# willake/cpu-ray-tracer

Measured on AMD Instinct MI355X. Metric: Mrays/sec (primary+secondary), 1280x720 64spp path trace — pipelined throughput over 878 consecutive 64-spp windows of one progressive render (single_render = one such render alone), higher is better.
Workload: dtype f32; 1 GPU; bunny_scene.xml FileScene BVH-SAH path tracer, 1280x720, 64 spp/step (passes=1, depthLimit=5); 1 step = 64 frames = the next spp window of a progressive render; the 878 steps are one crt_render job (14 render kernel launch(es), a wavefront per (tile, 128 consecutive frames), + ordered accumulate), one sync at the end; triangles=4968, parallelism=tile-wave x1

## Files before the change

cpu-ray-tracer_amd/csrc/abi.cpp:

```cpp
#include "../../include/crt_abi.h"
#include "device/launch.h"
#include "device/tile_class.h"
#include "host/grid_resolution.h"

#include <cmath>
#include <cstdarg>
#include <cstddef>
#include <cstdio>
#include <cstdlib>
#include <cstring>
#include <deque>
#include <string>
#include <algorithm>
#include <vector>
#include <chrono>

static_assert(sizeof(crt_bvh_node) == 32 && sizeof(crt_tri) == 112 && sizeof(crt_tlas_node) == 32, "reference layouts");
static_assert(sizeof(crt::NodePair) == 64 && sizeof(crt::LeafTri) == 48 && sizeof(crt::ShadeTri) == 64 && sizeof(crt::TlasNode) == 32 &&
              sizeof(crt::Instance) == 128 && sizeof(crt::Material) == 32 && offsetof(crt::Instance, T) == 64, "device layouts");
static_assert(sizeof(crt_counters) == sizeof(crt::Counters), "counter layout");
static_assert(sizeof(crt_kd_node) == 48 && sizeof(crt::KdNode) == sizeof(crt_kd_node) && sizeof(crt::AltTri) == 48, "flat KD node (uploaded as it comes), alternative accelerators' triangle record");
static_assert(offsetof(crt::PrimDev, red) == 536 && sizeof(crt::PrimDev) == 552, "PrimDev: 134 floats, then the two texel pointers");
static_assert(sizeof(crt::BlasAltDesc) == 72, "BLAS descriptor");
static_assert(sizeof(crt_shadow_ray) == 28 && sizeof(crt_ray) == 28 && sizeof(crt_hit) == 28, "query records");
static_assert(sizeof(crt_hit_info) == 48 && offsetof(crt_hit_info, material) == 12 && offsetof(crt_hit_info, N) == 16 && offsetof(crt_hit_info, albedo) == 32 && offsetof(crt_hit_info, v) == 44, "crt_hit_info: three 16-byte pieces");
static_assert(sizeof(crt::Instance) == 128 && offsetof(crt::Instance, triCount) == 112, "Instance record");

namespace {

thread_local std::string g_createError;

bool g_hooks = false;
inline const char* hook(const char* name) { return g_hooks ? getenv(name) : nullptr; }

struct EventPair { hipEvent_t a, b; int mode = -1; bool seen = false; };

}

extern "C" uint32_t crt_debug_query_grid(void)
{
    const char* e = hook("CRT_DEBUG_QUERY_GRID");
    const long k = e ? strtol(e, nullptr, 10) : 0;
    return k > 0 ? (uint32_t)(k > 0x7fffffffL ? 0x7fffffffL : k) : 0u;
}

struct crt_ctx {
    crt_config cfg{};
    std::string err;
    hipStream_t stream = nullptr;
    int tilesX = 0, tilesY = 0;
    uint32_t tileFirst = 0, tileStride = 1, tileCount = 0;
    void* dAccOwned = nullptr; void* dAcc = nullptr;
    std::vector<hipStream_t> streams; uint64_t launchSeq = 0;
    struct Region { size_t off, bytes; hipEvent_t freed; bool held = false; };
    std::deque<Region> inflight;
    char* pool = nullptr; size_t poolBytes = 0, poolHead = 0; bool poolCapped = false;
    hipEvent_t mustWait = nullptr;
    std::vector<hipEvent_t> freeEvents;
    std::vector<hipEvent_t> doneEvents;
    struct Ahead { hipEvent_t end; size_t off; const char* slab; uint64_t epoch; uint32_t sppFirst, nf, passes, used; };
    std::deque<Ahead> ahead;
    uint64_t epoch = 1;
    uint64_t tickEpoch = 0; uint32_t tickNextSpp = 0, tickPasses = 0;
    uint32_t aheadFrames = 0;
    hipStream_t aheadStream = nullptr;
    crt::Scene hScene{};
    crt::Counters* dCounters = nullptr;
    uint32_t* dQueryCursor = nullptr;
    int32_t* dInspectCounts = nullptr; void* dInspectWork = nullptr; size_t inspectCap = 0;
    uint32_t* dPixels = nullptr; float* dTileSums = nullptr;
    unsigned long long* dTileClocks = nullptr;
    std::vector<void*> sceneAllocs;
    float meshLo[3] = {0, 0, 0}, meshHi[3] = {0, 0, 0}; bool orderDirty = true;
    uint32_t* dTileOrder = nullptr;
    uint32_t* hTileOrder[2] = {nullptr, nullptr}; hipEvent_t orderCopied[2] = {nullptr, nullptr}; hipEvent_t orderReady = nullptr; int orderFlip = 0;
    bool classDirty = true;
    uint8_t* dTileClass = nullptr;
    uint8_t* hTileClass[2] = {nullptr, nullptr}; hipEvent_t classCopied[2] = {nullptr, nullptr}; int classFlip = 0;
    bool haveScene = false;
    struct Flat { int32_t kind = 0; uint64_t leafOff = 0, tlasOff = 0, tlasPairOff = 0, instOff = 0, shadeOff = 0; uint32_t tlasNodeCount = 0, maxHeight = 0;
                  uint32_t objects = 0;
                  std::vector<uint64_t> pairBase, triBase; std::vector<uint32_t> nodesUsed, triCount; std::vector<char> geom;
                  std::vector<float> rootBox; } flat;
    char* hStage[2] = {nullptr, nullptr}; size_t stageBytes[2] = {0, 0}; hipEvent_t stageCopied[2] = {nullptr, nullptr}; int stageFlip = 0;
    hipEvent_t sceneReady = nullptr, writeFence = nullptr;
    bool havePrim = false; crt::PrimDev prim{}; uint32_t* dPrimTex = nullptr;
    int renderAccel = 0;
    crt::AltAccelDev alt{}; bool haveKd = false, haveGrid = false; std::vector<void*> altAllocs[2]; crt::AltTri* altTris = nullptr; uint32_t altTriCount = 0;
    crt::TlasAltDev blasAlt[2]{}; bool haveBlas[2] = {false, false}; std::vector<void*> blasAllocs[2];
    bool hasAlt(int kind) const { return (kind == CRT_ACCEL_KDTREE && (haveKd || haveBlas[0])) || (kind == CRT_ACCEL_GRID && (haveGrid || haveBlas[1])); }
    char* dStage = nullptr; size_t stageCap = 0;
    static constexpr int kQuerySlots = 64;
    uint32_t* dQuerySlots = nullptr;
    struct QuerySlot { hipEvent_t done = nullptr; bool pending = false; } qslot[kQuerySlots];
    int qslotNext = 0;
    struct RefitPlan { void* dPlan = nullptr; uint32_t* dLevelOff = nullptr; uint32_t levels = 0, rootCode = 0; bool built = false; };
    std::vector<RefitPlan> refitPlans; std::vector<void*> refitAllocs;
    struct Refit {
        float* dBack = nullptr; float* hBack = nullptr; hipEvent_t done = nullptr;
        void release() { if (done) (void)hipEventDestroy(done); (void)hipFree(dBack); (void)hipHostFree(hBack); *this = Refit{}; }
    } refit;
    float* dRootBox = nullptr;
    struct TlasBuild {
        char* dBuild = nullptr; char* hBack = nullptr; size_t bytes = 0;
        hipEvent_t back = nullptr, done = nullptr, t0 = nullptr, t1 = nullptr; bool timed = false;
        void release() { for (hipEvent_t e : {back, done, t0, t1}) if (e) (void)hipEventDestroy(e); (void)hipFree(dBuild); (void)hipHostFree(hBack); *this = TlasBuild{}; }
    } tlasBuild;
    struct GridBuild {
        crt::GridBuildState* dState = nullptr; crt::GridBuildState* hState = nullptr;
        unsigned long long* dChunks = nullptr; uint32_t* dCursor = nullptr; int32_t* dUnsorted = nullptr; size_t cursorCap = 0, unsortedCap = 0;
        hipEvent_t back = nullptr, done = nullptr, t0 = nullptr, t1 = nullptr; bool built = false, timed = false; uint32_t blocks = 0;
        double waitMs[2] = {0, 0};
        void release() { for (hipEvent_t e : {back, done, t0, t1}) if (e) (void)hipEventDestroy(e); for (void* p : {(void*)dState, (void*)dChunks, (void*)dCursor, (void*)dUnsorted}) (void)hipFree(p); (void)hipHostFree(hState); *this = GridBuild{}; }
    } gridBuild;
    struct Retired { std::vector<void*> ptrs; void* pinned = nullptr; hipEvent_t unread = nullptr; };
    std::deque<Retired> retired; std::vector<hipEvent_t> retiredEvents;
    uint32_t gridRefCount = 0;
    struct BlasGrid { std::vector<crt::BlasAltDesc> desc; std::vector<uint32_t> cells, refs; std::vector<uint8_t> current; bool held = false; } blasGrid;
    hipEvent_t altReady = nullptr;
    static constexpr int kLatStages = 4;
    double tuneMs[kLatStages + 1] = {}; int tuneCount[kLatStages + 1] = {};
    hipEvent_t lastRenderEnd = nullptr;
    int latStage = 0;
    int latBest = 0;
    bool latDone = false;
    bool latConfirming = false; std::vector<int> latQueue;
    bool latWarm = false;
    uint32_t latSlots = 0;
    bool latProbed = false;
    std::vector<uint8_t> latL[kLatStages + 1];
    std::vector<uint32_t> latCost[kLatStages + 1];
    uint32_t* dTileCost = nullptr; uint32_t* hTileCost = nullptr; hipEvent_t costCopied = nullptr; bool costPending = false; int costStage = 0;
    uint32_t* dBlockDesc = nullptr; uint32_t* hBlockDesc = nullptr; uint32_t nBlocks = 0, descCap = 0; hipEvent_t descReady = nullptr;
    uint32_t* dJobCost = nullptr; uint32_t* hJobCost = nullptr; hipEvent_t jobCostCopied = nullptr; bool jobCostPending = false, jobCostValid = false;
    uint32_t recWaves = 0, recResident = 0, recWindows = 0; bool recPool = false;
    double poolWindowTicks = 0;
    std::vector<uint32_t> jobCost;
    std::vector<uint32_t> jobOrder;
    uint32_t* dJobDesc = nullptr; uint32_t* hJobDesc = nullptr; uint32_t jobDescCap = 0, jobBlocks = 0, jobHead = 0; hipEvent_t jobDescReady = nullptr;
    uint32_t planWindows = 0, planFrames = 0; bool planPool = false, planValid = false;
    double jobTrialMs[2] = {0, 0};
    uint32_t jobWaveOff = 0, jobWaveBlocks = 0, jobLongFrames = 0, jobLongWaves = 0, lastLongWaves = 0;
    std::vector<hipEvent_t> splitEvents;
    size_t splitSeq = 0; uint32_t splitLaunches = 0;
    uint64_t poolMinWaves = 65000;
    bool usePool = true;
    uint32_t ldsBytes = 0;
    uint32_t extraLds = 0;
    uint32_t poolLdsLimit = 0;
    std::vector<EventPair> evPool; size_t evUsedRender = 0, evUsedAcc = 0;
    std::deque<EventPair> evRender, evAcc;
    double foldedRenderMs = 0, foldedAccMs = 0; uint32_t foldedLaunches = 0, poolLaunches = 0;

    int fail(int code, const char* fmt, ...)
    {
        char buf[1024];
        va_list ap; va_start(ap, fmt); vsnprintf(buf, sizeof(buf), fmt, ap); va_end(ap);
        err = buf; return code;
    }
    int hip(hipError_t e, const char* what)
    {
        if (e == hipSuccess) return 0;
        return fail(CRT_ERR_DEVICE, "%s: %s", what, hipGetErrorString(e));
    }
    void freeAlt()
    {
        for (auto& v : altAllocs) { for (void* p : v) (void)hipFree(p); v.clear(); }
        if (altTris) (void)hipFree(altTris);
        altTris = nullptr; altTriCount = 0; haveKd = haveGrid = false; alt = crt::AltAccelDev{}; renderAccel = 0;
        for (int k = 0; k < 2; k++) { for (void* p : blasAllocs[k]) (void)hipFree(p); blasAllocs[k].clear(); haveBlas[k] = false; blasAlt[k] = crt::TlasAltDev{}; }
        blasGrid = BlasGrid{}; gridRefCount = 0;
        freeRetired(true);
    }
    void freeRetired(bool all)
    {
        while (!retired.empty()) {
            Retired& r = retired.front();
            if (!all && hipEventQuery(r.unread) != hipSuccess) { (void)hipGetLastError(); break; }
            for (void* p : r.ptrs) (void)hipFree(p);
            if (r.pinned) (void)hipHostFree(r.pinned);
            retiredEvents.push_back(r.unread); retired.pop_front();
        }
    }
    void freeScene()
    {
        for (void* p : sceneAllocs) (void)hipFree(p);
        sceneAllocs.clear(); haveScene = false; dRootBox = nullptr;
        for (void* p : refitAllocs) (void)hipFree(p);
        refitAllocs.clear(); refitPlans.clear();
        if (dPrimTex) { (void)hipFree(dPrimTex); dPrimTex = nullptr; }
        havePrim = false;
        freeAlt();
    }
};

#define HIPCK(ctx, call) do { hipError_t e_ = (call); if (e_ != hipSuccess) return (ctx)->hip(e_, #call); } while (0)

namespace {

template <class T>
int upload(crt_ctx* c, const std::vector<T>& v, const T** out)
{
    *out = nullptr;
    if (v.empty()) return 0;
    void* d = nullptr;
    HIPCK(c, hipMalloc(&d, v.size() * sizeof(T)));
    c->sceneAllocs.push_back(d);
    HIPCK(c, hipMemcpyAsync(d, v.data(), v.size() * sizeof(T), hipMemcpyHostToDevice, c->stream));
    HIPCK(c, hipStreamSynchronize(c->stream));
    *out = reinterpret_cast<const T*>(d);
    return 0;
}

template <class T>
int upload_array(crt_ctx* c, std::vector<void*>& allocs, const void* src, size_t bytes, const T** out)
{
    *out = nullptr; if (!bytes) return 0;
    void* d = nullptr; HIPCK(c, hipMalloc(&d, bytes)); allocs.push_back(d);
    HIPCK(c, hipMemcpy(d, src, bytes, hipMemcpyHostToDevice)); *out = static_cast<const T*>(d); return 0;
}

int bvh_height(crt_ctx* c, const crt_bvh& b, uint32_t* heightOut)
{
    std::vector<std::pair<uint32_t, uint32_t>> st; st.push_back({0u, 0u});
    uint32_t h = 0; size_t visited = 0;
    while (!st.empty()) {
        auto [n, d] = st.back(); st.pop_back();
        if (++visited > (size_t)b.nodesUsed) return c->fail(CRT_ERR_INVALID, "BVH node graph is not a tree");
        const crt_bvh_node& nd = b.nodes[n];
        if (nd.triCount > 0) { if (d > h) h = d; continue; }
        if (nd.leftFirst == 0 || nd.leftFirst + 1 >= b.nodesUsed) return c->fail(CRT_ERR_INVALID, "BVH child index out of range (node %u)", n);
        st.push_back({nd.leftFirst, d + 1}); st.push_back({nd.leftFirst + 1, d + 1});
    }
    *heightOut = h;
    return 0;
}

int wait_queries(crt_ctx* c)
{
    for (auto& q : c->qslot) if (q.pending) { HIPCK(c, hipEventSynchronize(q.done)); q.pending = false; }
    return 0;
}

hipError_t ensure_event(hipEvent_t* e, unsigned flags = hipEventDisableTiming) { return *e ? hipSuccess : hipEventCreateWithFlags(e, flags); }

int drain_all(crt_ctx* c)
{
    for (auto st : c->streams) HIPCK(c, hipStreamSynchronize(st));
    if (c->aheadStream) HIPCK(c, hipStreamSynchronize(c->aheadStream));
    HIPCK(c, hipStreamSynchronize(c->stream));
    return wait_queries(c);
}

}

extern "C" {

int crt_abi_version(void) { return CRT_ABI_VERSION; }

void crt_debug_enable_hooks(int on) { g_hooks = on != 0; }

static void primary_changed(crt_ctx* c) { crt::set_primary(c->hScene); c->classDirty = true; }

int crt_device_count(void)
{
    int n = 0;
    if (hipGetDeviceCount(&n) != hipSuccess) return 0;
    return n;
}

const char* crt_last_error(crt_ctx* ctx) { return ctx ? ctx->err.c_str() : g_createError.c_str(); }

int crt_create(crt_ctx** out, const crt_config* cfg)
{
    if (!out || !cfg) { g_createError = "crt_create: null argument"; return CRT_ERR_INVALID; }
    *out = nullptr;
    setenv("GPU_MAX_HW_QUEUES", "16", 0);
    if (cfg->width < 16 || cfg->height < 16) { g_createError = "crt_create: width and height must be at least one 16x16 tile"; return CRT_ERR_INVALID; }
    int ndev = 0;
    hipError_t e = hipGetDeviceCount(&ndev);
    if (e != hipSuccess || ndev == 0) {
        g_createError = "crt_create: no HIP device visible (this library has no CPU path)";
        return CRT_ERR_NO_DEVICE;
    }
    if (cfg->device < 0 || cfg->device >= ndev) { g_createError = "crt_create: device ordinal out of range"; return CRT_ERR_INVALID; }
    crt_ctx* c = new crt_ctx();
    c->cfg = *cfg;
    if (const char* k = hook("CRT_RENDER_KERNEL")) {
        c->usePool = strcmp(k, "tiles") != 0;
        if (!strcmp(k, "pool_always")) c->poolMinWaves = 0;
    }
    if (c->cfg.depthLimit < 0) c->cfg.depthLimit = 5;
    if (c->cfg.depthLimit > 5) { g_createError = "crt_create: depthLimit > 5 unsupported (throughput stack holds 5 factors; reference default is 5)"; delete c; return CRT_ERR_UNSUPPORTED; }
    if (c->cfg.maxFramesPerLaunch <= 0) c->cfg.maxFramesPerLaunch = c->cfg.collectStats ? 64 : 4096;
    if (c->cfg.maxFramesPerLaunch > 64) c->cfg.maxFramesPerLaunch = c->cfg.maxFramesPerLaunch / 64 * 64;
    if (c->cfg.renderStreams < 0) c->cfg.renderStreams = 0;
    c->tilesX = cfg->width / 16; c->tilesY = cfg->height / 16;
    const int tiles = c->tilesX * c->tilesY;
    int first = cfg->tileFirst, stride = cfg->tileStride <= 0 ? 1 : cfg->tileStride, count = cfg->tileCount;
    if (count < 0) { first = 0; stride = 1; count = tiles; }
    if (first < 0 || (count > 0 && (long long)first + (long long)(count - 1) * stride >= tiles)) {
        g_createError = "crt_create: tile range exceeds the image"; delete c; return CRT_ERR_INVALID;
    }
    c->tileFirst = (uint32_t)first; c->tileStride = (uint32_t)stride; c->tileCount = (uint32_t)count;

    auto bail = [&](hipError_t he, const char* what) {
        g_createError = std::string("crt_create: ") + what + ": " + hipGetErrorString(he);
        crt_destroy(c); return CRT_ERR_DEVICE;
    };
    if ((e = hipSetDevice(cfg->device)) != hipSuccess) return bail(e, "hipSetDevice");
    if ((e = hipStreamCreateWithFlags(&c->stream, hipStreamNonBlocking)) != hipSuccess) return bail(e, "hipStreamCreate");
    const size_t px = (size_t)cfg->width * cfg->height;
    if ((e = hipMalloc(&c->dAccOwned, px * 16)) != hipSuccess) return bail(e, "hipMalloc(accumulator)");
    c->dAcc = c->dAccOwned;
    if ((e = hipMemsetAsync(c->dAcc, 0, px * 16, c->stream)) != hipSuccess) return bail(e, "hipMemset(accumulator)");
    if ((e = hipMalloc((void**)&c->dPixels, px * 4)) != hipSuccess) return bail(e, "hipMalloc(pixels)");
    if ((e = hipMemsetAsync(c->dPixels, 0, px * 4, c->stream)) != hipSuccess) return bail(e, "hipMemset(pixels)");
    if ((e = hipMalloc((void**)&c->dTileSums, (size_t)tiles * 4)) != hipSuccess) return bail(e, "hipMalloc(tileSums)");
    if ((e = hipMemsetAsync(c->dTileSums, 0, (size_t)tiles * 4, c->stream)) != hipSuccess) return bail(e, "hipMemset(tileSums)");
    if ((e = hipMalloc((void**)&c->dCounters, sizeof(crt::Counters))) != hipSuccess) return bail(e, "hipMalloc(counters)");
    if ((e = hipMemsetAsync(c->dCounters, 0, sizeof(crt::Counters), c->stream)) != hipSuccess) return bail(e, "hipMemset(counters)");
    if ((e = hipMalloc((void**)&c->dQueryCursor, 64)) != hipSuccess) return bail(e, "hipMalloc(query cursor)");
    if ((e = hipMalloc((void**)&c->dQuerySlots, crt_ctx::kQuerySlots * 64)) != hipSuccess) return bail(e, "hipMalloc(query cursor slots)");
    if (c->cfg.collectStats && count > 0) {
        if ((e = hipMalloc((void**)&c->dTileClocks, (size_t)count * 144)) != hipSuccess) return bail(e, "hipMalloc(tileClocks)");
        if ((e = hipMemsetAsync(c->dTileClocks, 0, (size_t)count * 144, c->stream)) != hipSuccess) return bail(e, "hipMemset(tileClocks)");
    }
    memset(&c->hScene, 0, sizeof(c->hScene));
    const float aspect = (float)cfg->width / (float)cfg->height;
    crt::Scene& s = c->hScene;
    s.camPos[0] = 0; s.camPos[1] = 0; s.camPos[2] = -2;
    s.topLeft[0] = -aspect; s.topLeft[1] = 1; s.topLeft[2] = 0;
    s.topRight[0] = aspect; s.topRight[1] = 1; s.topRight[2] = 0;
    s.bottomLeft[0] = -aspect; s.bottomLeft[1] = -1; s.bottomLeft[2] = 0;
    s.W = cfg->width; s.H = cfg->height; s.invW = 1.0f / cfg->width; s.invH = 1.0f / cfg->height;
    s.depthLimit = c->cfg.depthLimit;
    primary_changed(c);
    if ((e = hipStreamSynchronize(c->stream)) != hipSuccess) return bail(e, "hipStreamSynchronize");
    *out = c;
    return CRT_OK;
}

void crt_destroy(crt_ctx* c)
{
    if (!c) return;
    (void)hipSetDevice(c->cfg.device);
    for (auto st : c->streams) (void)hipStreamSynchronize(st);
    if (c->aheadStream) (void)hipStreamSynchronize(c->aheadStream);
    if (c->stream) (void)hipStreamSynchronize(c->stream);
    for (auto& q : c->qslot) if (q.done) { if (q.pending) (void)hipEventSynchronize(q.done); (void)hipEventDestroy(q.done); }
    if (c->dQuerySlots) (void)hipFree(c->dQuerySlots);
    if (c->altReady) (void)hipEventDestroy(c->altReady);
    if (c->writeFence) (void)hipEventDestroy(c->writeFence);
    c->refit.release(); c->tlasBuild.release();
    c->freeScene();
    c->gridBuild.release();
    for (hipEvent_t e : c->retiredEvents) (void)hipEventDestroy(e);
    for (auto& a : c->ahead) (void)hipEventDestroy(a.end);
    if (c->aheadStream) (void)hipStreamDestroy(c->aheadStream);
    for (auto& ev : c->evPool) { (void)hipEventDestroy(ev.a); (void)hipEventDestroy(ev.b); }
    for (auto& ev : c->evRender) { (void)hipEventDestroy(ev.a); (void)hipEventDestroy(ev.b); }
    for (auto& ev : c->evAcc) { (void)hipEventDestroy(ev.a); (void)hipEventDestroy(ev.b); }
    if (c->dAccOwned) (void)hipFree(c->dAccOwned);
    for (auto st : c->streams) { (void)hipStreamSynchronize(st); (void)hipStreamDestroy(st); }
    for (auto& r : c->inflight) (void)hipEventDestroy(r.freed);
    for (auto e : c->freeEvents) (void)hipEventDestroy(e);
    if (c->mustWait) (void)hipEventDestroy(c->mustWait);
    if (c->pool) (void)hipFree(c->pool);
    for (auto e : c->doneEvents) (void)hipEventDestroy(e);
    if (c->dPixels) (void)hipFree(c->dPixels);
    if (c->dTileSums) (void)hipFree(c->dTileSums);
    if (c->dCounters) (void)hipFree(c->dCounters);
    if (c->dQueryCursor) (void)hipFree(c->dQueryCursor);
    if (c->dInspectCounts) (void)hipFree(c->dInspectCounts);
    if (c->dInspectWork) (void)hipFree(c->dInspectWork);
    if (c->dTileClocks) (void)hipFree(c->dTileClocks);
    if (c->dTileOrder) (void)hipFree(c->dTileOrder);
    if (c->dTileClass) (void)hipFree(c->dTileClass);
    if (c->dTileCost) (void)hipFree(c->dTileCost);
    if (c->dJobCost) (void)hipFree(c->dJobCost);
    if (c->dJobDesc) (void)hipFree(c->dJobDesc);
    if (c->hJobDesc) (void)hipHostFree(c->hJobDesc);
    if (c->jobDescReady) (void)hipEventDestroy(c->jobDescReady);
    if (c->hJobCost) (void)hipHostFree(c->hJobCost);
    if (c->jobCostCopied) (void)hipEventDestroy(c->jobCostCopied);
    for (auto e : c->splitEvents) (void)hipEventDestroy(e);
    if (c->hTileCost) (void)hipHostFree(c->hTileCost);
    if (c->costCopied) (void)hipEventDestroy(c->costCopied);
    if (c->dBlockDesc) (void)hipFree(c->dBlockDesc);
    if (c->hBlockDesc) (void)hipHostFree(c->hBlockDesc);
    if (c->descReady) (void)hipEventDestroy(c->descReady);
    if (c->dStage) (void)hipFree(c->dStage);
    for (int k = 0; k < 2; k++) { if (c->hTileOrder[k]) (void)hipHostFree(c->hTileOrder[k]); if (c->orderCopied[k]) (void)hipEventDestroy(c->orderCopied[k]); }
    for (int k = 0; k < 2; k++) { if (c->hTileClass[k]) (void)hipHostFree(c->hTileClass[k]); if (c->classCopied[k]) (void)hipEventDestroy(c->classCopied[k]); }
    for (int k = 0; k < 2; k++) { if (c->hStage[k]) (void)hipHostFree(c->hStage[k]); if (c->stageCopied[k]) (void)hipEventDestroy(c->stageCopied[k]); }
    if (c->stream) (void)hipStreamDestroy(c->stream);
    delete c;
}

int crt_upload_scene(crt_ctx* c, const crt_scene_desc* sd)
{
    if (!c || !sd) return CRT_ERR_INVALID;
    c->epoch++;
    HIPCK(c, hipSetDevice(c->cfg.device));
    if (sd->kind != CRT_SCENE_FILE && sd->kind != CRT_SCENE_TLAS) return c->fail(CRT_ERR_INVALID, "unknown scene kind %d", sd->kind);
    if (!sd->bvhs || sd->bvhCount == 0) return c->fail(CRT_ERR_INVALID, "scene has no acceleration structure");
    if (sd->kind == CRT_SCENE_FILE && sd->bvhCount != 1) return c->fail(CRT_ERR_INVALID, "CRT_SCENE_FILE takes exactly one BVH (FileScene::acc)");
    if (sd->kind == CRT_SCENE_TLAS && (sd->bvhCount > 256 || !sd->tlasNodes || sd->tlasNodeCount < 2 * sd->bvhCount))
        return c->fail(CRT_ERR_INVALID, "TLAS scene needs <= 256 BLAS (tlas_bvh.cpp:21) and 2*blasCount TLAS nodes");
    if (sd->textureCount == 0 || !sd->textures) return c->fail(CRT_ERR_INVALID, "floor and skydome textures are required");
    if (sd->floorTexture < 0 || sd->floorTexture >= (int)sd->textureCount || sd->skyTexture < 0 || sd->skyTexture >= (int)sd->textureCount)
        return c->fail(CRT_ERR_INVALID, "floor/sky texture index out of range");
    for (uint32_t i = 0; i < sd->textureCount; i++)
        if (!sd->textures[i].pixels || sd->textures[i].width <= 0 || sd->textures[i].height <= 0) return c->fail(CRT_ERR_INVALID, "texture %u is empty", i);
    if (sd->materialCount > 0 && !sd->materials) return c->fail(CRT_ERR_INVALID, "materialCount is %u but materials is NULL", sd->materialCount);
    for (uint32_t i = 0; i < sd->materialCount; i++)
        if (sd->materials[i].texture >= (int)sd->textureCount) return c->fail(CRT_ERR_INVALID, "material %u: texture index out of range", i);
    if (sd->kind == CRT_SCENE_FILE) {
        if (!sd->objMatIdx || sd->objCount == 0) return c->fail(CRT_ERR_INVALID, "CRT_SCENE_FILE needs objMatIdx");
        for (uint32_t i = 0; i < sd->objCount; i++)
            if (sd->objMatIdx[i] < 0 || sd->objMatIdx[i] >= (int)sd->materialCount) return c->fail(CRT_ERR_INVALID, "objMatIdx entry out of range");
    }

    uint64_t nPairs = 0, nTris = 0;
    uint32_t maxHeight = 0;
    for (uint32_t bi = 0; bi < sd->bvhCount; bi++) {
        const crt_bvh& b = sd->bvhs[bi];
        if (!b.nodes || !b.triangles || !b.triangleIndices || b.nodesUsed == 0 || b.triCount == 0) return c->fail(CRT_ERR_INVALID, "BVH %u is empty", bi);
        if ((b.nodesUsed & 1u) == 0) return c->fail(CRT_ERR_INVALID, "BVH %u: nodesUsed must be odd (root + child pairs)", bi);
        if (sd->kind == CRT_SCENE_TLAS && (b.matIdx < 0 || b.matIdx >= (int)sd->materialCount)) return c->fail(CRT_ERR_INVALID, "BLAS %u: matIdx out of range", bi);
        if (sd->kind == CRT_SCENE_TLAS && b.objIdx != (int)bi + 2)
            return c->fail(CRT_ERR_INVALID, "BLAS %u: objIdx must be %u (TLASFileScene numbers objects from 2, tlas_file_scene.cpp:13,51-53)", bi, bi + 2);
        uint32_t h = 0; int r = bvh_height(c, b, &h); if (r) return r;
        if (h > maxHeight) maxHeight = h;
        nPairs += b.nodesUsed / 2; nTris += b.triCount;
    }
    const uint64_t pairBytes = nPairs ? nPairs * 64 : 64;
    const uint64_t leafOffB = pairBytes, leafBytes = (nTris + 1) * 48;
    const uint64_t tlasOffB = (leafOffB + leafBytes + 63) & ~63ull;
    const uint64_t tlasBytes = (sd->kind == CRT_SCENE_TLAS) ? (uint64_t)sd->tlasNodeCount * 32 : 0;
    const uint64_t tlasPairOffB = (tlasOffB + tlasBytes + 63) & ~63ull;
    const uint64_t tlasPairBytes = (sd->kind == CRT_SCENE_TLAS) ? (uint64_t)sd->tlasNodeCount * 32 : 0;
    const uint64_t instOffB = (tlasPairOffB + tlasPairBytes + 127) & ~127ull;
    const uint64_t instBytes = (sd->kind == CRT_SCENE_TLAS) ? (uint64_t)sd->bvhCount * 128 : 0;
    const uint64_t shadeOffB = (instOffB + instBytes + 63) & ~63ull;
    const uint64_t total = shadeOffB + nTris * 64;
    if (total >= crt::kMaxGeomBytes) return c->fail(CRT_ERR_UNSUPPORTED, "scene geometry needs %llu bytes; this build addresses 4 GiB", (unsigned long long)total);
    if (sd->kind == CRT_SCENE_TLAS && sd->tlasNodeCount > 0x7fffu) return c->fail(CRT_ERR_UNSUPPORTED, "TLAS node index exceeds 15 bits");

    std::vector<char> geom((size_t)total, 0);
    crt::NodePair* pairs = reinterpret_cast<crt::NodePair*>(geom.data());
    crt::LeafTri* leaf = reinterpret_cast<crt::LeafTri*>(geom.data() + leafOffB);
    crt::TlasNode* tlas = reinterpret_cast<crt::TlasNode*>(geom.data() + tlasOffB);
    crt::NodePair* tlasPairs = reinterpret_cast<crt::NodePair*>(geom.data() + tlasPairOffB);
    const bool ref16ok = nPairs <= crt::kRef16MaxIndex && nTris < crt::kRef16MaxIndex && !hook("CRT_DEBUG_NO_REF16");
    const bool refWideOk = nPairs <= crt::kRefWideMaxIndex && nTris < crt::kRefWideMaxIndex && nPairs * 64 < crt::kMaxGeomBytes && leafOffB + nTris * 48 < crt::kMaxGeomBytes;
    const uint32_t poolRefBits = ref16ok ? 16u : (refWideOk ? 32u : 0u);
    const crt::PoolRefForm PR = crt::pool_ref_form(poolRefBits);
    crt::Instance* inst = reinterpret_cast<crt::Instance*>(geom.data() + instOffB);
    crt::ShadeTri* shade = reinterpret_cast<crt::ShadeTri*>(geom.data() + shadeOffB);

    uint64_t pairBase = 0, triBase = 0; uint32_t rootRef0 = 0, rootRef0_16 = 0;
    for (uint32_t bi = 0; bi < sd->bvhCount; bi++) {
        const crt_bvh& b = sd->bvhs[bi];
        auto ref_of = [&](uint32_t n, uint32_t* ref) -> int {
            const crt_bvh_node& nd = b.nodes[n];
            if (nd.triCount > 0) {
                if ((uint64_t)nd.leftFirst + nd.triCount > b.triCount) return c->fail(CRT_ERR_INVALID, "leaf range out of bounds (BVH %u node %u)", bi, n);
                *ref = (uint32_t)((leafOffB + (triBase + nd.leftFirst) * 48) >> 4);
            } else {
                if ((nd.leftFirst & 1u) == 0) return c->fail(CRT_ERR_INVALID, "interior node %u: children must be allocated pairwise starting at an odd index", n);
                *ref = crt::kRefInterior | (uint32_t)(((pairBase + ((nd.leftFirst - 1u) >> 1)) * 64) >> 4);
            }
            return 0;
        };
        auto ref16_of = [&](uint32_t n) -> uint32_t {
            const crt_bvh_node& nd = b.nodes[n];
            if (nd.triCount > 0) return (uint32_t)((triBase + nd.leftFirst + 1) & PR.indexMask);
            return PR.interior | (uint32_t)((pairBase + ((nd.leftFirst - 1u) >> 1)) & PR.indexMask);
        };
        int r;
        for (uint32_t n = 1; n + 1 < b.nodesUsed; n += 2) {
            crt::NodePair& p = pairs[pairBase + ((n - 1) >> 1)];
            for (int k = 0; k < 2; k++) {
                const crt_bvh_node& nd = b.nodes[n + k];
                memcpy(p.c[k].lo, nd.aabbMin, 12); memcpy(p.c[k].hi, nd.aabbMax, 12);
                if ((r = ref_of(n + k, &p.c[k].ref))) return r;
                p.c[k].ref16 = ref16_of(n + k);
            }
        }
        uint32_t rootRef = 0; if ((r = ref_of(0, &rootRef))) return r;
        const uint32_t rootRef16 = ref16_of(0);
        std::vector<uint32_t> remain(b.triCount, 1u);
        for (uint32_t n = 0; n < b.nodesUsed; n++) {
            const crt_bvh_node& nd = b.nodes[n];
            if (nd.triCount == 0) continue;
            for (uint32_t i = 0; i < nd.triCount; i++) remain[nd.leftFirst + i] = nd.triCount - i;
        }
        for (uint32_t j = 0; j < b.triCount; j++) {
            const uint32_t ti = b.triangleIndices[j];
            if (ti >= b.triCount) return c->fail(CRT_ERR_INVALID, "BVH %u: triangleIndices[%u] out of range", bi, j);
            const crt_tri& t = b.triangles[ti];
            crt::LeafTri& lt = leaf[triBase + j];
            for (int k = 0; k < 3; k++) { lt.v0[k] = t.vertex0[k]; lt.e1[k] = t.vertex1[k] - t.vertex0[k]; lt.e2[k] = t.vertex2[k] - t.vertex0[k]; }
            lt.shadeIdx = (uint32_t)(triBase + ti);
            lt.objIdx = (sd->kind == CRT_SCENE_TLAS) ? b.objIdx : t.objIdx;
            lt.remain = remain[j];
            if (sd->kind == CRT_SCENE_FILE && (t.objIdx < 2 || (uint32_t)(t.objIdx - 2) >= sd->objCount))
                return c->fail(CRT_ERR_INVALID, "triangle %u: objIdx %d has no entry in objMatIdx", ti, t.objIdx);
        }
        for (uint32_t ti = 0; ti < b.triCount; ti++) {
            const crt_tri& t = b.triangles[ti];
// ... 247 lines not shown
    } else if (s.rootRef & crt::kRefInterior) {
        memcpy(s.rootPair, f.geom.data() + ((size_t)(s.rootRef & crt::kRefOffsetMask) << 4), 64);
        s.rootIsPair = 1;
    }
    if (hook("CRT_DEBUG_NO_ROOTPAIR")) s.rootIsPair = 0;
    primary_changed(c);
    memcpy(c->meshLo, lo, 12); memcpy(c->meshHi, hi, 12); c->orderDirty = true;
}

static uint32_t pool_lds_need(const crt_ctx* c, uint32_t frames)
{
    return crt_pool_lds_bytes(c->hScene.stackDepth, crt_pool_streams(frames), c->hScene.poolRefBits) + c->extraLds;
}
static bool pool_can_run(crt_ctx* c, uint32_t frames)
{
    if (c->hScene.poolRefBits == 0u) return false;
    if (!c->poolLdsLimit) c->poolLdsLimit = crt_pool_lds_limit(c->cfg.device);
    return pool_lds_need(c, frames) <= c->poolLdsLimit;
}

static int check_tlas_height(crt_ctx* c, uint32_t tlasHeight)
{
    if ((c->hScene.bvhStack + tlasHeight + 1) * 64u * 4u + 15u * 256u > 64u * 1024u)
        return c->fail(CRT_ERR_UNSUPPORTED, "TLAS height %u needs %u bytes of LDS traversal stack per wave (> 64 KiB)", tlasHeight, (c->hScene.bvhStack + tlasHeight + 1) * 256u);
    return 0;
}

static void adopt_tlas(crt_ctx* c, uint32_t tlasHeight, const float* lo, const float* hi)
{
    crt::Scene& s = c->hScene;
    s.stackDepth = s.bvhStack + tlasHeight + 1;
    c->ldsBytes = s.stackDepth * 64u * 4u; c->latSlots = 0;
    set_root(c, CRT_SCENE_TLAS, lo, hi);
}

static void drop_blas_sets(crt_ctx* c)
{
    for (int k = 0; k < 2; k++) if (c->haveBlas[k]) { c->haveBlas[k] = false; if (c->renderAccel == k + 1) c->renderAccel = 0; }
}

int crt_update_scene(crt_ctx* c, const crt_scene_desc* sd, uint32_t what)
{
    if (!c || !sd) return CRT_ERR_INVALID;
    if (!c->haveScene) return c->fail(CRT_ERR_STATE, "crt_update_scene before crt_upload_scene");
    crt_ctx::Flat& f = c->flat;
    if (sd->kind != f.kind || sd->bvhCount != f.nodesUsed.size() || !sd->bvhs) return c->fail(CRT_ERR_INVALID, "crt_update_scene: scene kind / BVH count differ from the uploaded scene");
    if ((what & ~(uint32_t)(CRT_UPDATE_TRANSFORMS | CRT_UPDATE_BOUNDS)) || what == 0) return c->fail(CRT_ERR_INVALID, "crt_update_scene: unknown update flags");
    if ((what & CRT_UPDATE_TRANSFORMS) && f.kind != CRT_SCENE_TLAS) return c->fail(CRT_ERR_INVALID, "CRT_UPDATE_TRANSFORMS applies to two-level scenes (a FileScene bakes its transforms into the triangles)");
    HIPCK(c, hipSetDevice(c->cfg.device));
    for (uint32_t bi = 0; bi < sd->bvhCount; bi++)
        if (sd->bvhs[bi].nodesUsed != f.nodesUsed[bi] || sd->bvhs[bi].triCount != f.triCount[bi] || !sd->bvhs[bi].nodes || !sd->bvhs[bi].triangles || !sd->bvhs[bi].triangleIndices)
            return c->fail(CRT_ERR_INVALID, "crt_update_scene: BVH %u changed its topology (node / triangle count); upload the scene again", bi);
    if (f.kind == CRT_SCENE_TLAS && (!sd->tlasNodes || sd->tlasNodeCount != f.tlasNodeCount))
        return c->fail(CRT_ERR_INVALID, "crt_update_scene: a two-level scene needs the node array of the TLASBVH::Build that followed the change (tlasNodes, %u nodes as uploaded)", f.tlasNodeCount);
    if (what & CRT_UPDATE_BOUNDS) {
        const crt::LeafTri* leaf = reinterpret_cast<const crt::LeafTri*>(f.geom.data() + f.leafOff);
        for (uint32_t bi = 0; bi < sd->bvhCount; bi++) {
            const crt_bvh& b = sd->bvhs[bi];
            for (uint32_t j = 0; j < b.triCount; j++) {
                const uint32_t ti = b.triangleIndices[j];
                if (ti >= b.triCount) return c->fail(CRT_ERR_INVALID, "BVH %u: triangleIndices[%u] out of range", bi, j);
                if (leaf[f.triBase[bi] + j].shadeIdx != (uint32_t)(f.triBase[bi] + ti)) return c->fail(CRT_ERR_INVALID, "BVH %u: triangleIndices changed; Refit keeps the leaf order — upload the scene again", bi);
            }
        }
    }
    uint32_t tlasHeight = 0;
    std::vector<char> tlasImage;
    if (f.kind == CRT_SCENE_TLAS) {
        tlasImage.assign((size_t)(f.instOff - f.tlasOff), 0);
        int r = flatten_tlas(c, sd->tlasNodes, sd->tlasNodeCount, sd->bvhCount, reinterpret_cast<crt::TlasNode*>(tlasImage.data()),
                             reinterpret_cast<crt::NodePair*>(tlasImage.data() + (f.tlasPairOff - f.tlasOff)), &tlasHeight);
        if (r || (r = check_tlas_height(c, tlasHeight))) return r;
    }
    size_t lo = SIZE_MAX, hi = 0;
    auto touch = [&](size_t a, size_t b) { if (a < lo) lo = a; if (b > hi) hi = b; };
    if (what & CRT_UPDATE_BOUNDS) {
        crt::NodePair* pairs = reinterpret_cast<crt::NodePair*>(f.geom.data());
        crt::LeafTri* leaf = reinterpret_cast<crt::LeafTri*>(f.geom.data() + f.leafOff);
        for (uint32_t bi = 0; bi < sd->bvhCount; bi++) {
            const crt_bvh& b = sd->bvhs[bi];
            for (uint32_t n = 1; n + 1 < b.nodesUsed; n += 2) {
                crt::NodePair& p = pairs[f.pairBase[bi] + ((n - 1) >> 1)];
                for (int k = 0; k < 2; k++) { memcpy(p.c[k].lo, b.nodes[n + k].aabbMin, 12); memcpy(p.c[k].hi, b.nodes[n + k].aabbMax, 12); }
            }
            for (uint32_t j = 0; j < b.triCount; j++) {
                const crt_tri& t = b.triangles[b.triangleIndices[j]];
                crt::LeafTri& lt = leaf[f.triBase[bi] + j];
                for (int k = 0; k < 3; k++) { lt.v0[k] = t.vertex0[k]; lt.e1[k] = t.vertex1[k] - t.vertex0[k]; lt.e2[k] = t.vertex2[k] - t.vertex0[k]; }
            }
        }
        touch(0, (size_t)f.tlasOff);
        for (uint32_t bi = 0; bi < sd->bvhCount; bi++) { memcpy(&f.rootBox[6 * bi], sd->bvhs[bi].nodes[0].aabbMin, 12); memcpy(&f.rootBox[6 * bi + 3], sd->bvhs[bi].nodes[0].aabbMax, 12); }
    }
    if (f.kind == CRT_SCENE_TLAS) {
        if (what & CRT_UPDATE_TRANSFORMS) {
            crt::Instance* inst = reinterpret_cast<crt::Instance*>(f.geom.data() + f.instOff);
            for (uint32_t bi = 0; bi < sd->bvhCount; bi++) { memcpy(inst[bi].invT, sd->bvhs[bi].invT, 48); memcpy(inst[bi].T, sd->bvhs[bi].T, 48); }
        }
        memcpy(f.geom.data() + f.tlasOff, tlasImage.data(), tlasImage.size());
        touch((size_t)f.tlasOff, (size_t)f.shadeOff);
    }
    if (lo >= hi) return CRT_OK;
    const int k = c->stageFlip ^= 1;
    const size_t boxBytes = ((what & CRT_UPDATE_BOUNDS) && c->dRootBox) ? f.rootBox.size() * 4u : 0u;
    const size_t geomBytes = hi - lo, bytes = geomBytes + boxBytes;
    if (c->stageBytes[k] < bytes) {
        if (c->hStage[k]) { HIPCK(c, hipEventSynchronize(c->stageCopied[k])); HIPCK(c, hipHostFree(c->hStage[k])); c->hStage[k] = nullptr; }
        HIPCK(c, hipHostMalloc((void**)&c->hStage[k], bytes, hipHostMallocDefault)); c->stageBytes[k] = bytes;
        HIPCK(c, ensure_event(&c->stageCopied[k]));
    } else HIPCK(c, hipEventSynchronize(c->stageCopied[k]));
    memcpy(c->hStage[k], f.geom.data() + lo, geomBytes);
    if (boxBytes) memcpy(c->hStage[k] + geomBytes, f.rootBox.data(), boxBytes);
    { const int r = begin_scene_write(c, c->stream); if (r) return r; }
    if (what & CRT_UPDATE_BOUNDS) {
        std::fill(c->blasGrid.current.begin(), c->blasGrid.current.end(), (uint8_t)0);
        drop_blas_sets(c);
    }
    HIPCK(c, hipMemcpyAsync(const_cast<char*>(c->hScene.geom) + lo, c->hStage[k], geomBytes, hipMemcpyHostToDevice, c->stream));
    if (boxBytes) HIPCK(c, hipMemcpyAsync(c->dRootBox, c->hStage[k] + geomBytes, boxBytes, hipMemcpyHostToDevice, c->stream));
    { const int r = end_scene_write(c, c->stream, c->stageCopied[k]); if (r) return r; }
    if (f.kind == CRT_SCENE_TLAS) adopt_tlas(c, tlasHeight, sd->tlasNodes[0].aabbMin, sd->tlasNodes[0].aabbMax);
    else set_root(c, f.kind, sd->bvhs[0].nodes[0].aabbMin, sd->bvhs[0].nodes[0].aabbMax);
    return CRT_OK;
}

int crt_set_camera(crt_ctx* c, const float camPos[3], const float tl[3], const float tr[3], const float bl[3])
{
    if (!c || !camPos || !tl || !tr || !bl) return CRT_ERR_INVALID;
    HIPCK(c, hipSetDevice(c->cfg.device));
    crt::Scene& s = c->hScene;
    if (!memcmp(s.camPos, camPos, 12) && !memcmp(s.topLeft, tl, 12) && !memcmp(s.topRight, tr, 12) && !memcmp(s.bottomLeft, bl, 12)) return CRT_OK;
    memcpy(s.camPos, camPos, 12); memcpy(s.topLeft, tl, 12); memcpy(s.topRight, tr, 12); memcpy(s.bottomLeft, bl, 12);
    primary_changed(c);
    c->orderDirty = true; c->epoch++;
    return CRT_OK;
}

static int upload_tile_order(crt_ctx* c, const std::vector<uint32_t>& order)
{
    if (!c->dTileOrder) HIPCK(c, hipMalloc((void**)&c->dTileOrder, (size_t)c->tileCount * 4));
    { const int r = order_behind_ahead(c); if (r) return r; }
    const int k = c->orderFlip ^= 1;
    if (!c->hTileOrder[k]) {
        HIPCK(c, hipHostMalloc((void**)&c->hTileOrder[k], (size_t)c->tileCount * 4, hipHostMallocDefault));
        HIPCK(c, ensure_event(&c->orderCopied[k]));
    } else HIPCK(c, hipEventSynchronize(c->orderCopied[k]));
    memcpy(c->hTileOrder[k], order.data(), order.size() * 4);
    HIPCK(c, hipMemcpyAsync(c->dTileOrder, c->hTileOrder[k], order.size() * 4, hipMemcpyHostToDevice, c->stream));
    HIPCK(c, hipEventRecord(c->orderCopied[k], c->stream));
    c->orderReady = c->orderCopied[k];
    return 0;
}

static int update_tile_order(crt_ctx* c)
{
    if (!c->orderDirty || c->tileCount == 0) return 0;
    const crt::Scene& s = c->hScene;
    double R[3], Dn[3], N[3];
    for (int k = 0; k < 3; k++) { R[k] = (double)s.topRight[k] - s.topLeft[k]; Dn[k] = (double)s.bottomLeft[k] - s.topLeft[k]; }
    N[0] = R[1] * Dn[2] - R[2] * Dn[1]; N[1] = R[2] * Dn[0] - R[0] * Dn[2]; N[2] = R[0] * Dn[1] - R[1] * Dn[0];
    const double rr = R[0] * R[0] + R[1] * R[1] + R[2] * R[2], dd = Dn[0] * Dn[0] + Dn[1] * Dn[1] + Dn[2] * Dn[2];
    double E[3]; for (int k = 0; k < 3; k++) E[k] = (double)s.topLeft[k] - s.camPos[k];
    const double num = E[0] * N[0] + E[1] * N[1] + E[2] * N[2];
    auto rect_of = [&](const float* P8, int r[4]) -> bool {
        double u0 = 1e30, u1 = -1e30, v0 = 1e30, v1 = -1e30;
        for (int i = 0; i < 8; i++) {
            const float* P = P8 + 3 * i;
            double d[3] = {P[0] - s.camPos[0], P[1] - s.camPos[1], P[2] - s.camPos[2]};
            const double den = d[0] * N[0] + d[1] * N[1] + d[2] * N[2];
            const double t = den != 0 ? num / den : -1;
            if (!(t > 0) || rr == 0 || dd == 0) return false;
            double Q[3]; for (int k = 0; k < 3; k++) Q[k] = s.camPos[k] + t * d[k] - s.topLeft[k];
            const double u = (Q[0] * R[0] + Q[1] * R[1] + Q[2] * R[2]) / rr, v = (Q[0] * Dn[0] + Q[1] * Dn[1] + Q[2] * Dn[2]) / dd;
            if (u < u0) u0 = u; if (u > u1) u1 = u; if (v < v0) v0 = v; if (v > v1) v1 = v;
        }
        r[0] = (int)floor(u0 * c->cfg.width / 16.0) - 1; r[1] = (int)floor(u1 * c->cfg.width / 16.0) + 1;
        r[2] = (int)floor(v0 * c->cfg.height / 16.0) - 1; r[3] = (int)floor(v1 * c->cfg.height / 16.0) + 1;
        return true;
    };
    float world[24];
    for (int i = 0; i < 8; i++) { world[3 * i] = (i & 1) ? c->meshHi[0] : c->meshLo[0]; world[3 * i + 1] = (i & 2) ? c->meshHi[1] : c->meshLo[1]; world[3 * i + 2] = (i & 4) ? c->meshHi[2] : c->meshLo[2]; }
    int wr[4] = {0, c->tilesX - 1, 0, c->tilesY - 1};
    (void)rect_of(world, wr);
    std::vector<uint32_t> first, second, rest;
    for (uint32_t i = 0; i < c->tileCount; i++) {
        const uint32_t tile = c->tileFirst + i * c->tileStride;
        const int tx = (int)(tile % (uint32_t)c->tilesX), ty = (int)(tile / (uint32_t)c->tilesX);
        const bool inRect = tx >= wr[0] && tx <= wr[1] && ty >= wr[2] && ty <= wr[3];
        if (inRect) first.push_back(i); else rest.push_back(i);
    }
    for (int k = 0; k <= crt_ctx::kLatStages; k++) { c->tuneCount[k] = 0; c->tuneMs[k] = 0; }
    c->latStage = 0; c->latBest = 0; c->latDone = false; c->latWarm = false; c->latConfirming = false; c->latQueue.clear(); c->costPending = false; c->latProbed = false;
    first.insert(first.end(), rest.begin(), rest.end());
    c->jobCostValid = false; c->jobCostPending = false; c->planValid = false;
    { const int r = upload_tile_order(c, first); if (r) return r; }
    c->orderDirty = false;
    return 0;
}

static int update_tile_class(crt_ctx* c)
{
    if (!c->classDirty || c->tileCount == 0) return 0;
    if (!c->dTileClass) HIPCK(c, hipMalloc((void**)&c->dTileClass, (size_t)c->tileCount));
    { const int r = order_behind_ahead(c); if (r) return r; }
    const int k = c->classFlip ^= 1;
    if (!c->hTileClass[k]) {
        HIPCK(c, hipHostMalloc((void**)&c->hTileClass[k], (size_t)c->tileCount, hipHostMallocDefault));
        HIPCK(c, ensure_event(&c->classCopied[k]));
    } else HIPCK(c, hipEventSynchronize(c->classCopied[k]));
    crt::classify_tiles(c->hScene, c->cfg.width, c->cfg.height, (uint32_t)c->tilesX, c->tileFirst, c->tileStride, c->tileCount, c->hTileClass[k]);
    HIPCK(c, hipMemcpyAsync(c->dTileClass, c->hTileClass[k], (size_t)c->tileCount, hipMemcpyHostToDevice, c->stream));
    HIPCK(c, hipEventRecord(c->classCopied[k], c->stream));
    c->orderReady = c->classCopied[k];
    c->classDirty = false;
    return 0;
}

static size_t sample_bytes_per_window(const crt_ctx* c, uint32_t passes) { return (size_t)c->tileCount * 256u * 64u * passes * 16u; }
static size_t window_bytes(const crt_ctx* c, uint32_t passes) { return sample_bytes_per_window(c, passes) + (c->usePool ? crt_pool_scratch_bytes_per_window(c->tileCount) : 0); }

static uint32_t block_desc(uint32_t tile, uint32_t laneBase, uint32_t lanes, uint32_t window) { uint32_t lg = 0; while ((1u << lg) < lanes) lg++; return tile | (laneBase << 16) | (lg << 22) | (window << 25); }
static const uint32_t kLatLanes[7] = {64u, 32u, 16u, 8u, 4u, 2u, 1u};
static const double kLatG[7] = {1.0, 0.93, 0.88, 0.79, 0.69, 0.57, 0.48};
static int lat_index(uint32_t L) { int k = 0; while (k < 6 && kLatLanes[k] != L) k++; return k; }

static uint8_t next_lanes(uint8_t lanes, uint32_t cost, double T)
{
    int k = lat_index(lanes); const double unit = (double)cost / kLatG[k];
    while (k < 6 && unit * kLatG[k] > T) k++;
    while (k > 0 && unit * kLatG[k - 1] <= 0.9 * T) k--;
    return (uint8_t)kLatLanes[k];
}
extern "C" int crt_debug_next_lanes(const uint8_t* lanes, const uint32_t* cost, uint32_t n, double T, uint8_t* out)
{
    if (!lanes || !cost || !out) return CRT_ERR_INVALID;
    for (uint32_t i = 0; i < n; i++) { if (lanes[i] == 0 || lanes[i] > 64 || (64 % lanes[i]) != 0) return CRT_ERR_INVALID; out[i] = next_lanes(lanes[i], cost[i], T); }
    return CRT_OK;
}

static double solve_block_table(const std::vector<uint8_t>& lanes, const std::vector<uint32_t>& cost, double budget, std::vector<uint8_t>& out)
{
    const size_t n = cost.size();
    double topUnit = 0; for (size_t i = 0; i < n; i++) topUnit = std::max(topUnit, (double)cost[i] / kLatG[lat_index(lanes[i])]);
    out.assign(n, 64);
    if (topUnit <= 0) return 0;
    auto waves = [&](double T) { double w = 0; for (size_t i = 0; i < n; i++) w += 64.0 / next_lanes(lanes[i], cost[i], T); return w; };
    double lo = kLatG[6] * topUnit, hi = topUnit;
    if (waves(lo) > budget) { for (int it = 0; it < 14; it++) { const double mid = 0.5 * (lo + hi); if (waves(mid) <= budget) hi = mid; else lo = mid; } lo = hi; }
    for (size_t i = 0; i < n; i++) out[i] = next_lanes(lanes[i], cost[i], lo);
    return lo;
}
extern "C" int crt_debug_solve_block_table(const uint8_t* lanes, const uint32_t* cost, uint32_t n, double budget, uint8_t* out, double* T)
{
    if (!lanes || !cost || !out) return CRT_ERR_INVALID;
    for (uint32_t i = 0; i < n; i++) if (lanes[i] == 0 || lanes[i] > 64 || (64 % lanes[i]) != 0) return CRT_ERR_INVALID;
    std::vector<uint8_t> L; const double t = solve_block_table(std::vector<uint8_t>(lanes, lanes + n), std::vector<uint32_t>(cost, cost + n), budget, L);
    if (n) memcpy(out, L.data(), n);
    if (T) *T = t;
    return CRT_OK;
}
static double lat_budget(crt_ctx* c)
{
    if (!c->latSlots) c->latSlots = crt_render_resident_waves(c->cfg.device, c->hScene.kind, c->ldsBytes);
    double share = 0.98;
    if (const char* e = hook("CRT_LAT_BUDGET")) { const double v = atof(e); if (v > 0) share = v; }
    return share * (double)c->latSlots;
}

static int upload_block_table(crt_ctx* c, const std::vector<uint8_t>& lanes, const std::vector<uint32_t>& cost)
{
    const uint32_t n = c->tileCount;
    std::vector<uint32_t> order(n);
    for (uint32_t i = 0; i < n; i++) order[i] = i;
    std::stable_sort(order.begin(), order.end(), [&](uint32_t a, uint32_t b) { return cost[a] > cost[b]; });
    std::vector<uint32_t> table; table.reserve((size_t)n * 2);
    for (uint32_t r = 0; r < n; r++) {
        const uint32_t tl = order[r], L = lanes[tl];
        for (uint32_t base = 0; base < 64u; base += L) table.push_back(block_desc(tl, base, L, 0u));
    }
    if (table.size() > 0x7fffffffull) return c->fail(CRT_ERR_INVALID, "block table too large");
    if (hook("CRT_LAT_VERBOSE")) fprintf(stderr, "[crt] latency table: %zu wavefronts for %u tiles (slowest tile of the base stage %.2f ms)\n", table.size(), n, n ? cost[order[0]] * 1e-5 : 0.0);
    if (c->descCap < table.size()) {
        if (c->dBlockDesc) (void)hipFree(c->dBlockDesc);
        if (c->hBlockDesc) (void)hipHostFree(c->hBlockDesc);
        c->dBlockDesc = nullptr; c->hBlockDesc = nullptr; c->descCap = 0;
        const size_t cap = table.size() + table.size() / 2;
        HIPCK(c, hipMalloc((void**)&c->dBlockDesc, cap * 4));
        HIPCK(c, hipHostMalloc((void**)&c->hBlockDesc, cap * 4, hipHostMallocDefault));
        c->descCap = (uint32_t)cap;
    } else if (c->descReady) HIPCK(c, hipEventSynchronize(c->descReady));
    HIPCK(c, ensure_event(&c->descReady));
    memcpy(c->hBlockDesc, table.data(), table.size() * 4);
    { const int r = order_behind_ahead(c); if (r) return r; }
    HIPCK(c, hipMemcpyAsync(c->dBlockDesc, c->hBlockDesc, table.size() * 4, hipMemcpyHostToDevice, c->stream));
    HIPCK(c, hipEventRecord(c->descReady, c->stream));
    c->nBlocks = (uint32_t)table.size();
    return 0;
}

static int next_block_table(crt_ctx* c)
{
    const uint32_t n = c->tileCount; const int K = crt_ctx::kLatStages;
    const int s = c->costStage;
    if (s == 0 && !c->latWarm && !c->latProbed) { c->latWarm = true; return 0; }
    c->latCost[s].assign(c->hTileCost, c->hTileCost + n);
    if (s == 0 && !c->latProbed) c->latL[0].assign(n, 64);
    if (c->tuneCount[s] && (c->latBest == s || !c->tuneCount[c->latBest] || c->tuneMs[s] < c->tuneMs[c->latBest])) c->latBest = s;
    bool last = s >= K;
    std::vector<std::pair<double, uint32_t>> steps;
    if (const char* e = hook("CRT_LAT_POLICY")) {
        for (const char* p = e; *p;) {
            char* q = nullptr; const double sh = strtod(p, &q); if (q == p || *q != ':') break;
            const long L = strtol(q + 1, &q, 10); if (L < 1 || L > 64 || (64 % L) != 0) break;
            steps.push_back({sh, (uint32_t)L});
            p = (*q == ',') ? q + 1 : q; if (*q != ',') break;
        }
        if (s >= 1) last = true;
    }
    auto install = [&](int stage) -> int {
        if ((stage != 0 || c->latProbed) && stage != c->latStage) { const int r = upload_block_table(c, c->latL[stage], c->latCost[stage]); if (r) return r; }
        c->latStage = stage; return 0;
    };
    auto fastest = [&](int except) { int b = -1; for (int k = 0; k <= K; k++) if (k != except && c->tuneCount[k] && (b < 0 || c->tuneMs[k] < c->tuneMs[b])) b = k; return b; };
    auto finish = [&]() -> int {
        c->latDone = true; c->latConfirming = false;
        const int b = fastest(-1); c->latBest = b < 0 ? 0 : b;
        if (hook("CRT_LAT_FORCE")) c->latBest = s;
        if (hook("CRT_LAT_VERBOSE")) { fprintf(stderr, "[crt] latency stages:"); for (int k = 0; k <= K; k++) if (c->tuneCount[k]) fprintf(stderr, " %d: %.2f ms", k, c->tuneMs[k]); fprintf(stderr, " -> %d\n", c->latBest); }
        return install(c->latBest);
    };
    if (c->latConfirming) {
        if (!c->latQueue.empty()) c->latQueue.erase(c->latQueue.begin());
        if (!c->latQueue.empty()) return install(c->latQueue.front());
        return finish();
    }
    if (last) {
        const int a = fastest(-1), b2 = fastest(a);
        if (hook("CRT_LAT_FORCE") || a < 0 || b2 < 0) return finish();
        c->latQueue = {a, b2}; c->latConfirming = true;
        return install(a);
    }
    const int b = c->latBest;
    const std::vector<uint8_t>& baseL = c->latL[b]; const std::vector<uint32_t>& baseC = c->latCost[b];
    uint32_t top = 0; for (uint32_t i = 0; i < n; i++) top = baseC[i] > top ? baseC[i] : top;
    std::vector<uint8_t>& L = c->latL[s + 1]; L = baseL;
    if (!steps.empty()) {
        for (uint32_t i = 0; i < n; i++)
            for (const auto& st : steps) if (top > 0 && (double)baseC[i] >= st.first * (double)top) { L[i] = (uint8_t)st.second; break; }
    } else {
        const double T = solve_block_table(c->latL[s], c->latCost[s], lat_budget(c), L);
        if (hook("CRT_LAT_VERBOSE")) fprintf(stderr, "[crt] stage %d: aim %.2f ms\n", s + 1, T * 1e-5);
    }
    const int r = upload_block_table(c, L, steps.empty() ? c->latCost[s] : baseC);
    if (r) return r;
    c->latStage = s + 1;
    return 0;
}

static void harvest_tuning(crt_ctx* c)
{
    for (auto& ev : c->evRender) {
        if (ev.mode < 0 || ev.seen) continue;
        if (hipEventQuery(ev.b) != hipSuccess) break;
        float t = 0;
        if (hipEventElapsedTime(&t, ev.a, ev.b) == hipSuccess) {
            if (ev.mode >= 100) { double& m = c->jobTrialMs[ev.mode - 100]; m = (m > 0 && m < t) ? m : t; }
            else { c->tuneMs[ev.mode] = c->tuneCount[ev.mode] ? (c->tuneMs[ev.mode] < t ? c->tuneMs[ev.mode] : t) : t; c->tuneCount[ev.mode]++; }
        }
        ev.seen = true;
    }
}

static void fold_completed(crt_ctx* c, std::deque<EventPair>& list, double* ms, uint32_t* count)
{
    while (list.size() > 64 && hipEventQuery(list.front().b) == hipSuccess) {
        float t = 0;
        if (hipEventElapsedTime(&t, list.front().a, list.front().b) == hipSuccess) *ms += t;
        if (count) (*count)++;
        c->evPool.push_back(list.front()); list.pop_front();
    }
}

static int take_event(crt_ctx* c, std::deque<EventPair>& list, EventPair* out)
{
    EventPair ev;
    if (c->evPool.empty()) {
        HIPCK(c, hipEventCreate(&ev.a)); HIPCK(c, hipEventCreate(&ev.b));
    } else { ev = c->evPool.back(); c->evPool.pop_back(); }
    ev.mode = -1; ev.seen = false;
    list.push_back(ev); *out = ev;
    return 0;
}

static int release_ahead_region(crt_ctx* c, const crt_ctx::Ahead& a)
{
    for (auto& r : c->inflight)
        if (r.held && r.off == a.off) { HIPCK(c, hipEventRecord(r.freed, c->stream)); r.held = false; return 0; }
    return c->fail(CRT_ERR_DEVICE, "render-ahead region at %zu is not in the slab ring", a.off);
}

static int discard_ahead(crt_ctx* c)
{
    while (!c->ahead.empty()) {
        const crt_ctx::Ahead a = c->ahead.front(); c->ahead.pop_front();
        HIPCK(c, hipStreamWaitEvent(c->stream, a.end, 0));
        c->doneEvents.push_back(a.end);
        const int r = release_ahead_region(c, a); if (r) return r;
    }
    c->aheadFrames = 0;
    return 0;
}

static int ensure_pool(crt_ctx* c, uint32_t frames, uint32_t passes, uint32_t* maxFOut)
{
    const size_t windowBytes = window_bytes(c, passes);
    uint32_t maxF = (uint32_t)c->cfg.maxFramesPerLaunch;
    uint32_t maxW = maxF >= 64u ? maxF / 64u : 1u;
    const uint32_t wantW = (frames + 63u) / 64u;
    const uint32_t callW = wantW < maxW ? wantW : maxW;
    size_t want = (size_t)callW * windowBytes * (wantW > callW ? 2u : 1u);
    if (want < 8 * windowBytes) want = 8 * windowBytes;
    if (want > c->poolBytes && !(c->poolCapped && windowBytes <= c->poolBytes)) {
        { const int r = discard_ahead(c); if (r) return r; }
        HIPCK(c, hipStreamSynchronize(c->stream));
        for (auto st : c->streams) HIPCK(c, hipStreamSynchronize(st));
        if (c->aheadStream) HIPCK(c, hipStreamSynchronize(c->aheadStream));
        for (auto& r : c->inflight) c->freeEvents.push_back(r.freed);
        c->inflight.clear(); c->poolHead = 0;
        if (c->pool) { HIPCK(c, hipFree(c->pool)); c->pool = nullptr; c->poolBytes = 0; }
        size_t freeB = 0, totalB = 0;
        HIPCK(c, hipMemGetInfo(&freeB, &totalB));
        const size_t budget = freeB / 2;
        if (budget < windowBytes) return c->fail(CRT_ERR_DEVICE, "not enough free HBM for one 64-frame sample slab (%zu bytes needed, %zu free)", windowBytes, freeB);
        c->poolCapped = want > budget;
        if (want > budget) want = budget;
        want = want / windowBytes * windowBytes;
        HIPCK(c, hipMalloc((void**)&c->pool, want));
        c->poolBytes = want;
    }
    {
        uint32_t fitW = (uint32_t)(c->poolBytes / windowBytes);
        if (wantW > fitW && fitW >= 2) fitW /= 2;
        if (maxW > fitW) maxW = fitW;
    }
    if (maxF >= 64u) maxF = maxW * 64u;
    *maxFOut = maxF;
    return 0;
}

int crt_reserve(crt_ctx* c, uint32_t frames, uint32_t passes)
{
    if (!c) return CRT_ERR_INVALID;
    if (passes < 1 || passes > 4) return c->fail(CRT_ERR_INVALID, "passes must be 1..4");
    HIPCK(c, hipSetDevice(c->cfg.device));
    { const int r = discard_ahead(c); if (r) return r; }
    if (c->tileCount == 0 || frames == 0) return CRT_OK;
    uint32_t maxF = 0;
    return ensure_pool(c, frames, passes, &maxF);
}

static int take_region(crt_ctx* c, size_t need, hipStream_t st, size_t* offOut)
{
    for (;;) {
        bool ok = false; size_t off = 0;
        if (c->inflight.empty()) { off = 0; ok = need <= c->poolBytes; }
        else {
            const size_t tail = c->inflight.front().off;
            if (c->poolHead > tail) {
                if (c->poolBytes - c->poolHead >= need) { off = c->poolHead; ok = true; }
                else if (tail >= need) { off = 0; ok = true; }
            } else if (c->poolHead < tail && tail - c->poolHead >= need) { off = c->poolHead; ok = true; }
        }
        if (ok) {
            if (c->mustWait) HIPCK(c, hipStreamWaitEvent(st, c->mustWait, 0));
            c->poolHead = off + need; *offOut = off;
            return 0;
        }
        if (c->inflight.empty()) return c->fail(CRT_ERR_DEVICE, "slab pool of %zu bytes cannot hold a launch of %zu bytes", c->poolBytes, need);
        if (c->inflight.front().held) return 1;
        if (c->mustWait) c->freeEvents.push_back(c->mustWait);
        c->mustWait = c->inflight.front().freed;
        c->inflight.pop_front();
    }
}

static size_t job_cost_clk_offset(const crt_ctx* c) { return (((size_t)c->tileCount + 1u) & ~(size_t)1u) * 4u; }
static size_t job_cost_bytes(const crt_ctx* c) { return job_cost_clk_offset(c) + 24u; }

static int adopt_job_costs(crt_ctx* c)
{
    const uint32_t n = c->tileCount;
    c->jobCost.assign(c->hJobCost, c->hJobCost + n);
    {
        const unsigned long long* clk = reinterpret_cast<const unsigned long long*>(reinterpret_cast<const char*>(c->hJobCost) + job_cost_clk_offset(c));
        const double s0 = (clk[0] && clk[1] && clk[1] > ~clk[0]) ? (double)(clk[1] - ~clk[0]) : 0.0;
        const double drain = (double)clk[2] / (double)(c->recResident ? c->recResident : 1u);
        c->poolWindowTicks = 0;
        if (c->recWindows && (double)c->recWaves >= 1.5 * (double)c->recResident && s0 > 0) c->poolWindowTicks = (s0 + drain) / (double)c->recWindows / (c->recPool ? 1.0 : 1.2);
        if (hook("CRT_LAT_VERBOSE")) fprintf(stderr, "[crt] measured %u windows with %s: %u wavefronts, last one started %.2f ms after the first, then %.2f ms of drain -> %.3f ms of machine time per window under the pool\n", c->recWindows, c->recPool ? "the pool" : "one stream per lane", c->recWaves, s0 * 1e-5, drain * 1e-5, c->poolWindowTicks * 1e-5);
    }
    c->jobOrder.resize(n);
    for (uint32_t i = 0; i < n; i++) c->jobOrder[i] = i;
    std::stable_sort(c->jobOrder.begin(), c->jobOrder.end(), [&](uint32_t a, uint32_t b) { return c->jobCost[a] > c->jobCost[b]; });
    c->jobCostValid = true; c->planValid = false;
    return upload_tile_order(c, c->jobOrder);
}

static void plan_job(const crt_ctx* c, uint32_t windows, uint32_t frames, bool pool, std::vector<uint32_t>& table, uint32_t* head)
{
    table.clear(); *head = 0;
    const uint32_t n = c->tileCount;
    if (!c->jobCostValid || windows < 2u || windows > 64u || n > 0x10000u || c->cfg.collectStats || hook("CRT_SPLIT_OFF")) return;
    if (pool && c->streams.size() < 2) return;
    if (const char* e = hook("CRT_SPLIT_FORCE")) {
        const uint32_t h = std::min<uint32_t>((uint32_t)atoi(e), pool ? n - 1u : n);
        static const uint32_t Ls[4] = {64u, 16u, 2u, 1u};
        for (uint32_t r = 0; r < (pool ? h : n); r++) { const uint32_t L = r < h ? Ls[r & 3u] : 64u; for (uint32_t w = 0; w < windows; w++) for (uint32_t b0 = 0; b0 < 64u; b0 += L) table.push_back(block_desc(c->jobOrder[r], b0, L, w)); }
        *head = h; return;
    }
    double poolLong = 2.4, wideLoad = 1.1, poolSlots = 4096.0, wideMt = 1.2, narrowSlots = 3500.0;
    if (const char* e = hook("CRT_PLAN_NARROW_SLOTS")) narrowSlots = atof(e);
    const double K = (double)windows;
    double costSum = 0; for (uint32_t v : c->jobCost) costSum += (double)v;
    const double perCost = (c->poolWindowTicks > 0 && costSum > 0) ? c->poolWindowTicks / costSum : 1.0 / poolSlots;
    auto cheapest = [&](double v, double T, int* cls) -> double {
        if (pool && poolLong * v <= T) { *cls = 0; return K * v * perCost; }
        if (wideLoad * v <= T) { *cls = 1; return K * wideMt * v * perCost; }
        int k = 1; while (k < 6 && kLatG[k] * v > T) k++;
        *cls = 2 + k; return K * (64.0 / kLatLanes[k]) * kLatG[k] * v / narrowSlots;
    };
    auto machine = [&](double T) { double m = 0; int cls; for (uint32_t v : c->jobCost) m += cheapest((double)v, T, &cls); return m; };
    const double top = (double)c->jobCost[c->jobOrder[0]];
    double lo = top * kLatG[6], hi = std::max(poolLong * top, machine(1e30)) * 1.01;
    if (machine(lo) <= lo) hi = lo;
    else for (int it = 0; it < 50; it++) { const double mid = 0.5 * (lo + hi); if (machine(mid) <= mid) hi = mid; else lo = mid; }
    const double T = hi;
    uint32_t h = 0, narrow = 0; std::vector<uint8_t> lanes(n, 64);
    for (uint32_t r = 0; r < n; r++) {
        int cls; (void)cheapest((double)c->jobCost[c->jobOrder[r]], T, &cls);
        if (cls != 0) h = r + 1u;
        if (cls >= 2) { lanes[r] = (uint8_t)kLatLanes[cls - 2]; narrow++; }
    }
    if (pool && h >= n) h = n - 1u;
    if (hook("CRT_LAT_VERBOSE")) fprintf(stderr, "[crt] job of %u windows, %u tiles: makespan aim %.1f ms (most expensive tile %.2f ms); %u tiles to the block table, %u of them narrow, %s\n", windows, n, T * 1e-5, top * 1e-5, pool ? h : (narrow ? n : 0u), narrow, pool ? "rest to the pool" : "no pool");
    if (pool ? h == 0u : narrow == 0u) return;
    const uint32_t upto = pool ? h : n;
    for (uint32_t r = 0; r < upto; r++) {
        const uint32_t L = lanes[r];
        for (uint32_t w = 0; w < windows; w++) {
            const uint32_t fw = std::min(64u, frames - w * 64u);
            for (uint32_t b0 = 0; b0 < fw; b0 += L) table.push_back(block_desc(c->jobOrder[r], b0, L, w));
        }
    }
    if (table.size() > (4u << 20)) { table.clear(); *head = 0; return; }
    *head = pool ? h : 0u;
}

struct PoolWaveTerms { double poolLong = 2.4, load = 1.0, safety = 1.0, guard = 12.0, share = 1.0; };
static uint64_t pool_wave_plan(const uint32_t* cost, uint32_t nr, uint32_t frames, uint32_t S, double perCost, double startTicks, uint32_t resident, const PoolWaveTerms& tm,
                               std::vector<uint32_t>& wf, uint32_t* longFrames, std::vector<double>* start, double* aimOut)
{
    wf.assign(nr, S); *longFrames = 0;
    if (start) start->assign(nr, 0.0);
    if (aimOut) *aimOut = 0;
    const uint64_t perTile = (frames + S - 1u) / S, plain = (uint64_t)nr * perTile;
    if (!cost || S <= 64u || nr == 0u) return plain;
    const uint32_t F1 = (uint32_t)((double)frames * std::min(tm.share, 1.0)) / (8u * S) * (8u * S);
    if (F1 == 0u) return plain;
    double aim = startTicks, m = startTicks;
    std::vector<double> st(nr);
    for (uint32_t r = 0; r < nr; r++) { st[r] = m; m += (double)(F1 / 64u) * (double)cost[r] * perCost; aim += (double)((frames + 63u) / 64u) * (double)cost[r] * perCost; }
    if (start) *start = st;
    if (aimOut) *aimOut = aim;
    if ((double)plain < tm.guard * (double)resident) return plain;
    const uint64_t shortWaves = (uint64_t)nr * ((frames - F1 + S - 1u) / S);
    for (int kMax = 3; kMax >= 1; kMax--) {
        uint64_t waves = shortWaves; bool any = false;
        for (uint32_t r = 0; r < nr; r++) {
            int k = kMax;
            while (k > 0 && st[r] + tm.safety * tm.poolLong * tm.load * (double)cost[r] * (double)((uint64_t)S << k) / 128.0 > aim) k--;
            wf[r] = S << k; any = any || k > 0;
            waves += F1 / wf[r];
        }
        if (!any) break;
        if ((double)waves >= tm.guard * (double)resident) { *longFrames = F1; return waves; }
    }
    wf.assign(nr, S);
    return plain;
}
static uint32_t pool_wave_table(const std::vector<uint32_t>& wf, uint32_t longFrames, uint32_t S, std::vector<uint32_t>& tab, uint32_t* longWaves)
{
    tab.resize(2 * wf.size()); uint32_t b = 0, lw = 0;
    for (size_t r = 0; r < wf.size(); r++) {
        tab[2 * r] = b; tab[2 * r + 1] = wf[r];
        b += longFrames / wf[r];
        if (wf[r] > S) lw += longFrames / wf[r];
    }
    if (longWaves) *longWaves = lw;
    return b;
}
static bool pool_wave_terms(PoolWaveTerms& tm)
{
    if (const char* e = hook("CRT_POOL_REFILL_SAFETY")) { const double v = atof(e); if (v > 0) tm.safety = v; }
    if (const char* e = hook("CRT_POOL_REFILL_GUARD")) { const double v = atof(e); if (v > 0) tm.guard = v; }
    if (const char* e = hook("CRT_POOL_REFILL_SHARE")) { const double v = atof(e); if (v > 0) tm.share = v; }
    return !hook("CRT_POOL_REFILL_OFF");
}
static uint32_t forced_wave_frames(uint32_t S)
{
    const char* e = hook("CRT_POOL_WAVE_FRAMES");
    if (!e) return 0u;
    const long v = atol(e);
    if (v < (long)S) return S;
    return (uint32_t)std::min<long>(v, 8192) / S * S;
}

static int install_job_plan(crt_ctx* c, uint32_t windows, uint32_t frames, bool pool)
{
    if (c->planValid && c->planWindows == windows && c->planFrames == frames && c->planPool == pool) return 0;
    std::vector<uint32_t> table; uint32_t head = 0;
    plan_job(c, windows, frames, pool, table, &head);
    c->planValid = true; c->planWindows = windows; c->planFrames = frames; c->planPool = pool; c->jobHead = head; c->jobBlocks = (uint32_t)table.size();
    c->jobTrialMs[0] = c->jobTrialMs[1] = 0;
    c->jobWaveOff = c->jobWaveBlocks = c->jobLongFrames = c->jobLongWaves = 0;
    PoolWaveTerms terms;
    const uint32_t S = crt_pool_streams(frames);
    if (pool && c->jobCostValid && !c->cfg.collectStats && head < c->tileCount && pool_wave_terms(terms) && !forced_wave_frames(S)) {
        const uint32_t nr = c->tileCount - head;
        std::vector<uint32_t> cost(nr), wf, tab;
        double costSum = 0; for (uint32_t v : c->jobCost) costSum += (double)v;
        const double perCost = (c->poolWindowTicks > 0 && costSum > 0) ? c->poolWindowTicks / costSum : 1.0 / 4096.0;
        double startTicks = 0;
        for (uint32_t r = 0; r < head; r++) startTicks += (double)windows * 1.2 * (double)c->jobCost[c->jobOrder[r]] * perCost;
        for (uint32_t r = 0; r < nr; r++) cost[r] = c->jobCost[c->jobOrder[head + r]];
        double aim = 0; uint32_t F1 = 0, lw = 0, blocks = 0;
        pool_wave_plan(cost.data(), nr, frames, S, perCost, startTicks, 4096u, terms, wf, &F1, nullptr, &aim);
        if (F1) blocks = pool_wave_table(wf, F1, S, tab, &lw);
        if (lw) {
            c->jobWaveOff = (uint32_t)table.size(); c->jobWaveBlocks = blocks; c->jobLongFrames = F1; c->jobLongWaves = lw;
            table.insert(table.end(), tab.begin(), tab.end());
        }
        if (hook("CRT_LAT_VERBOSE")) {
            uint32_t cnt[4] = {0, 0, 0, 0}; double share[4] = {0, 0, 0, 0}, sum = 0;
            for (uint32_t r = 0; r < nr; r++) { int k = 0; while ((S << k) < wf[r]) k++; cnt[k]++; share[k] += cost[r]; sum += cost[r]; }
            fprintf(stderr, "[crt] pool launch of %u ranks x %u frames: aim %.1f ms, most expensive tile %.2f ms, long part %u frames in %u wavefronts, %u of them own more than %u frames (safety %.2f, guard %.1f x 4096, share %.2f); tiles by frames per wavefront (share of the cost):",
                    nr, frames, aim * 1e-5, nr ? cost[0] * 1e-5 : 0.0, F1, blocks, lw, S, terms.safety, terms.guard, terms.share);
            for (int k = 0; k < 4; k++) fprintf(stderr, " %u: %u (%.3f)", S << k, cnt[k], sum > 0 ? share[k] / sum : 0.0);
            fprintf(stderr, "\n");
        }
    }
    if (table.empty()) return 0;
    if (c->jobDescCap < table.size()) {
        if (c->dJobDesc) (void)hipFree(c->dJobDesc);
        if (c->hJobDesc) (void)hipHostFree(c->hJobDesc);
        c->dJobDesc = nullptr; c->hJobDesc = nullptr; c->jobDescCap = 0;
        const size_t cap = table.size() + table.size() / 2;
        HIPCK(c, hipMalloc((void**)&c->dJobDesc, cap * 4));
        HIPCK(c, hipHostMalloc((void**)&c->hJobDesc, cap * 4, hipHostMallocDefault));
        c->jobDescCap = (uint32_t)cap;
    } else if (c->jobDescReady) HIPCK(c, hipEventSynchronize(c->jobDescReady));
    HIPCK(c, ensure_event(&c->jobDescReady));
    memcpy(c->hJobDesc, table.data(), table.size() * 4);
    { const int r = order_behind_ahead(c); if (r) return r; }
    HIPCK(c, hipMemcpyAsync(c->dJobDesc, c->hJobDesc, table.size() * 4, hipMemcpyHostToDevice, c->stream));
    HIPCK(c, hipEventRecord(c->jobDescReady, c->stream));
    return 0;
}

struct Launch {
    hipStream_t st = nullptr; EventPair ev{}; void* slab = nullptr; uint32_t sppFirst = 0, nf = 0, passes = 1, windows = 1;
    const uint32_t* blockDesc = nullptr; uint32_t nBlocks = 0;
    bool wantCost = false, wantJobCost = false, pool = false;
    uint32_t head = 0, jobBlocks = 0; unsigned long long* jobClk = nullptr;
    uint32_t waveFrames = 0, waveBlocks = 0, longFrames = 0, longWaves = 0; const uint32_t* waveTab = nullptr;
};

static int next_block_table(crt_ctx* c);
static int probe_tile_costs(crt_ctx* c, hipStream_t st);

static int tuner_prepare(crt_ctx* c, Launch& L)
{
    int r;
    const bool gpuIdle = !c->lastRenderEnd || hipEventQuery(c->lastRenderEnd) == hipSuccess;
    if (L.nf <= 64u && L.nf >= 8u && gpuIdle && !c->cfg.collectStats && c->tileCount <= 0x10000u && !hook("CRT_LAT_OFF")) {
        if (c->costPending && hipEventQuery(c->costCopied) == hipSuccess) { c->costPending = false; harvest_tuning(c); if ((r = next_block_table(c))) return r; }
        if (c->latStage == 0 && !c->latProbed && !c->latWarm && !c->costPending && L.nf == 64u && !hook("CRT_LAT_POLICY") && !hook("CRT_LAT_NO_PROBE")) { if ((r = probe_tile_costs(c, L.st))) return r; }
        const int stage = c->latStage;
        if (stage || c->latProbed) { L.blockDesc = c->dBlockDesc; L.nBlocks = c->nBlocks; HIPCK(c, hipStreamWaitEvent(L.st, c->descReady, 0)); }
        L.wantCost = (!c->latDone && !c->costPending) || (c->latDone && hook("CRT_LAT_RECORD"));
        c->evRender.back().mode = c->latDone ? -1 : stage;
        if (L.wantCost && !c->latDone) c->costStage = stage;
    }
    if (L.wantCost) {
        if (!c->dTileCost) {
            HIPCK(c, hipMalloc((void**)&c->dTileCost, (size_t)c->tileCount * 4));
            HIPCK(c, hipHostMalloc((void**)&c->hTileCost, (size_t)c->tileCount * 4, hipHostMallocDefault));
            HIPCK(c, ensure_event(&c->costCopied));
        }
        else HIPCK(c, hipStreamWaitEvent(L.st, c->costCopied, 0));
        HIPCK(c, hipMemsetAsync(c->dTileCost, 0, (size_t)c->tileCount * 4, L.st));
    }
    return 0;
}

static int planner_prepare(crt_ctx* c, Launch& L)
{
    int r;
    if (L.nf > 64u && !c->cfg.collectStats) {
        if (c->jobCostPending && hipEventQuery(c->jobCostCopied) == hipSuccess) { c->jobCostPending = false; if ((r = adopt_job_costs(c))) return r; HIPCK(c, hipStreamWaitEvent(L.st, c->orderReady, 0)); }
        L.wantJobCost = !c->jobCostValid && !c->jobCostPending && L.nf >= 128u;
        if (L.wantJobCost) {
            if (!c->dJobCost) {
                HIPCK(c, hipMalloc((void**)&c->dJobCost, job_cost_bytes(c)));
                HIPCK(c, hipHostMalloc((void**)&c->hJobCost, job_cost_bytes(c), hipHostMallocDefault));
                HIPCK(c, ensure_event(&c->jobCostCopied));
            } else HIPCK(c, hipStreamWaitEvent(L.st, c->jobCostCopied, 0));
            HIPCK(c, hipMemsetAsync(c->dJobCost, 0, job_cost_bytes(c), L.st));
        }
    }
    const bool poolByDefault = c->hScene.poolRefBits == 16u || c->poolMinWaves == 0;
    const uint64_t minWaves = c->poolMinWaves != 65000u ? c->poolMinWaves : (c->jobCostValid ? 43000u : 65000u);
    L.pool = c->usePool && poolByDefault && pool_can_run(c, L.nf) && (uint64_t)c->tileCount * L.windows >= minWaves && (c->poolMinWaves == 0 || L.nf > 64u);
    if (L.nf > 64u && c->jobCostValid) {
        if ((r = install_job_plan(c, L.windows, L.nf, L.pool))) return r;
        int use = 1;
        if ((c->jobBlocks || c->jobLongWaves) && !hook("CRT_PLAN_NO_TRIAL")) {
            if (c->jobTrialMs[1] > 0 && c->jobTrialMs[0] > 0) use = c->jobTrialMs[1] <= c->jobTrialMs[0] ? 1 : 0;
            else if (c->jobTrialMs[1] > 0 && c->jobTrialMs[0] == 0) use = 0;
            c->evRender.back().mode = 100 + use;
        }
        if (use) { L.head = c->jobHead; L.jobBlocks = c->jobBlocks; if (L.pool && c->jobLongWaves) { L.waveTab = c->dJobDesc + c->jobWaveOff; L.waveBlocks = c->jobWaveBlocks; L.longFrames = c->jobLongFrames; L.longWaves = c->jobLongWaves; } }
    }
    if (L.pool) if (const uint32_t S = crt_pool_streams(L.nf); const uint32_t n = forced_wave_frames(S)) {
        L.waveFrames = n; L.waveTab = nullptr; L.waveBlocks = 0;
        L.longWaves = n > S ? (c->tileCount - L.head) * (L.nf / n + ((L.nf % n) > S ? 1u : 0u)) : 0u;
    }
    if (L.jobBlocks || L.waveTab) HIPCK(c, hipStreamWaitEvent(L.st, c->jobDescReady, 0));
    if (L.wantJobCost) {
        L.jobClk = reinterpret_cast<unsigned long long*>(reinterpret_cast<char*>(c->dJobCost) + job_cost_clk_offset(c));
        c->recPool = L.pool; c->recWindows = L.windows;
        const uint32_t perWave = L.pool ? std::max(crt_pool_streams(L.nf), L.waveFrames) : 64u;
        c->recWaves = L.pool ? c->tileCount * ((L.nf + perWave - 1u) / perWave) : c->tileCount * L.windows;
        c->recResident = L.pool ? 4096u : 5120u;
        if (L.pool && c->hScene.poolRefBits == 32u)
            c->recResident = 256u * std::min(16u, (160u * 1024u) / std::max(1u, pool_lds_need(c, L.nf)));
    }
    return 0;
}

static hipError_t launch_render_kernels(crt_ctx* c, const Launch& L)
{
    hipStream_t st = L.st;
    hipError_t le = hipSuccess;
    auto join = [&](hipStream_t other) -> hipError_t {
        if (other == st) return hipSuccess;
        hipError_t e = hipSuccess;
        if (c->splitEvents.size() < 32) { hipEvent_t ne; e = hipEventCreateWithFlags(&ne, hipEventDisableTiming); if (e == hipSuccess) c->splitEvents.push_back(ne); }
        if (e == hipSuccess) { hipEvent_t je = c->splitEvents[c->splitSeq++ % c->splitEvents.size()]; e = hipEventRecord(je, other); if (e == hipSuccess) e = hipStreamWaitEvent(st, je, 0); }
        return e;
    };
    auto launch_table = [&](const uint32_t* desc, uint32_t nBlocks, uint32_t* cost) -> hipError_t {
        return crt_launch_render(&c->hScene, L.slab, c->dCounters, c->dTileClocks, c->dTileOrder, c->tileFirst, c->tileStride, c->tileCount, (uint32_t)c->tilesX,
                                 L.sppFirst, L.nf, L.passes, c->ldsBytes, 0, desc, nBlocks, cost, 0u, nullptr, st);
    };
    if (L.pool) {
        void* scratch = (char*)L.slab + (size_t)L.windows * sample_bytes_per_window(c, L.passes);
        hipStream_t st2 = st;
        if (L.jobBlocks) {
            le = launch_table(c->dJobDesc, L.jobBlocks, nullptr);
            st2 = c->streams[(size_t)(c->launchSeq++ % c->streams.size())];
            if (le == hipSuccess && st2 != st) le = hipStreamWaitEvent(st2, L.ev.a, 0);
        }
        if (le == hipSuccess)
            le = crt_launch_render_pool(&c->hScene, L.slab, scratch, c->dCounters, c->dTileClocks, c->dTileOrder, c->tileFirst, c->tileStride, c->tileCount, (uint32_t)c->tilesX,
                                        L.sppFirst, L.nf, L.passes, c->cfg.collectStats, L.jobBlocks ? L.head : 0u, L.waveFrames, L.waveTab, L.waveBlocks, L.longFrames,
                                        L.wantJobCost ? c->dJobCost : nullptr, L.jobClk,
                                        (c->classDirty || hook("CRT_DEBUG_NO_TILE_CLASS")) ? nullptr : c->dTileClass , c->extraLds, st2);
        if (le == hipSuccess) c->lastLongWaves = L.longWaves;
        if (L.jobBlocks && le == hipSuccess) le = join(st2);
    } else if (L.jobBlocks) {
        le = launch_table(c->dJobDesc, L.jobBlocks, nullptr);
    } else if (L.blockDesc && L.nBlocks) {
        le = launch_table(L.blockDesc, L.nBlocks, L.wantCost ? c->dTileCost : nullptr);
    } else {
        le = crt_launch_render(&c->hScene, L.slab, c->dCounters, c->dTileClocks, c->dTileOrder, c->tileFirst, c->tileStride, c->tileCount, (uint32_t)c->tilesX,
                               L.sppFirst, L.nf, L.passes, c->ldsBytes, c->cfg.collectStats, nullptr, 0u,
                               L.wantCost ? c->dTileCost : (L.wantJobCost ? c->dJobCost : nullptr), 0u, L.jobClk, st);
    }
    if (L.jobBlocks && le == hipSuccess) c->splitLaunches++;
    return le;
}

static int probe_tile_costs(crt_ctx* c, hipStream_t st)
{
    const uint32_t n = c->tileCount;
    if (!c->dTileCost) {
        HIPCK(c, hipMalloc((void**)&c->dTileCost, (size_t)n * 4));
        HIPCK(c, hipHostMalloc((void**)&c->hTileCost, (size_t)n * 4, hipHostMallocDefault));
        HIPCK(c, ensure_event(&c->costCopied));
    } else HIPCK(c, hipEventSynchronize(c->costCopied));
    const auto tp0 = std::chrono::steady_clock::now();
    HIPCK(c, crt_launch_probe(&c->hScene, c->tileFirst, c->tileStride, n, (uint32_t)c->tilesX, c->dTileCost, st));
    HIPCK(c, hipMemcpyAsync(c->hTileCost, c->dTileCost, (size_t)n * 4, hipMemcpyDeviceToHost, st));
    HIPCK(c, hipEventRecord(c->costCopied, st));
    HIPCK(c, hipStreamSynchronize(st));
    const auto tp1 = std::chrono::steady_clock::now();
    std::vector<uint32_t>& est = c->latCost[0]; est.assign(c->hTileCost, c->hTileCost + n);
    for (uint32_t i = 0; i < n; i++) est[i] += 18u * crt_probe_paths();
    std::vector<uint8_t>& L = c->latL[0]; L.assign(n, 64);
    solve_block_table(std::vector<uint8_t>(n, 64), est, lat_budget(c), L);
    c->latProbed = true;
    bool any = false; for (uint32_t i = 0; i < n; i++) any = any || L[i] != 64;
    if (!any) { c->latProbed = false; return 0; }
    const auto tp2 = std::chrono::steady_clock::now();
    const int r = upload_block_table(c, L, est);
    if (hook("CRT_LAT_VERBOSE")) { const auto tp3 = std::chrono::steady_clock::now(); auto ms = [](auto a, auto b) { return std::chrono::duration<double, std::milli>(b - a).count(); };
        fprintf(stderr, "[crt] cost probe: launch + wait %.3f ms, table solved in %.3f ms, uploaded in %.3f ms\n", ms(tp0, tp1), ms(tp1, tp2), ms(tp2, tp3)); }
    return r;
}

static int launch_frames(crt_ctx* c, uint32_t sppFirst, uint32_t nf, uint32_t passes, hipStream_t st, crt_ctx::Ahead* ahead)
{
    const size_t windowBytes = window_bytes(c, passes);
    size_t off = 0; int r;
    if ((r = take_region(c, (size_t)((nf + 63u) / 64u) * windowBytes, st, &off))) return r;
    if (c->orderReady) HIPCK(c, hipStreamWaitEvent(st, c->orderReady, 0));
    if ((r = wait_scene(c, st))) return r;
    void* slab = c->pool + off;
    EventPair ev;
    harvest_tuning(c);
    fold_completed(c, c->evRender, &c->foldedRenderMs, &c->foldedLaunches); fold_completed(c, c->evAcc, &c->foldedAccMs, nullptr);
    if ((r = take_event(c, c->evRender, &ev))) return r;
    struct PairGuard { crt_ctx* c; bool armed; ~PairGuard() { if (armed && !c->evRender.empty()) { c->evPool.push_back(c->evRender.back()); c->evRender.pop_back(); } } } pairGuard{c, true};
    Launch L; L.st = st; L.ev = ev; L.slab = slab; L.sppFirst = sppFirst; L.nf = nf; L.passes = passes; L.windows = (nf + 63u) / 64u;
    if ((r = tuner_prepare(c, L))) return r;
    if ((r = planner_prepare(c, L))) return r;
    HIPCK(c, hipEventRecord(ev.a, st));
    const bool pool = L.pool, wantCost = L.wantCost, wantJobCost = L.wantJobCost;
    const hipError_t le = hook("CRT_DEBUG_FAIL_LAUNCH") ? hipErrorInvalidConfiguration  : launch_render_kernels(c, L);
    if (le != hipSuccess) {
        return c->hip(le, pool ? "launch of render_pool_kernel" : "launch of render_tiles_kernel");
    }
    if (pool) c->poolLaunches++;
    HIPCK(c, hipEventRecord(ev.b, st));
    pairGuard.armed = false;
    c->lastRenderEnd = ev.b;
    if (wantJobCost) {
        HIPCK(c, hipMemcpyAsync(c->hJobCost, c->dJobCost, job_cost_bytes(c), hipMemcpyDeviceToHost, st));
        HIPCK(c, hipEventRecord(c->jobCostCopied, st));
        c->jobCostPending = true;
    }
    if (wantCost && !pool && !c->latDone) {
        HIPCK(c, hipMemcpyAsync(c->hTileCost, c->dTileCost, (size_t)c->tileCount * 4, hipMemcpyDeviceToHost, st));
        HIPCK(c, hipEventRecord(c->costCopied, st));
        c->costPending = true;
    }
    crt_ctx::Region reg; reg.off = off; reg.bytes = (size_t)((nf + 63u) / 64u) * windowBytes;
    if (c->freeEvents.empty()) HIPCK(c, hipEventCreateWithFlags(&reg.freed, hipEventDisableTiming));
    else { reg.freed = c->freeEvents.back(); c->freeEvents.pop_back(); }
    if (ahead) {
        hipEvent_t end = nullptr;
        if (c->doneEvents.empty()) { const hipError_t e = hipEventCreateWithFlags(&end, hipEventDisableTiming); if (e != hipSuccess) { c->freeEvents.push_back(reg.freed); return c->hip(e, "hipEventCreate"); } }
        else { end = c->doneEvents.back(); c->doneEvents.pop_back(); }
        const hipError_t e = hipEventRecord(end, st);
        if (e != hipSuccess) { c->doneEvents.push_back(end); c->freeEvents.push_back(reg.freed); return c->hip(e, "hipEventRecord"); }
        reg.held = true;
        c->inflight.push_back(reg);
        *ahead = crt_ctx::Ahead{end, off, (const char*)slab, c->epoch, sppFirst, nf, passes, 0u};
        return 0;
    }
    HIPCK(c, hipStreamWaitEvent(c->stream, ev.b, 0));
    if ((r = take_event(c, c->evAcc, &ev))) return r;
    HIPCK(c, hipEventRecord(ev.a, c->stream));
    HIPCK(c, crt_launch_accumulate(slab, c->dAcc, c->tileFirst, c->tileStride, c->tileCount, (uint32_t)c->tilesX, (uint32_t)c->cfg.width, nf, passes, c->stream));
    HIPCK(c, hipEventRecord(ev.b, c->stream));
    HIPCK(c, hipEventRecord(reg.freed, c->stream));
    c->inflight.push_back(reg);
    return 0;
}

int crt_render(crt_ctx* c, uint32_t spp_first, uint32_t frames, uint32_t passes)
{
    if (!c) return CRT_ERR_INVALID;
    if (!c->haveScene && !c->havePrim) return c->fail(CRT_ERR_STATE, "crt_render before crt_upload_scene");
    if (passes < 1 || passes > 4) return c->fail(CRT_ERR_INVALID, "passes must be 1..4 (the reference's UI range, renderer.cpp:178)");
    HIPCK(c, hipSetDevice(c->cfg.device));
    { int r = discard_ahead(c); if (r) return r; }
    if (c->tileCount == 0 || frames == 0) return CRT_OK;
    { int r = update_tile_order(c); if (r) return r; }
    { int r = update_tile_class(c); if (r) return r; }
    if (c->streams.empty()) {
        int n = c->cfg.renderStreams;
        if (n <= 0) n = 7;
        if (n > 16) n = 16;
        if (c->cfg.collectStats) n = 1;
        c->streams.resize((size_t)n);
        for (auto& st : c->streams) HIPCK(c, hipStreamCreateWithFlags(&st, hipStreamNonBlocking));
    }
    uint32_t maxF = 0;
    { int r = ensure_pool(c, frames, passes, &maxF); if (r) return r; }
    const size_t windowBytes = window_bytes(c, passes);
    if (c->renderAccel != 0 || c->havePrim) {
        for (uint32_t f0 = 0; f0 < frames; f0 += maxF) {
            const uint32_t nf = (frames - f0 < maxF) ? frames - f0 : maxF;
            size_t off = 0; int r;
            if ((r = take_region(c, (size_t)((nf + 63u) / 64u) * windowBytes, c->stream, &off))) return r;
            if ((r = wait_scene(c, c->stream))) return r;
            void* slab = c->pool + off;
            if (c->havePrim) HIPCK(c, crt_launch_render_prim(&c->hScene, &c->prim, slab, c->dCounters, c->tileFirst, c->tileStride, c->tileCount, (uint32_t)c->tilesX, spp_first + f0 * passes, nf, passes, c->stream));
            else HIPCK(c, crt_launch_render_alt(c->renderAccel, &c->hScene, &c->alt, &c->blasAlt[c->renderAccel - 1], slab, c->dCounters, c->tileFirst, c->tileStride, c->tileCount, (uint32_t)c->tilesX, spp_first + f0 * passes, nf, passes, c->stream));
            HIPCK(c, crt_launch_accumulate(slab, c->dAcc, c->tileFirst, c->tileStride, c->tileCount, (uint32_t)c->tilesX, (uint32_t)c->cfg.width, nf, passes, c->stream));
            crt_ctx::Region reg; reg.off = off; reg.bytes = (size_t)((nf + 63u) / 64u) * windowBytes;
            if (c->freeEvents.empty()) HIPCK(c, hipEventCreateWithFlags(&reg.freed, hipEventDisableTiming));
            else { reg.freed = c->freeEvents.back(); c->freeEvents.pop_back(); }
            HIPCK(c, hipEventRecord(reg.freed, c->stream));
            c->inflight.push_back(reg);
        }
        return CRT_OK;
    }
    for (uint32_t f0 = 0; f0 < frames; f0 += maxF) {
        const uint32_t nf = (frames - f0 < maxF) ? frames - f0 : maxF;
        const int r = launch_frames(c, spp_first + f0 * passes, nf, passes, c->streams[(size_t)(c->launchSeq++ % c->streams.size())], nullptr);
        if (r) return r > 0 ? c->fail(CRT_ERR_DEVICE, "slab ring blocked by a render-ahead region") : r;
    }
    return CRT_OK;
}

int crt_sync(crt_ctx* c)
{
    if (!c) return CRT_ERR_INVALID;
    HIPCK(c, hipSetDevice(c->cfg.device));
    HIPCK(c, hipStreamSynchronize(c->stream));
    for (auto st : c->streams) HIPCK(c, hipStreamSynchronize(st));
    if (c->aheadStream) HIPCK(c, hipStreamSynchronize(c->aheadStream));
    return CRT_OK;
}

int crt_clear(crt_ctx* c)
{
    if (!c) return CRT_ERR_INVALID;
    HIPCK(c, hipSetDevice(c->cfg.device));
    HIPCK(c, hipMemsetAsync(c->dAcc, 0, (size_t)c->cfg.width * c->cfg.height * 16, c->stream));
    return CRT_OK;
}

int crt_read_accumulator(crt_ctx* c, float* host)
{
    if (!c || !host) return CRT_ERR_INVALID;
    HIPCK(c, hipSetDevice(c->cfg.device));
    HIPCK(c, hipMemcpyAsync(host, c->dAcc, (size_t)c->cfg.width * c->cfg.height * 16, hipMemcpyDeviceToHost, c->stream));
    HIPCK(c, hipStreamSynchronize(c->stream));
    return CRT_OK;
}

static int read_screen(crt_ctx* c, uint32_t* hostPixels, float* energy)
{
    const int tiles = c->tilesX * c->tilesY;
    if (hostPixels) HIPCK(c, hipMemcpyAsync(hostPixels, c->dPixels, (size_t)c->cfg.width * c->cfg.height * 4, hipMemcpyDeviceToHost, c->stream));
    std::vector<float> sums(tiles);
    HIPCK(c, hipMemcpyAsync(sums.data(), c->dTileSums, (size_t)tiles * 4, hipMemcpyDeviceToHost, c->stream));
    HIPCK(c, hipStreamSynchronize(c->stream));
    if (energy) { float e = 0; for (int i = 0; i < tiles; i++) e += sums[i]; *energy = e; }
    return CRT_OK;
}

int crt_resolve_screen(crt_ctx* c, float scale, uint32_t* hostPixels, float* energy)
{
    if (!c) return CRT_ERR_INVALID;
    HIPCK(c, hipSetDevice(c->cfg.device));
    HIPCK(c, crt_launch_resolve(c->dAcc, c->dPixels, c->dTileSums, c->tileFirst, c->tileStride, c->tileCount, (uint32_t)c->tilesX, (uint32_t)c->cfg.width, scale, c->stream));
    return read_screen(c, hostPixels, energy);
}

static constexpr uint32_t kAheadMaxFrames = 256;

static int launch_ahead(crt_ctx* c, uint32_t sppFirst, uint32_t passes)
{
    if (!c->aheadStream) {
        int least = 0, greatest = 0;
        HIPCK(c, hipDeviceGetStreamPriorityRange(&least, &greatest));
        HIPCK(c, hipStreamCreateWithPriority(&c->aheadStream, hipStreamNonBlocking, least));
    }
    uint32_t nf = c->aheadFrames ? std::min(2u * c->aheadFrames, kAheadMaxFrames) : 64u;
    if (nf > (uint32_t)c->cfg.maxFramesPerLaunch) nf = (uint32_t)c->cfg.maxFramesPerLaunch;
    const uint32_t poolW = (uint32_t)(c->poolBytes / window_bytes(c, passes));
    if (nf > poolW / 2u * 64u) nf = poolW / 2u * 64u;
    if (nf == 0 || c->streams.empty()) return 0;
    hipStream_t st = hook("CRT_AHEAD_NORMAL_PRIORITY") ? c->streams[(size_t)(c->launchSeq++ % c->streams.size())] : c->aheadStream;
    crt_ctx::Ahead a{};
    const int r = launch_frames(c, sppFirst, nf, passes, st, &a);
    if (r < 0) return r;
    if (r > 0) return 0;
    c->ahead.push_back(a); c->aheadFrames = nf;
    return 0;
}

int crt_tick(crt_ctx* c, uint32_t spp, uint32_t passes, uint32_t* hostPixels, float* hostRgba, float* energy)
{
    if (!c) return CRT_ERR_INVALID;
    if (!c->haveScene && !c->havePrim) return c->fail(CRT_ERR_STATE, "crt_tick before crt_upload_scene");
    if (passes < 1 || passes > 4) return c->fail(CRT_ERR_INVALID, "passes must be 1..4 (the reference's UI range, renderer.cpp:178)");
    HIPCK(c, hipSetDevice(c->cfg.device));
    const float scale = 1.0f / (float)(spp + passes);
    const bool eligible = !c->cfg.collectStats && c->renderAccel == 0 && !c->havePrim && c->tileCount > 0;
    const bool streak = eligible && c->tickEpoch == c->epoch && spp == c->tickNextSpp && passes == c->tickPasses;
    c->tickEpoch = c->epoch; c->tickNextSpp = spp + passes; c->tickPasses = passes;
    const bool hit = !c->ahead.empty() && c->ahead.front().epoch == c->epoch && c->ahead.front().passes == passes &&
                     spp == c->ahead.front().sppFirst + c->ahead.front().used * passes;
    int r;
    if (hit) {
        crt_ctx::Ahead& a = c->ahead.front();
        const uint32_t f = a.used++;
        HIPCK(c, hipStreamWaitEvent(c->stream, a.end, 0));
        HIPCK(c, crt_launch_commit_frame(a.slab + (size_t)(f / 64u) * sample_bytes_per_window(c, passes), f % 64u, passes, c->dAcc, c->dPixels, c->dTileSums,
                                         c->tileFirst, c->tileStride, c->tileCount, (uint32_t)c->tilesX, (uint32_t)c->cfg.width, scale, c->stream));
        if (a.used == a.nf) {
            const crt_ctx::Ahead done = a; c->ahead.pop_front();
            c->doneEvents.push_back(done.end);
            if ((r = release_ahead_region(c, done))) return r;
        }
        if (c->ahead.size() < 2u) {
            const uint32_t next = c->ahead.empty() ? spp + passes : c->ahead.back().sppFirst + c->ahead.back().nf * passes;
            if ((r = launch_ahead(c, next, passes))) return r;
        }
    } else {
        if ((r = crt_render(c, spp, 1, passes))) return r;
        HIPCK(c, crt_launch_resolve(c->dAcc, c->dPixels, c->dTileSums, c->tileFirst, c->tileStride, c->tileCount, (uint32_t)c->tilesX, (uint32_t)c->cfg.width, scale, c->stream));
    }
    if (hostRgba) HIPCK(c, hipMemcpyAsync(hostRgba, c->dAcc, (size_t)c->cfg.width * c->cfg.height * 16, hipMemcpyDeviceToHost, c->stream));
    if ((r = read_screen(c, hostPixels, energy))) return r;
    if (!hit && streak && (r = launch_ahead(c, spp + passes, passes))) return r;
    return CRT_OK;
}

int crt_whitted_tick(crt_ctx* c, uint32_t* hostPixels)
{
    if (!c) return CRT_ERR_INVALID;
    if (!c->haveScene) return c->fail(CRT_ERR_STATE, "crt_whitted_tick before crt_upload_scene");
    HIPCK(c, hipSetDevice(c->cfg.device));
    HIPCK(c, crt_launch_whitted(&c->hScene, c->renderAccel, &c->alt, c->renderAccel ? &c->blasAlt[c->renderAccel - 1] : nullptr, c->dAcc, c->dPixels, c->dCounters, c->ldsBytes, c->stream));
    if (hostPixels) HIPCK(c, hipMemcpyAsync(hostPixels, c->dPixels, (size_t)c->cfg.width * c->cfg.height * 4, hipMemcpyDeviceToHost, c->stream));
    HIPCK(c, hipStreamSynchronize(c->stream));
    return CRT_OK;
// ... 939 lines not shown
    if (!c || !out) return CRT_ERR_INVALID;
    if (!c->dTileClocks) return c->fail(CRT_ERR_STATE, "tile clocks are recorded only by a collectStats context");
    HIPCK(c, hipSetDevice(c->cfg.device));
    HIPCK(c, hipMemcpyAsync(out, c->dTileClocks, (size_t)c->tileCount * 16, hipMemcpyDeviceToHost, c->stream));
    HIPCK(c, hipStreamSynchronize(c->stream));
    return CRT_OK;
}

extern "C" int crt_debug_pool_lds(crt_ctx* c, uint32_t frames, uint32_t* bytes, uint32_t* limit, uint32_t* refBits)
{
    if (!c || !c->haveScene) return -1;
    if (!c->poolLdsLimit) c->poolLdsLimit = crt_pool_lds_limit(c->cfg.device);
    if (bytes) *bytes = c->hScene.poolRefBits ? pool_lds_need(c, frames) : 0u;
    if (limit) *limit = c->poolLdsLimit;
    if (refBits) *refBits = c->hScene.poolRefBits;
    return 0;
}
extern "C" int crt_debug_live_events(crt_ctx* c) { return c ? (int)(2 * (c->evRender.size() + c->evAcc.size() + c->evPool.size())) : -1; }

extern "C" int crt_debug_check_reciprocals(crt_ctx* c, uint64_t* out)
{
    if (!c || !out) return CRT_ERR_INVALID;
    HIPCK(c, hipSetDevice(c->cfg.device));
    unsigned long long* d = nullptr;
    HIPCK(c, hipMalloc(&d, 32));
    hipError_t e = hipMemsetAsync(d, 0, 32, c->stream);
    if (e == hipSuccess) e = crt_launch_check_reciprocals(d, c->stream);
    if (e == hipSuccess) e = hipMemcpyAsync(out, d, 32, hipMemcpyDeviceToHost, c->stream);
    if (e == hipSuccess) e = hipStreamSynchronize(c->stream);
    (void)hipFree(d);
    HIPCK(c, e);
    return CRT_OK;
}

extern "C" int crt_debug_check_sqrt(crt_ctx* c, uint64_t* out)
{
    if (!c || !out) return CRT_ERR_INVALID;
    HIPCK(c, hipSetDevice(c->cfg.device));
    unsigned long long* d = nullptr;
    HIPCK(c, hipMalloc(&d, 16));
    hipError_t e = hipMemsetAsync(d, 0, 16, c->stream);
    if (e == hipSuccess) e = crt_launch_check_sqrt(d, c->stream);
    if (e == hipSuccess) e = hipMemcpyAsync(out, d, 16, hipMemcpyDeviceToHost, c->stream);
    if (e == hipSuccess) e = hipStreamSynchronize(c->stream);
    (void)hipFree(d);
    HIPCK(c, e);
    return CRT_OK;
}

extern "C" int crt_debug_primary_block(crt_ctx* c, float* out, float* camera, float* lightFloor)
{
    if (!c || !out) return CRT_ERR_INVALID;
    const crt::Scene& s = c->hScene;
    static_assert(offsetof(crt::Scene, primRoot) == offsetof(crt::Scene, rootPair) + 64 && offsetof(crt::Scene, primDown) + 12 == offsetof(crt::Scene, rootPair) + 64 + 4 * crt::kPrimFloats, "primary block");
    memcpy(out, s.rootPair, 64 + 4 * crt::kPrimFloats);
    if (camera) memcpy(camera, s.camPos, 48);
    if (lightFloor) { lightFloor[0] = s.lightInvT[7]; lightFloor[1] = s.lightInvT[3]; lightFloor[2] = s.lightInvT[11]; lightFloor[3] = s.floorD; }
    return CRT_OK;
}
extern "C" int crt_debug_primary_block_host(int op, const float* in, float* out)
{
    static crt::Scene s{};
    if (!in || !out || op < 0 || op > 2) return CRT_ERR_INVALID;
    if (op == 0) {
        s = crt::Scene{};
        s.camPos[2] = -2; s.topLeft[0] = -1; s.topLeft[1] = 1; s.topRight[0] = 1; s.topRight[1] = 1; s.bottomLeft[0] = -1; s.bottomLeft[1] = -1;
        memcpy(s.lightInvT, in, 48); s.floorD = in[12]; memcpy(s.rootPair, in + 13, 64); s.rootIsPair = 1;
    } else if (op == 1) { memcpy(s.camPos, in, 12); memcpy(s.topLeft, in + 3, 12); memcpy(s.topRight, in + 6, 12); memcpy(s.bottomLeft, in + 9, 12); }
    else memcpy(s.rootPair, in, 64);
    crt::set_primary(s);
    memcpy(out, s.rootPair, 64 + 4 * crt::kPrimFloats);
    return CRT_OK;
}

extern "C" int crt_debug_tile_classes(crt_ctx* c, uint8_t* out, uint32_t cap)
{
    if (!c || (!out && cap)) return CRT_ERR_INVALID;
    HIPCK(c, hipSetDevice(c->cfg.device));
    { const int r = update_tile_class(c); if (r) return r; }
    const uint32_t n = cap < c->tileCount ? cap : c->tileCount;
    if (n) {
        HIPCK(c, hipMemcpyAsync(out, c->dTileClass, n, hipMemcpyDeviceToHost, c->stream));
        HIPCK(c, hipStreamSynchronize(c->stream));
    }
    return (int)c->tileCount;
}
extern "C" int crt_debug_tile_classes_host(const float* in, uint32_t flags, int W, int H, uint32_t tileFirst, uint32_t tileStride, uint32_t tileCount, uint8_t* out)
{
    if (!in || !out || W < 16 || H < 16 || tileStride == 0) return CRT_ERR_INVALID;
    const uint32_t tilesX = (uint32_t)(W / 16), tiles = tilesX * (uint32_t)(H / 16);
    if (tileCount && (unsigned long long)tileFirst + (unsigned long long)(tileCount - 1) * tileStride >= tiles) return CRT_ERR_INVALID;
    crt::Scene s{};
    memcpy(s.camPos, in, 12); memcpy(s.topLeft, in + 3, 12); memcpy(s.topRight, in + 6, 12); memcpy(s.bottomLeft, in + 9, 12);
    s.W = W; s.H = H; s.invW = 1.0f / W; s.invH = 1.0f / H;
    s.lightInvT[0] = s.lightInvT[5] = s.lightInvT[10] = 1.0f; s.lightInvT[3] = in[12]; s.lightInvT[7] = in[13]; s.lightInvT[11] = in[14];
    s.lightSize = in[15]; s.floorN[1] = 1.0f; s.floorD = in[16];
    memcpy(s.rootPair, in + 17, 64);
    s.lightAxis = flags & 1u; s.floorAxisY = (flags >> 1) & 1u; s.rootIsPair = (flags >> 2) & 1u;
    crt::set_primary(s);
    crt::classify_tiles(s, W, H, tilesX, tileFirst, tileStride, tileCount, out);
    return CRT_OK;
}

static int device_probe(crt_ctx* c, int op, const void* in, void* out, uint32_t n)
{
    static const uint8_t words[18][2] = {{1, 1}, {1, 1}, {2, 1}, {1, 1}, {2, 1}, {6, 7}, {1, 18}, {4, 1}, {5, 3}, {13, 2}, {16, 4}, {2, 2}, {2, 2}, {2, 2}, {2, 2}, {4, 2}, {2, 1}, {5, 3}};
    if (!c || !in || !out || op < 0 || op > 17 || n > (1u << 25)) return CRT_ERR_INVALID;
    if (n == 0) return CRT_OK;
    const size_t inBytes = (size_t)n * words[op][0] * 4, outBytes = (size_t)n * words[op][1] * 4;
    HIPCK(c, hipSetDevice(c->cfg.device));
    char* d = nullptr;
    HIPCK(c, hipMalloc((void**)&d, inBytes + outBytes));
    hipError_t e = hipMemcpyAsync(d, in, inBytes, hipMemcpyHostToDevice, c->stream);
    if (e == hipSuccess) e = (op <= 10 || op == 17) ? crt_launch_probe_f32(op, d, d + inBytes, n, c->stream) : crt_launch_probe_f64(op, d, d + inBytes, n, c->stream);
    if (e == hipSuccess) e = hipMemcpyAsync(out, d + inBytes, outBytes, hipMemcpyDeviceToHost, c->stream);
    if (e == hipSuccess) e = hipStreamSynchronize(c->stream);
    (void)hipFree(d);
    HIPCK(c, e);
    return CRT_OK;
}
extern "C" int crt_debug_device_probe(crt_ctx* c, int op, const void* in, void* out, uint32_t n) { return (op > 16) ? CRT_ERR_INVALID : device_probe(c, op, in, out, n); }
extern "C" int crt_debug_sky_probe(crt_ctx* c, const void* in, void* out, uint32_t n) { return device_probe(c, 17, in, out, n); }

extern "C" int crt_debug_plan_job(const uint32_t* cost, uint32_t n, uint32_t windows, uint32_t frames, int pool, double poolWindowTicks,
                                  uint32_t* table, uint32_t tableCap, uint32_t* head, uint32_t* order)
{
    if (!cost || !n || !table || !head || !order) return CRT_ERR_INVALID;
    crt_ctx c;
    c.tileCount = n; c.jobCostValid = true; c.poolWindowTicks = poolWindowTicks;
    c.streams.assign(2, nullptr);
    c.jobCost.assign(cost, cost + n);
    c.jobOrder.resize(n);
    for (uint32_t i = 0; i < n; i++) c.jobOrder[i] = i;
    std::stable_sort(c.jobOrder.begin(), c.jobOrder.end(), [&](uint32_t a, uint32_t b) { return c.jobCost[a] > c.jobCost[b]; });
    std::vector<uint32_t> t; uint32_t h = 0;
    plan_job(&c, windows, frames, pool != 0, t, &h);
    c.streams.clear();
    if (t.size() > tableCap) return CRT_ERR_INVALID;
    memcpy(table, t.data(), t.size() * 4); memcpy(order, c.jobOrder.data(), (size_t)n * 4); *head = h;
    return (int)t.size();
}

extern "C" long long crt_debug_pool_wave_plan(const uint32_t* cost, uint32_t nr, uint32_t frames, double perCost, double startTicks, uint32_t resident, double safety, double guard,
                                              double share, uint32_t* wf, uint32_t* longFrames, double* start, double* aim)
{
    if (!nr || !frames || !wf || !longFrames) return CRT_ERR_INVALID;
    PoolWaveTerms tm; if (safety > 0) tm.safety = safety; if (guard > 0) tm.guard = guard; if (share > 0) tm.share = share;
    std::vector<uint32_t> w; std::vector<double> st;
    const uint64_t waves = pool_wave_plan(cost, nr, frames, crt_pool_streams(frames), perCost, startTicks, resident, tm, w, longFrames, &st, aim);
    memcpy(wf, w.data(), (size_t)nr * 4);
    if (start) memcpy(start, st.data(), (size_t)nr * 8);
    return (long long)waves;
}
extern "C" int crt_debug_pool_long_waves(crt_ctx* c) { return c ? (int)c->lastLongWaves : -1; }
extern "C" void crt_debug_pool_wave_terms(double* out) { const PoolWaveTerms tm; out[0] = tm.poolLong; out[1] = tm.load; out[2] = tm.safety; out[3] = tm.guard; out[4] = tm.share; }

extern "C" int crt_debug_tile_costs(crt_ctx* c, uint32_t* out)
{
    if (!c || !out || !c->dTileCost) return CRT_ERR_INVALID;
    HIPCK(c, hipSetDevice(c->cfg.device));
    HIPCK(c, hipDeviceSynchronize());
    HIPCK(c, hipMemcpy(out, c->dTileCost, (size_t)c->tileCount * 4, hipMemcpyDeviceToHost));
    return CRT_OK;
}

extern "C" int crt_debug_lat_stage(crt_ctx* c, int stage, uint8_t* lanes, uint32_t* cost)
{
    if (!c || stage < 0 || stage > crt_ctx::kLatStages) return CRT_ERR_INVALID;
    if (c->latL[stage].size() != c->tileCount || c->latCost[stage].size() != c->tileCount) return CRT_ERR_STATE;
    if (lanes) memcpy(lanes, c->latL[stage].data(), c->tileCount);
    if (cost) memcpy(cost, c->latCost[stage].data(), (size_t)c->tileCount * 4);
    return c->latStage;
}

extern "C" int crt_debug_tile_stamps(crt_ctx* c, uint64_t* out)
{
    if (!c || !out || !c->dTileClocks) return CRT_ERR_INVALID;
    HIPCK(c, hipSetDevice(c->cfg.device));
    HIPCK(c, hipMemcpyAsync(out, c->dTileClocks + 2 * (size_t)c->tileCount, (size_t)c->tileCount * 128, hipMemcpyDeviceToHost, c->stream));
    HIPCK(c, hipStreamSynchronize(c->stream));
    return CRT_OK;
}

int crt_bind_accumulator(crt_ctx* c, void* p)
{
    if (!c) return CRT_ERR_INVALID;
    if (p && ((uintptr_t)p & 15u)) return c->fail(CRT_ERR_INVALID, "accumulator pointer must be 16-byte aligned");
    HIPCK(c, hipSetDevice(c->cfg.device));
    HIPCK(c, hipStreamSynchronize(c->stream));
    c->dAcc = p ? p : c->dAccOwned;
    return CRT_OK;
}

int crt_accumulator_device_ptr(crt_ctx* c, void** p)
{
    if (!c || !p) return CRT_ERR_INVALID;
    *p = c->dAcc; return CRT_OK;
}

}
```

cpu-ray-tracer_amd/csrc/device/launch.h:

```cpp
#pragma once
#include "layout.h"

#include <hip/hip_runtime.h>

extern "C" {

hipError_t crt_launch_check_reciprocals(unsigned long long* out, hipStream_t stream);
hipError_t crt_launch_check_sqrt(unsigned long long* out, hipStream_t stream);
hipError_t crt_launch_render(const crt::Scene* sc, void* slab, crt::Counters* counters, unsigned long long* tileClocks, const uint32_t* tileOrder, uint32_t tileFirst, uint32_t tileStride,
    uint32_t tileCount, uint32_t tilesX, uint32_t sppFirst, uint32_t frames, uint32_t passes, uint32_t ldsBytes, int collectStats, const uint32_t* blockDesc, uint32_t nBlocks, uint32_t* tileCost,
    uint32_t rankCount, unsigned long long* launchClk, hipStream_t stream);
uint32_t crt_render_resident_waves(int device, int kind, uint32_t ldsBytes);
hipError_t crt_launch_accumulate(const void* slab, void* acc, uint32_t tileFirst, uint32_t tileStride, uint32_t tileCount, uint32_t tilesX, uint32_t W, uint32_t frames, uint32_t passes,
    hipStream_t stream);
hipError_t crt_launch_find_nearest(const crt::Scene* sc, const void* rays, void* hits, uint32_t n, crt::Counters* counters, uint32_t ldsBytes, uint32_t* cursor, hipStream_t stream);
hipError_t crt_launch_is_occluded(const crt::Scene* sc, const void* rays, int32_t* occluded, uint32_t n, uint32_t ldsBytes, uint32_t* cursor, hipStream_t stream);
hipError_t crt_launch_whitted(const crt::Scene* sc, int accel, const crt::AltAccelDev* alt, const crt::TlasAltDev* tl, void* acc, uint32_t* pixels, crt::Counters* counters, uint32_t ldsBytes,
    hipStream_t stream);
size_t crt_whitted_inspect_work_bytes(uint32_t pixelCount);
hipError_t crt_launch_whitted_inspect(const crt::Scene* sc, int accel, const crt::AltAccelDev* alt, const crt::TlasAltDev* tl, int inspect, int32_t peakIn, void* acc, uint32_t* pixels,
    crt::Counters* counters, int32_t* trav, int32_t* tested, void* work, uint32_t ldsBytes, hipStream_t stream);
hipError_t crt_launch_resolve(const void* acc, uint32_t* pixels, float* tileSums, uint32_t tileFirst, uint32_t tileStride, uint32_t tileCount, uint32_t tilesX, uint32_t W, float scale,
    hipStream_t stream);
hipError_t crt_launch_commit_frame(const void* slabWindow, uint32_t frameInWindow, uint32_t passes, void* acc, uint32_t* pixels, float* tileSums, uint32_t tileFirst, uint32_t tileStride,
    uint32_t tileCount, uint32_t tilesX, uint32_t W, float scale, hipStream_t stream);

uint32_t crt_pool_streams(uint32_t frames);
size_t crt_pool_scratch_bytes_per_window(uint32_t tileCount);
hipError_t crt_launch_render_pool(const crt::Scene* sc, void* slab, void* facScratch, crt::Counters* counters, unsigned long long* tileClocks, const uint32_t* tileOrder, uint32_t tileFirst,
    uint32_t tileStride, uint32_t tileCount, uint32_t tilesX, uint32_t sppFirst, uint32_t frames, uint32_t passes, int collectStats, uint32_t rankFirst, uint32_t waveFrames,
    const uint32_t* waveTab, uint32_t tabBlocks, uint32_t longFrames, uint32_t* tileCost, unsigned long long* launchClk,
    const uint8_t* tileClass , uint32_t extraLds ,
    hipStream_t stream);
uint32_t crt_pool_lds_bytes(uint32_t stackDepth, uint32_t streams, uint32_t refBits );
uint32_t crt_pool_lds_limit(int device);
int crt_debug_pool_stamps(unsigned long long* out, int reset);
int crt_debug_pool_density(unsigned long long* out, int reset);
size_t crt_debug_pool_timeline(unsigned long long* out, size_t cap);

uint32_t crt_probe_paths(void);
hipError_t crt_launch_probe(const crt::Scene* sc, uint32_t tileFirst, uint32_t tileStride, uint32_t tileCount, uint32_t tilesX, uint32_t* tileCost, hipStream_t stream);
hipError_t crt_launch_render_alt(int accel, const crt::Scene* sc, const crt::AltAccelDev* acc, const crt::TlasAltDev* tl, void* slab, crt::Counters* counters, uint32_t tileFirst, uint32_t tileStride,
    uint32_t tileCount, uint32_t tilesX, uint32_t sppFirst, uint32_t frames, uint32_t passes, hipStream_t stream);
hipError_t crt_launch_sample_query(int accel, const crt::Scene* sc, const crt::AltAccelDev* acc, const crt::TlasAltDev* tl, const void* rays, uint32_t* seeds, float* rgb, uint32_t n,
    crt::Counters* counters, uint32_t* cursor, uint32_t* residentLanes, hipStream_t stream);

hipError_t crt_launch_find_nearest_prim(const crt::PrimDev* p, const void* rays, void* hits, uint32_t n, hipStream_t stream);
hipError_t crt_launch_render_prim(const crt::Scene* sc, const crt::PrimDev* p, void* slab, crt::Counters* counters, uint32_t tileFirst, uint32_t tileStride, uint32_t tileCount, uint32_t tilesX,
    uint32_t sppFirst, uint32_t frames, uint32_t passes, hipStream_t stream);
hipError_t crt_launch_sample_query_prim(const crt::Scene* sc, const crt::PrimDev* p, const void* rays, uint32_t* seeds, float* rgb, uint32_t n, crt::Counters* counters, uint32_t* cursor,
    uint32_t* residentLanes, hipStream_t stream);
hipError_t crt_launch_probe_f64(int op, const void* in, void* out, uint32_t n, hipStream_t stream);

hipError_t crt_launch_find_nearest_alt(int kind, const crt::Scene* sc, const crt::AltAccelDev* acc, const void* rays, void* hits, uint32_t n, uint32_t* cursor, hipStream_t stream);
hipError_t crt_launch_is_occluded_alt(int kind, const crt::Scene* sc, const crt::AltAccelDev* acc, const void* rays, int32_t* occluded, uint32_t n, uint32_t* cursor, hipStream_t stream);
hipError_t crt_launch_tlas_alt_query(int kind, bool occl, const crt::Scene* sc, const crt::TlasAltDev* tl, const void* rays, void* out, uint32_t n, uint32_t* cursor, hipStream_t stream);

hipError_t crt_launch_hit_info(const crt::Scene* sc, const void* rays, const void* hits, void* out, uint32_t n, uint32_t objects, uint32_t fileTris, hipStream_t stream);
hipError_t crt_launch_sky_color(const crt::Scene* sc, const void* rays, float* rgb, uint32_t n, hipStream_t stream);
hipError_t crt_launch_refit(char* geom, uint32_t leafOff, uint32_t pairBase, uint32_t triBase, uint32_t triCount, const float* pos, const void* plan, const uint32_t* levelOff, uint32_t levels,
    uint32_t rootCode, float* out, hipStream_t stream);
hipError_t crt_launch_probe_f32(int op, const void* in, void* out, uint32_t n, hipStream_t stream);

uint32_t crt_grid_build_blocks(int device);
size_t crt_grid_scan_chunks(uint32_t cells);
hipError_t crt_launch_grid_bounds(const float* pos, uint32_t triCount, crt::GridBuildState* state, uint32_t maxBlocks, hipStream_t stream);
hipError_t crt_launch_grid_count(const float* pos, uint32_t triCount, const crt::GridParams* g, uint32_t cells, uint32_t* counts, unsigned long long* chunkSums, crt::GridBuildState* state,
    uint32_t maxBlocks, hipStream_t stream);
hipError_t crt_launch_grid_fill(const float* pos, uint32_t triCount, const crt::GridParams* g, uint32_t cells, const uint32_t* cellStart, uint32_t* cursor, int32_t* unsorted, int32_t* refs,
    uint32_t total, const char* geom, uint32_t leafOff, uint32_t triBase, int globalIdx, crt::AltTri* tris, uint32_t maxBlocks, hipStream_t stream);

hipError_t crt_launch_tlas_build(const char* geom, uint32_t instOff, const float* T, const float* rootBox, uint32_t blasCount, uint32_t pairRel, uint32_t instRel, uint32_t poolRefBits,
    void* out, hipStream_t stream);

uint32_t crt_debug_query_grid(void);

}

namespace crt {

inline uint32_t bounded_query_grid(uint32_t grid) { const uint32_t k = crt_debug_query_grid(); return (k != 0u && k < grid) ? k : grid; }

inline uint32_t query_grid(uint32_t n, uint32_t ldsBytes)
{
    uint32_t perCu = ldsBytes ? (160u * 1024u) / ldsBytes : 16u; if (perCu > 16u) perCu = 16u; if (perCu < 4u) perCu = 4u;
    const uint32_t need = (n + 63u) / 64u, fill = 256u * perCu;
    return bounded_query_grid(need < fill ? need : fill);
}

inline bool query_launch_begin(uint32_t n, uint32_t* cursor, hipStream_t stream, hipError_t* status)
{
    *status = hipSuccess;
    if (n == 0) return false;
    if (!cursor) { *status = hipErrorInvalidValue; return false; }
    if (hipMemsetAsync(cursor, 0, 4, stream) != hipSuccess) { *status = hipGetLastError(); return false; }
    return true;
}

}
```

cpu-ray-tracer_amd/csrc/device/render_pool.hip:

```cpp
#include <type_traits>
#include "launch.h"
#include "sample_body.h"

namespace crt {

enum : uint32_t {
    F_OX = 0, F_OY, F_OZ, F_DX, F_DY, F_DZ,
    F_RX, F_RY, F_RZ,
    F_T,
    F_SEED, F_META,
    F_U, F_V,
    F_COUNT,
    F_CUR = F_U, F_PEND = F_V,
    F_TRI = F_RX
};
constexpr uint32_t kMetaItemMask = 0x7ffu, kMetaDepthShift = 11u, kMetaInside = 1u << 14, kMetaFresh = 1u << 15, kMetaObjShift = 16u, kMetaLowMask = 0xffffu;
constexpr uint32_t kQueueMask = 127u;

#ifndef CRT_POOL_MIN_WAVES
#define CRT_POOL_MIN_WAVES 4
#endif
#ifndef CRT_POOL_WIDE_MIN_WAVES
#define CRT_POOL_WIDE_MIN_WAVES 4
#endif
#ifndef CRT_POOL_NODE_STEPS
#define CRT_POOL_NODE_STEPS 2
#endif
#ifndef CRT_POOL_NODE2_MIN
#define CRT_POOL_NODE2_MIN 16
#endif
#ifndef CRT_POOL_STARVE
#define CRT_POOL_STARVE 40
#endif

#ifdef CRT_POOL_STAMPS
__device__ unsigned long long g_poolStamps[16];
#define CRT_PSTAMP(var) unsigned long long var; asm volatile("s_memtime %0\n\ts_waitcnt lgkmcnt(0)" : "=s"(var) :: "memory")
#define CRT_PACC(i, a, b) (pst[i] += (b) - (a))
#else
#define CRT_PSTAMP(var)
#define CRT_PACC(i, a, b)
#endif
#ifdef CRT_POOL_DENS
__device__ unsigned long long g_poolDens[48];
#define CRT_DENS(i, v) (dens[i] += (uint32_t)(v))
#define CRT_DENS_MASK(i, pred) (dens[i] += (uint32_t)__popcll(__builtin_amdgcn_ballot_w64(pred)))
#define CRT_LIVE_BUCKET(n) ((n) >= 112u ? 0u : (n) >= 96u ? 1u : (n) >= 64u ? 2u : 3u)
#else
#define CRT_DENS(i, v)
#define CRT_DENS_MASK(i, pred)
#endif
#ifdef CRT_POOL_TIMELINE
__device__ unsigned long long* g_poolTimeline = nullptr;
#endif
__device__ __forceinline__ bool lane_in(uint64_t m) { return __builtin_amdgcn_inverse_ballot_w64(m); }
__device__ __forceinline__ uint64_t finite3_mask(f3 v)
{
    const float inf = __builtin_inff();
    return __builtin_amdgcn_fcmpf(__builtin_fabsf(v.x), inf, 4) & __builtin_amdgcn_fcmpf(__builtin_fabsf(v.y), inf, 4) & __builtin_amdgcn_fcmpf(__builtin_fabsf(v.z), inf, 4);
}
#define CRT_CTL_SEQ() asm volatile("")
__device__ __forceinline__ bool ctl_free(uint64_t mRes) { CRT_CTL_SEQ(); return mRes != ~0ull; }
__device__ __forceinline__ uint32_t fresh(uint32_t x) { asm("" : "+s"(x)); return x; }
__device__ __forceinline__ uint32_t pop32(uint64_t m) { uint32_t n = (uint32_t)__builtin_popcountll(m); asm("" : "+s"(n)); return n; }
__device__ __forceinline__ uint64_t mask_ne(uint32_t a, uint32_t b) { return __builtin_amdgcn_uicmp(a, b, 33); }
__device__ __forceinline__ uint64_t mask_eq(uint32_t a, uint32_t b) { return __builtin_amdgcn_uicmp(a, b, 32); }
__device__ __forceinline__ uint64_t mask_ult(uint32_t a, uint32_t b) { return __builtin_amdgcn_uicmp(a, b, 36); }
__device__ __forceinline__ uint64_t mask_ule(uint32_t a, uint32_t b) { return __builtin_amdgcn_uicmp(a, b, 37); }
__device__ __forceinline__ uint64_t mask_sge(int a, int b) { return __builtin_amdgcn_sicmp(a, b, 39); }
__device__ __forceinline__ uint32_t rank_in(uint64_t m) { return __builtin_amdgcn_mbcnt_hi((uint32_t)(m >> 32), __builtin_amdgcn_mbcnt_lo((uint32_t)m, 0u)); }

template <int KIND, bool COUNT, int S, int REFBITS = 16>
__global__ __launch_bounds__(64, REFBITS == 32 ? CRT_POOL_WIDE_MIN_WAVES : CRT_POOL_MIN_WAVES) void render_pool_kernel(const Scene sc, float4* __restrict__ slab, float* __restrict__ facScratch, Counters* __restrict__ counters,
                                                             unsigned long long* __restrict__ tileClocks, const uint32_t* __restrict__ tileOrder,
                                                             uint32_t tileFirst, uint32_t tileStride, uint32_t tileCount, uint32_t tilesX,
                                                             uint32_t sppFirst, uint32_t frames, uint32_t passes, uint32_t groups, uint32_t waveFrames, const uint32_t* __restrict__ waveTab, uint32_t tabBlocks, uint32_t longFrames,
                                                             uint32_t rankFirst, uint32_t* __restrict__ tileCost, unsigned long long* __restrict__ launchClk, const uint8_t* __restrict__ tileClass)
{
    extern __shared__ uint32_t lds[];
    const uint32_t lane = threadIdx.x;
#ifdef CRT_POOL_TIMELINE
    const unsigned long long tl0 = wall_clock64();
#endif
    const unsigned long long clk0 = (COUNT || tileCost) ? wall_clock64() : 0ull;
    if (launchClk && lane == 0) { atomicMax(&launchClk[0], ~clk0); atomicMax(&launchClk[1], clk0); }
    uint32_t rank0, grp, wf = waveFrames, first = 0u, limit = frames;
    if (waveTab) {
        if (blockIdx.x < tabBlocks) {
            uint32_t lo = 0u, hi = tileCount - rankFirst;
            while (hi - lo > 1u) { const uint32_t mid = (lo + hi) >> 1; if (waveTab[2u * mid] <= blockIdx.x) lo = mid; else hi = mid; }
            rank0 = lo; grp = blockIdx.x - waveTab[2u * lo]; wf = waveTab[2u * lo + 1u]; limit = longFrames;
        } else { const uint32_t b = blockIdx.x - tabBlocks; rank0 = b / groups; grp = b - rank0 * groups; wf = (uint32_t)S; first = longFrames; }
    } else { rank0 = blockIdx.x / groups; grp = blockIdx.x - rank0 * groups; }
    const uint32_t rank = rank0 + rankFirst;
    if (rank >= tileCount) return;
    const uint32_t tl = tileOrder ? tileOrder[rank] : rank;
    const uint32_t frame0 = first + grp * wf;
    if (frame0 >= limit) return;
    const uint32_t nOwn = (limit - frame0 < wf) ? limit - frame0 : wf;
    const uint32_t nStreams = nOwn < (uint32_t)S ? nOwn : (uint32_t)S;
    const uint32_t tile = tileFirst + tl * tileStride;
    const uint32_t tx = tile % tilesX, ty = tile / tilesX;
    const uint32_t tcls = tileClass ? __builtin_amdgcn_readfirstlane((uint32_t)tileClass[tl]) : 0u;
    auto not_sky = [&]() -> bool { return fresh(tcls) != kTileSky; };
    const char* __restrict__ geom = sc.geom;
    float* __restrict__ fac = facScratch + (size_t)blockIdx.x * (15u * (uint32_t)S);

    constexpr PoolRefForm R = pool_ref_form((uint32_t)REFBITS);
    using StackEntry = std::conditional_t<REFBITS == 32, uint32_t, uint16_t>;
    constexpr uint32_t kEntryB = (uint32_t)sizeof(StackEntry), kLevelB = 64u * kEntryB;
    char* const ldsB = reinterpret_cast<char*>(lds);
    const uint32_t laneB = lane * kEntryB;
    uint32_t* st = lds + (sc.stackDepth + 1u) * (kLevelB / 4u);
    float* stf = reinterpret_cast<float*>(st);
    uint8_t* qEnd = reinterpret_cast<uint8_t*>(st + F_COUNT * S);
    uint8_t* qBnc = qEnd + 128, * qRdy = qEnd + 256;
    uint16_t* slotFrame = reinterpret_cast<uint16_t*>(qEnd + 384);
    auto stk_top = [&](uint32_t at) -> uint32_t { return *reinterpret_cast<const StackEntry*>(ldsB + at); };
    auto stk_put = [&](uint32_t at, uint32_t v) { *reinterpret_cast<StackEntry*>(ldsB + at) = (StackEntry)v; };

    Cnt cn; cn.rays = cn.primary = cn.interior = cn.leaf = cn.tri = cn.tlas = cn.visits = cn.meshhits = 0;
    uint32_t trips = 0;
#ifdef CRT_POOL_DENS
    uint32_t dens[48]; for (int i = 0; i < 48; i++) dens[i] = 0;
    uint32_t live = nStreams; unsigned long long liveClk = wall_clock64();
#endif
    const uint32_t items = 256u * passes;
    const uint32_t rowLen = 64u * passes;
    const f3 nil3 = mk3(0.0f, 0.0f, 0.0f);

    for (uint32_t s = lane; s < nStreams; s += 64u) {
        st[F_SEED * S + s] = init_seed(tx + ty * (uint32_t)sc.W + (sppFirst + (frame0 + s) * passes) * 1799u);
        st[F_META * S + s] = kMetaFresh;
        qEnd[s] = (uint8_t)s;
        if (S > 64) slotFrame[s] = (uint16_t)s;
    }
    uint32_t nLive = nStreams;
    uint32_t nextFrame = nStreams;
    uint32_t endH = 0, endT = nStreams, bncH = 0, bncT = 0, rdyH = 0, rdyT = 0;

    uint64_t mRes = 0ull;
    uint64_t mFinite = ~0ull;
    uint32_t sid = 0, cur = kRefDone, spB = laneB, metaLo = 0u;
    f3 tO = nil3, tD = nil3, trD = nil3;
    Hit h; h.t = 1e34f; h.u = 0; h.v = 0; h.objIdx = -1; h.triIdx = -1;
    rec4 q0 = {0, 0, 0, 0}, q1 = q0, q2 = q0, q3 = q0;

    auto new_ray = [&](auto primary, uint64_t mAct, uint32_t s, f3 v, bool norm, f3 O, uint32_t seed, uint32_t meta) {
        constexpr bool PRIM = decltype(primary)::value;
        const bool act = lane_in(mAct);
        const bool noLight = PRIM && (tcls & kTileNoLight) != 0u, noFloor = PRIM && (tcls & kTileNoFloor) != 0u, noTree = PRIM && (tcls & kTileNoTree) != 0u;
        f3 D = v, rD = v; Hit nh; nh.t = 1e34f; nh.u = 0; nh.v = 0; nh.objIdx = -1; nh.triIdx = -1;
        uint32_t ncur = kRefDone, pend = 0u;
        if (act) {
            const float inv = rcp_exact(sqrt_exact(dot3(v, v)));
            D = norm ? v * inv : v;
            cn.rays++;
            if (!PRIM || not_sky()) {
                rD = rcp_exact3(D);
                hit_light_floor<PRIM>(light_floor_from_kernarg<PRIM>(), O, D, nh, noLight, noFloor);
            }
            if (noTree) {
                if (COUNT) { if (KIND == 0) cn.interior++; else cn.tlas++; }
            } else if (sc.rootIsPair) {
                const kernarg_f rp = scene_floats(offsetof(Scene, rootPair));
                const rec4 a0 = {rp[0], rp[1], rp[2], rp[3]}, a1 = {rp[4], rp[5], rp[6], rp[7]};
                const rec4 b0 = {rp[8], rp[9], rp[10], rp[11]}, b1 = {rp[12], rp[13], rp[14], rp[15]};
                float d1, d2;
                const bool allFinite = (__builtin_amdgcn_ballot_w64(true) & ~finite3_mask(rD)) == 0ull;
                if constexpr (PRIM) {
                    const f3 ra0 = mk3(rp[16], rp[17], rp[18]), ra1 = mk3(rp[19], rp[20], rp[21]), rb0 = mk3(rp[22], rp[23], rp[24]), rb1 = mk3(rp[25], rp[26], rp[27]);
                    if (allFinite) { d1 = box_fast_rel(ra0, ra1, rD, nh.t); d2 = box_fast_rel(rb0, rb1, rD, nh.t); }
                    else { d1 = box_exact_rel(ra0, ra1, rD, nh.t); d2 = box_exact_rel(rb0, rb1, rD, nh.t); }
                } else if (allFinite) { d1 = box_fast(a0, a1, O, rD, nh.t); d2 = box_fast(b0, b1, O, rD, nh.t); }
                else { d1 = box_exact(a0, a1, O, rD, nh.t); d2 = box_exact(b0, b1, O, rD, nh.t); }
                const Ordered o = ordered_step(d1, d2, asu(a1.w), asu(b1.w));
                pend = o.push ? o.farRef : 0u;
                ncur = o.hitN ? o.nearRef : kRefDone;
                if (COUNT) { if (KIND == 0) cn.interior++; else cn.tlas++; }
            } else ncur = sc.rootRef16;
            if (COUNT && KIND == 0 && (ncur & R.tagMask) == 0u && ncur != kRefDone) cn.leaf++;
            if (!PRIM || not_sky()) {
                stf[F_OX * S + s] = O.x; stf[F_OY * S + s] = O.y; stf[F_OZ * S + s] = O.z;
                stf[F_RX * S + s] = rD.x; stf[F_RY * S + s] = rD.y; stf[F_RZ * S + s] = rD.z;
                stf[F_T * S + s] = nh.t;
                st[F_CUR * S + s] = ncur; st[F_PEND * S + s] = pend;
            }
            stf[F_DX * S + s] = D.x; stf[F_DY * S + s] = D.y; stf[F_DZ * S + s] = D.z;
            st[F_SEED * S + s] = seed; st[F_META * S + s] = meta | ((uint32_t)(nh.objIdx + 1) << kMetaObjShift);
        }
        uint64_t mW = 0ull, mE = mAct, mB = 0ull;
        if (!PRIM || not_sky()) {
            const uint32_t depth = (meta >> kMetaDepthShift) & 7u;
            mW = mAct & mask_ne(ncur, kRefDone);
            const uint64_t mStop = mask_ule((uint32_t)(nh.objIdx + 1), 1u) | mask_sge((int)depth, sc.depthLimit);
            mE = mAct & ~mW & mStop; mB = mAct & ~mW & ~mStop;
            if (lane_in(mW)) qRdy[(rdyT + rank_in(mW)) & kQueueMask] = (uint8_t)s;
            if (lane_in(mB)) qBnc[(bncT + rank_in(mB)) & kQueueMask] = (uint8_t)s;
            rdyT += (uint32_t)__popcll(mW); bncT += (uint32_t)__popcll(mB);
        }
        CRT_DENS(20, __popcll(mAct)); CRT_DENS(19, __popcll(mW));
        if (lane_in(mE)) qEnd[(endT + rank_in(mE)) & kQueueMask] = (uint8_t)s;
        endT += (uint32_t)__popcll(mE);
    };
    auto world_ray = [&]() {
        tO = mk3(stf[F_OX * S + sid], stf[F_OY * S + sid], stf[F_OZ * S + sid]);
        tD = mk3(stf[F_DX * S + sid], stf[F_DY * S + sid], stf[F_DZ * S + sid]);
        trD = mk3(stf[F_RX * S + sid], stf[F_RY * S + sid], stf[F_RZ * S + sid]);
    };

    uint64_t mNode2 = 0ull;
    auto node_step = [&](auto exactTag, uint64_t m) {
        constexpr bool allFinite = !decltype(exactTag)::value;
        if (lane_in(m)) {
            if (COUNT) { if (KIND == 1 && (cur & R.tlasBit) != 0u) cn.tlas++; else cn.interior++; }
            const uint32_t top = stk_top(spB);
            float d1, d2;
            if constexpr (allFinite) { d1 = box_fast(q0, q1, tO, trD, h.t); d2 = box_fast(q2, q3, tO, trD, h.t); }
            else { d1 = box_exact(q0, q1, tO, trD, h.t); d2 = box_exact(q2, q3, tO, trD, h.t); }
            const Ordered o = ordered_step(d1, d2, asu(q1.w), asu(q3.w));
            stk_put(spB + kLevelB, o.farRef);
            const bool pop = !o.hitN && spB != laneB;
            cur = o.hitN ? o.nearRef : (pop ? top : kRefDone);
            spB = spB + (o.push ? kLevelB : 0u) - (pop ? kLevelB : 0u);
            if (COUNT && (cur & R.tagMask) == 0u && cur != kRefDone) cn.leaf++;
        }
    };
    auto record_offset = [&]() -> uint32_t {
        const uint32_t idx = cur & R.indexMask;
        const bool inter = (cur & R.interior) != 0u;
        uint32_t oa = idx * (inter ? 64u : 48u) + (inter ? 0u : sc.leafOff - 48u);
        if (KIND == 1 && (cur & R.tlasBit) != 0u)
            oa = (cur & R.interior) ? sc.instOff + idx * 128u : sc.tlasPairOff + idx * 64u;
        return oa;
    };
    auto load_records = [&](uint64_t m) {
        const uint32_t oa = record_offset();
        if (lane_in(m)) { q0 = ldp<0>(geom, oa); q1 = ldp<1>(geom, oa); q2 = ldp<2>(geom, oa); q3 = ldp<3>(geom, oa); }
    };

    auto tri_step = [&](uint64_t m) {
        CRT_DENS(3, 1); CRT_DENS(4, __popcll(m));
        if (lane_in(m)) {
            if (COUNT) cn.tri++;
            const uint32_t top = stk_top(spB);
            hit_tri(q0, q1, q2, tO, tD, h);
            const bool more = asu(q2.w) > 1u;
            const bool pop = !more && spB != laneB;
            const uint32_t next = more ? cur + 1u : (pop ? top : kRefDone);
            spB -= pop ? kLevelB : 0u;
            if (COUNT && !more && (next & R.tagMask) == 0u && next != kRefDone) cn.leaf++;
            cur = next;
        }
    };

#ifdef CRT_POOL_STAMPS
    unsigned long long pst[12] = {0, 0, 0, 0, 0, 0, 0, 0, 0, 0, 0, 0};
#endif
    for (;;) {
        CRT_PSTAMP(p0);
        if (mRes != 0ull) {
            uint64_t mNode, mTlas = 0ull;
            if (KIND == 0) mNode = mRes & __builtin_amdgcn_ballot_w64(cur > R.interior - 1u);
            else { mTlas = mRes & __builtin_amdgcn_ballot_w64(cur >= R.tlasLeaf); mNode = mRes & __builtin_amdgcn_ballot_w64(cur - R.tlasBit < R.interior); }
            const uint64_t mTri = mRes & ~(mNode | mTlas);
            asm volatile("" : "+v"(q0), "+v"(q1), "+v"(q2), "+v"(q3));
            CRT_DENS(22, __popcll(mRes));
            if (mNode) { CRT_DENS(1, 1); CRT_DENS(2, __popcll(mNode)); }

            if (KIND == 1 && mTlas) { CRT_DENS(23, 1); CRT_DENS(24, __popcll(mTlas)); }
            uint64_t mBack = 0ull;
            if (KIND == 1 && mTlas != 0ull) {
                if (lane_in(mTlas)) {
                    if (COUNT) { cn.tlas++; cn.visits++; }
                    const f3 O = mk3(stf[F_OX * S + sid], stf[F_OY * S + sid], stf[F_OZ * S + sid]);
                    const f3 D = mk3(stf[F_DX * S + sid], stf[F_DY * S + sid], stf[F_DZ * S + sid]);
                    to_object_space(q0, q1, q2, O, D, tO, tD, trD);
                    spB += kLevelB; stk_put(spB, R.ret);
                    const uint32_t next = asu(q3.y);
                    if (COUNT && (next & R.tagMask) == 0u && next != kRefDone) cn.leaf++;
                    cur = next;
                }
                mFinite = (mFinite & ~mTlas) | (mTlas & finite3_mask(trD));
            }
            uint64_t mLeafNow = 0ull;
            auto node_phase = [&](auto exactTag) {
                if (mNode != 0ull) node_step(exactTag, mNode);
#if CRT_POOL_NODE_STEPS > 1
#pragma unroll
                for (int rep = 1; rep < CRT_POOL_NODE_STEPS; rep++) {
                    const uint64_t mStepped = rep == 1 ? mNode : mNode2;
                    mNode2 = mStepped & (KIND == 0 ? __builtin_amdgcn_ballot_w64(cur > R.interior - 1u) : __builtin_amdgcn_ballot_w64(cur - R.tlasBit < R.interior));
                    if (pop32(mNode2) < (uint32_t)CRT_POOL_NODE2_MIN) { mNode2 = 0ull; break; }
                    const uint64_t mLeaf = mStepped & __builtin_amdgcn_ballot_w64((cur & R.tagMask) == 0u) & ~__builtin_amdgcn_ballot_w64(cur == kRefDone);
                    load_records(mNode2 | mLeaf);
                    mLeafNow |= mLeaf;
                    CRT_DENS(28, 1); CRT_DENS(29, __popcll(mNode2));
                    node_step(exactTag, mNode2);
                }
#endif
            };
            if (mNode != 0ull) {
                uint64_t mInf = mNode & ~mFinite, mInf2 = mInf;
                asm("" : "+s"(mInf2));
                if (__builtin_expect(mInf == 0ull, 1)) node_phase(std::false_type{});
                if (__builtin_expect(mInf2 != 0ull, 0)) node_phase(std::true_type{});
            }
            const uint64_t mTriAll = mTri | mLeafNow;
            if (mTriAll != 0ull) tri_step(mTriAll);
            if (KIND == 1) {
                mBack = (mNode | mTriAll) & __builtin_amdgcn_ballot_w64(cur == R.ret);
                if (mBack != 0ull) {
                    if (lane_in(mBack)) {
                        world_ray();
                        const bool pop = spB != laneB;
                        const uint32_t top = stk_top(spB);
                        cur = pop ? top : kRefDone; spB -= pop ? kLevelB : 0u;
                        if (COUNT && (cur & R.tagMask) == 0u && cur != kRefDone) cn.leaf++;
                    }
                    mFinite = (mFinite & ~mBack) | (mBack & finite3_mask(trD));
                }
            }
            asm volatile("" ::: "memory");
            const uint64_t mFin = mRes & __builtin_amdgcn_ballot_w64(cur == kRefDone);
            if (mFin != 0ull) {
                CRT_DENS(5, 1); CRT_DENS(6, __popcll(mFin));
                const uint32_t depth = (metaLo >> kMetaDepthShift) & 7u;
                const uint64_t mStop = __builtin_amdgcn_ballot_w64((uint32_t)(h.objIdx + 1) <= 1u) | __builtin_amdgcn_ballot_w64((int)depth >= sc.depthLimit);
                const uint64_t mE = mFin & mStop, mB = mFin & ~mStop;
                if (lane_in(mFin)) {
                    stf[F_T * S + sid] = h.t; stf[F_U * S + sid] = h.u; stf[F_V * S + sid] = h.v;
                    st[F_TRI * S + sid] = (uint32_t)h.triIdx;
                    st[F_META * S + sid] = metaLo | ((uint32_t)(h.objIdx + 1) << kMetaObjShift);
                }
                if (lane_in(mE)) qEnd[(endT + rank_in(mE)) & kQueueMask] = (uint8_t)sid;
                if (lane_in(mB)) qBnc[(bncT + rank_in(mB)) & kQueueMask] = (uint8_t)sid;
                endT += (uint32_t)__popcll(mE); bncT += (uint32_t)__popcll(mB);
                mRes &= ~mFin;
            }
            asm volatile("" ::: "memory");
        }
        CRT_PSTAMP(p1); CRT_PACC(0, p0, p1);
        if (COUNT) trips++;
        CRT_DENS(0, 1);
#ifdef CRT_POOL_STAMPS
        pst[9]++;
#endif
#ifdef CRT_POOL_DENS
        dens[32u + CRT_LIVE_BUCKET(live)]++;
#endif
        {
            const uint32_t nRdy = rdyT - rdyH;
            const uint64_t mFree = ~mRes;
            if (nRdy != 0u) if (ctl_free(mRes)) {
                const uint32_t myRank = rank_in(mFree);
                const uint64_t mTake = mFree & __builtin_amdgcn_ballot_w64(myRank < nRdy);
                CRT_DENS(7, 1); CRT_DENS(8, __popcll(mTake));
                if (lane_in(mTake)) {
                    sid = qRdy[(rdyH + myRank) & kQueueMask];
                    tO = mk3(stf[F_OX * S + sid], stf[F_OY * S + sid], stf[F_OZ * S + sid]);
                    tD = mk3(stf[F_DX * S + sid], stf[F_DY * S + sid], stf[F_DZ * S + sid]);
                    trD = mk3(stf[F_RX * S + sid], stf[F_RY * S + sid], stf[F_RZ * S + sid]);
                    const uint32_t meta = st[F_META * S + sid];
                    h.t = stf[F_T * S + sid]; h.objIdx = (int)(meta >> kMetaObjShift) - 1; h.u = 0; h.v = 0; h.triIdx = -1;
                    metaLo = meta & kMetaLowMask;
                    cur = st[F_CUR * S + sid];
                    const uint32_t pend = st[F_PEND * S + sid];
                    stk_put(laneB + kLevelB, pend);
                    spB = laneB + (pend ? kLevelB : 0u);
                }
                mFinite = (mFinite & ~mTake) | (mTake & finite3_mask(trD));
                mRes |= mTake;
                rdyH += (uint32_t)__popcll(mTake);
            }
            if (mRes != 0ull) {
                CRT_DENS(21, 1);
                uint32_t oa = record_offset();
                if (!lane_in(mRes)) oa = 0u;
                q0 = ldp<0>(geom, oa); q1 = ldp<1>(geom, oa); q2 = ldp<2>(geom, oa); q3 = ldp<3>(geom, oa);
            }
        }
        asm volatile("" ::: "memory");
        const uint32_t nEnd = endT - endH, nBnc = bncT - bncH;
        uint32_t walking = pop32(mRes) + (rdyT - rdyH), fullest = nEnd | nBnc;
        asm("" : "+s"(walking));
        walking = fullest >= 64u ? 0u : walking;
        asm("" : "+s"(walking), "+s"(fullest));
        if (walking < (uint32_t)CRT_POOL_STARVE) {
            const uint32_t run = fullest >= 64u ? (nEnd >> 6) | ((nBnc >> 6) << 8) : (nEnd >= nBnc ? nEnd : nBnc << 8);
            const uint32_t runEnd = run & 0xffu, runBnc = run >> 8;

            CRT_PSTAMP(p2b); CRT_PACC(1, p1, p2b);
            if (runEnd != 0u) {
                const uint32_t n = nEnd < 64u ? nEnd : 64u;
                const uint64_t mActE = mask_ult(lane, n);
                const bool act = lane_in(mActE);
                const uint32_t s = act ? qEnd[(endH + lane) & kQueueMask] : 0u;
                endH += n;
                uint32_t meta = 0, seed = 0; int obj = -1; f3 D = nil3;
                if (act) { meta = st[F_META * S + s]; seed = st[F_SEED * S + s]; obj = (int)(meta >> kMetaObjShift) - 1; D = mk3(stf[F_DX * S + s], stf[F_DY * S + s], stf[F_DZ * S + s]); }
                const int depth = (int)((meta >> kMetaDepthShift) & 7u);
                uint32_t item = meta & kMetaItemMask;
                const uint64_t mFirst = mask_ne(meta & kMetaFresh, 0u), mEnded = mActE & ~mFirst, mMiss = mEnded & mask_eq(meta >> kMetaObjShift, 0u);
                const bool first = lane_in(mFirst), ended = lane_in(mEnded), miss = lane_in(mMiss);
#ifdef CRT_POOL_DENS
                dens[36u + CRT_LIVE_BUCKET(live)]++;
#endif
                CRT_DENS(9, 1); CRT_DENS(10, n); CRT_DENS_MASK(11, miss); CRT_DENS_MASK(13, act && first); CRT_DENS_MASK(25, ended && depth > 0); CRT_DENS_MASK(26, ended && depth > 1); CRT_DENS_MASK(27, ended && depth > 2);
                if (ended && obj >= 2) cn.meshhits++;
                float fk[15];
#pragma unroll
                for (int k = 0; k < 5; k++) {
                    fk[3 * k] = fk[3 * k + 1] = fk[3 * k + 2] = 0.0f;
                    if (not_sky()) if (ended && depth > k) {
#pragma unroll
                        for (int j = 0; j < 3; j++) fk[3 * k + j] = __hip_atomic_load(fac + (3 * k + j) * S + s, __ATOMIC_RELAXED, __HIP_MEMORY_SCOPE_AGENT);
                    }
                }
                uint32_t skyTexel = 0u;
                if (miss) {
                    float phi, theta; sky_angles(D, phi, theta);
                    const kernarg_f sk = scene_floats(offsetof(Scene, skyOffset));
                    skyTexel = sc.texels[tex_index(asu(sk[0]), (int)asu(sk[1]), (int)asu(sk[2]), phi * CRT_INV2PI, theta * CRT_INVPI)];
                }
                bool gen = act && first;
                size_t sampleAt = 0;
                if (ended) {
                    uint32_t pix = item, pass = 0;
                    if (fresh(passes) != 1u) { pix = item / passes; pass = item - pix * passes; }
                    const uint32_t fr = frame0 + (S > 64 ? (uint32_t)slotFrame[s] : s);
                    sampleAt = (((size_t)(fr >> 6) * tileCount + tl) * 256u + pix) * rowLen + ((fr & 63u) * passes + pass);
                    item++;
                    gen = item < items;
                }
                uint64_t mGen = mFirst | (mEnded & mask_ult(item, items));
                const uint64_t mDone = mEnded & ~mGen;
                if (mDone != 0ull) {
                    uint64_t mTake = 0ull;
                    if (S > 64) if (nextFrame < nOwn) {
                        const uint32_t f = nextFrame + rank_in(mDone);
                        mTake = mDone & mask_ult(f, nOwn);
                        if (lane_in(mTake)) {
                            slotFrame[s] = (uint16_t)f;
                            seed = init_seed(tx + ty * (uint32_t)sc.W + (sppFirst + (frame0 + f) * passes) * 1799u);
                            item = 0u;
                        }
                        nextFrame += pop32(mTake);
                        mGen |= mTake;
                    }
                    nLive -= pop32(mDone & ~mTake);
                }
                gen = lane_in(mGen);
#ifdef CRT_POOL_DENS
                {
                    const uint32_t gone = (uint32_t)__popcll(__builtin_amdgcn_ballot_w64(ended) & ~__builtin_amdgcn_ballot_w64(gen));
                    if (gone) { const unsigned long long now = wall_clock64(); dens[44u + CRT_LIVE_BUCKET(live)] += (uint32_t)(now - liveClk); liveClk = now; live -= gone; }
                }
#endif
                const kernarg_f cam = scene_floats(offsetof(Scene, camPos));
                const f3 camPos = mk3(cam[0], cam[1], cam[2]);
                f3 v = camPos;
                if (gen) {
                    const uint32_t pix = (fresh(passes) == 1u) ? item : item / passes;
                    const f3 TL = mk3(cam[3], cam[4], cam[5]);
                    constexpr size_t pc = (offsetof(Scene, primRight) - offsetof(Scene, camPos)) / 4;
                    const f3 right = mk3(cam[pc], cam[pc + 1], cam[pc + 2]), down = mk3(cam[pc + 3], cam[pc + 4], cam[pc + 5]);
                    v = primary_target(camPos, TL, right, down, cam[12], cam[13], tx, ty, pix, seed);
                    cn.primary++;
                }
                CRT_DENS_MASK(12, gen);
                CRT_PSTAMP(e1); CRT_PACC(2, p2b, e1);
                new_ray(std::true_type{}, mGen, s, v, true, camPos, seed, item);
                CRT_PSTAMP(e2); CRT_PACC(3, e1, e2);
                if (ended) {
                    f3 L = miss ? tex_unpack(skyTexel) : ((depth >= sc.depthLimit) ? mk3(0, 0, 0) : mk3(24, 24, 22));
                    if (not_sky()) {
#pragma unroll
                        for (int k = 4; k >= 0; k--)
                            if (depth > k) L = mk3(fk[3 * k], fk[3 * k + 1], fk[3 * k + 2]) * L;
                    }
                    slab[sampleAt] = make_float4(L.x, L.y, L.z, 0.0f);
                }
#ifdef CRT_POOL_STAMPS
                { CRT_PSTAMP(e3); CRT_PACC(4, e2, e3); pst[10]++; }
#endif
                asm volatile("" :: "v"(fk[0]), "v"(fk[1]), "v"(fk[2]), "v"(fk[3]), "v"(fk[4]), "v"(fk[5]), "v"(fk[6]), "v"(fk[7]), "v"(fk[8]), "v"(fk[9]), "v"(fk[10]), "v"(fk[11]), "v"(fk[12]), "v"(fk[13]), "v"(fk[14]), "v"(skyTexel));
            }
            CRT_PSTAMP(p3);
            asm volatile("" ::: "memory");
            if (runBnc != 0u) {
                const uint32_t n = nBnc < 64u ? nBnc : 64u;
                const uint64_t mActB = mask_ult(lane, n);
                const bool act = lane_in(mActB);
                const uint32_t s = act ? qBnc[(bncH + lane) & kQueueMask] : 0u;
                bncH += n;
                f3 O = nil3, D = nil3; float ht = 0, hu = 0, hv = 0; int obj = 1; uint32_t tri = 0, seed = 0, meta = 0;
                if (act) {
                    tri = st[F_TRI * S + s];
                    O = mk3(stf[F_OX * S + s], stf[F_OY * S + s], stf[F_OZ * S + s]);
                    D = mk3(stf[F_DX * S + s], stf[F_DY * S + s], stf[F_DZ * S + s]);
                    ht = stf[F_T * S + s]; hu = stf[F_U * S + s]; hv = stf[F_V * S + s];
                    seed = st[F_SEED * S + s]; meta = st[F_META * S + s]; obj = (int)(meta >> kMetaObjShift) - 1;
                }
                const bool mesh = act && obj >= 2;
#ifdef CRT_POOL_DENS
                dens[40u + CRT_LIVE_BUCKET(live)]++;
#endif
                CRT_DENS(14, 1); CRT_DENS(15, n); CRT_DENS_MASK(16, mesh);
                rec4 s0 = {0, 0, 0, 0}, s1 = s0, s2 = s0, s3 = s0;
                if (mesh) { const uint32_t so = sc.shadeOff + tri * 64u; s0 = ldp<0>(geom, so); s1 = ldp<1>(geom, so); s2 = ldp<2>(geom, so); s3 = ldp<3>(geom, so); cn.meshhits++; }
                const bool inside = (meta & kMetaInside) != 0u;
                const int depth = (int)((meta >> kMetaDepthShift) & 7u);
                const uint32_t item = meta & kMetaItemMask;
                f3 v = O; bool newInside = false;
                if (act) {
                    const f3 I = O + ht * D;
                    SurfPoint p;
                    if (obj == 1) {
                        const kernarg_f fl = scene_floats(offsetof(Scene, floorN));
                        const kernarg_f fm = scene_floats(offsetof(Scene, floorMat));
                        const rec4 m0 = {fm[0], fm[1], fm[2], fm[3]}, m1 = {fm[4], fm[5], fm[6], fm[7]};
                        p = floor_point(mk3(fl[0], fl[1], fl[2]), fl[4], m0, m1, I);
                    } else p = mesh_point<KIND>(s0, s1, s2, s3, hu, hv, obj, geom, sc.instOff, sc.mats);
                    const f3 N = face_ray(p.N, D);
                    uint32_t texel = 0x00ffffffu;
                    if (p.tW > 0) texel = sc.texels[tex_index(p.tOff, p.tW, p.tH, p.tu, p.tv)];
                    const f3 medium = medium_of(inside, p.absorb, ht);
                    CRT_PSTAMP(b1); CRT_PACC(5, p3, b1);
                    const Bounce b = draw_bounce(seed, D, N, inside, p.refl, p.refr);
                    newInside = b.newInside;
                    const f3 c = (p.tW > 0) ? tex_unpack(texel) : mk3(1.0f, 1.0f, 1.0f);
                    CRT_PSTAMP(b2); CRT_PACC(6, b1, b2);
                    const float inv = rcp_exact(sqrt_exact(dot3(b.v, b.v)));
                    const f3 nv = b.branch == kDiffuse ? b.v * inv : b.v;
                    v = nv;
                    const f3 factor = bounce_factor(b.branch, c, medium, nv, N);
                    float* fd = fac + (3 * depth) * S + s;
                    __hip_atomic_store(fd, factor.x, __ATOMIC_RELAXED, __HIP_MEMORY_SCOPE_AGENT);
                    __hip_atomic_store(fd + S, factor.y, __ATOMIC_RELAXED, __HIP_MEMORY_SCOPE_AGENT);
                    __hip_atomic_store(fd + 2 * S, factor.z, __ATOMIC_RELAXED, __HIP_MEMORY_SCOPE_AGENT);
                    O = I + nv * CRT_EPS;
                    CRT_PSTAMP(b3); CRT_PACC(7, b2, b3);
                }
                CRT_PSTAMP(b4);
                new_ray(std::false_type{}, mActB, s, v, false, O, seed, item | ((uint32_t)(depth + 1) << kMetaDepthShift) | (newInside ? kMetaInside : 0u));
#ifdef CRT_POOL_STAMPS
                { CRT_PSTAMP(b5); CRT_PACC(8, b4, b5); pst[11]++; }
#endif
                asm volatile("" :: "v"(s0), "v"(s1), "v"(s2), "v"(s3));
            }
        }
        if (nLive == 0u) break;
    }
#ifdef CRT_POOL_STAMPS
    if (lane == 0) for (int i = 0; i < 12; i++) atomicAdd(&g_poolStamps[i], pst[i]);
#endif
#ifdef CRT_POOL_DENS
    dens[44u + CRT_LIVE_BUCKET(live)] += (uint32_t)(wall_clock64() - liveClk);
    if (lane == 0) for (int i = 0; i < 48; i++) if (dens[i]) atomicAdd(&g_poolDens[i], (unsigned long long)dens[i]);
#endif

#ifdef CRT_POOL_TIMELINE
    if (lane == 0 && g_poolTimeline) { uint32_t hw; asm volatile("s_getreg_b32 %0, hwreg(HW_REG_HW_ID)" : "=s"(hw)); g_poolTimeline[3 * (size_t)blockIdx.x] = tl0; g_poolTimeline[3 * (size_t)blockIdx.x + 1] = wall_clock64(); g_poolTimeline[3 * (size_t)blockIdx.x + 2] = hw; }
#endif
    if (tileCost && lane == 0 && nOwn == (uint32_t)S) atomicMax(&tileCost[tl], (uint32_t)((wall_clock64() - clk0) * 64ull / (uint32_t)S));
    if (launchClk && lane == 0) { const unsigned long long now = wall_clock64(), last = __hip_atomic_load(&launchClk[1], __ATOMIC_RELAXED, __HIP_MEMORY_SCOPE_AGENT), from = last > clk0 ? last : clk0; if (now > from) atomicAdd(&launchClk[2], now - from); }
    if (COUNT && tileClocks && lane == 0 && nOwn == frames) {
        tileClocks[2 * tl] = wall_clock64() - clk0;
        tileClocks[2 * tl + 1] = trips;
    }
    uint32_t vals[8] = {cn.rays, cn.primary, cn.interior, cn.leaf, cn.tri, cn.tlas, cn.visits, cn.meshhits};
#pragma unroll
    for (int i = 0; i < 8; i++) {
        if (!COUNT && i >= 2 && i != 7) continue;
        uint32_t sum = wave_sum(vals[i]);
        if (lane == 0 && sum) atomicAdd(&counters->v[i], (unsigned long long)sum);
    }
}

}

#ifndef CRT_POOL_STREAMS
#define CRT_POOL_STREAMS 128
#endif
extern "C" uint32_t crt_pool_streams(uint32_t frames) { return frames > 64u ? (uint32_t)CRT_POOL_STREAMS : 64u; }
extern "C" uint32_t crt_pool_lds_bytes(uint32_t stackDepth, uint32_t streams, uint32_t refBits) { return (stackDepth + 1u) * 64u * (refBits / 8u) + crt::F_COUNT * streams * 4u + 3u * 128u + (streams > 64u ? 2u * streams : 0u); }
extern "C" uint32_t crt_pool_lds_limit(int device)
{
    static uint32_t known[64] = {};
    if (device >= 0 && device < 64 && known[device]) return known[device];
    int v = 0;
    if (hipDeviceGetAttribute(&v, hipDeviceAttributeMaxSharedMemoryPerBlock, device) != hipSuccess || v <= 0) { (void)hipGetLastError(); return 0u; }
    const uint32_t limit = (uint32_t)v < 64u * 1024u ? (uint32_t)v : 64u * 1024u;
    if (device >= 0 && device < 64) known[device] = limit;
    return limit;
}
extern "C" size_t crt_pool_scratch_bytes_per_window(uint32_t tileCount) { return (size_t)tileCount * 128u * 15u * 4u; }

#ifdef CRT_POOL_STAMPS
extern "C" int crt_debug_pool_stamps(unsigned long long* out, int reset)
{
    if (out && hipMemcpyFromSymbol(out, HIP_SYMBOL(crt::g_poolStamps), 128) != hipSuccess) return -1;
    if (reset) { unsigned long long z[16] = {}; if (hipMemcpyToSymbol(HIP_SYMBOL(crt::g_poolStamps), z, 128) != hipSuccess) return -1; }
    return 0;
}
#endif
#ifdef CRT_POOL_DENS
extern "C" int crt_debug_pool_density(unsigned long long* out, int reset)
{
    if (out && hipMemcpyFromSymbol(out, HIP_SYMBOL(crt::g_poolDens), 384) != hipSuccess) return -1;
    if (reset) { unsigned long long z[48] = {}; if (hipMemcpyToSymbol(HIP_SYMBOL(crt::g_poolDens), z, 384) != hipSuccess) return -1; }
    return 0;
}
#endif
#ifdef CRT_POOL_TIMELINE
static unsigned long long* g_timelineHost = nullptr; static size_t g_timelineCount = 0;
extern "C" size_t crt_debug_pool_timeline(unsigned long long* out, size_t cap)
{
    const size_t n = g_timelineCount < cap ? g_timelineCount : cap;
    if (out && n) (void)hipMemcpy(out, g_timelineHost, n * 24, hipMemcpyDeviceToHost);
    return g_timelineCount;
}
#endif
extern "C" hipError_t crt_launch_render_pool(const crt::Scene* sc, void* slab, void* facScratch, crt::Counters* counters, unsigned long long* tileClocks, const uint32_t* tileOrder,
                                             uint32_t tileFirst, uint32_t tileStride, uint32_t tileCount, uint32_t tilesX, uint32_t sppFirst,
                                             uint32_t frames, uint32_t passes, int collectStats, uint32_t rankFirst, uint32_t waveFrames, const uint32_t* waveTab, uint32_t tabBlocks, uint32_t longFrames,
                                             uint32_t* tileCost, unsigned long long* launchClk, const uint8_t* tileClass, uint32_t extraLds, hipStream_t stream)
{
    if (tileCount == 0 || frames == 0) return hipSuccess;
    if (sc->poolRefBits != 16u && sc->poolRefBits != 32u) return hipErrorInvalidValue;
    const uint32_t S = crt_pool_streams(frames);
    const uint32_t wf = (S == 64u || waveFrames < S) ? S : waveFrames;
    if (wf % S != 0u || wf > 0xff80u) return hipErrorInvalidValue;
    if (S == 64u) waveTab = nullptr;
    if (waveTab && (tabBlocks == 0u || longFrames == 0u || longFrames > frames)) return hipErrorInvalidValue;
    const uint32_t groups = waveTab ? (frames - longFrames + S - 1u) / S : (frames + wf - 1u) / wf;
    if ((unsigned long long)tileCount * ((frames + S - 1u) / S) > 0x7fffffffull) return hipErrorInvalidValue;
    if (rankFirst >= tileCount) return hipSuccess;
    dim3 grid(waveTab ? tabBlocks + (tileCount - rankFirst) * groups : (tileCount - rankFirst) * groups), block(64);
#ifdef CRT_POOL_TIMELINE
    { static unsigned long long* buf = nullptr; static size_t cap = 0;
      if (cap < (size_t)grid.x) { if (buf) (void)hipFree(buf); (void)hipMalloc((void**)&buf, (size_t)grid.x * 24); cap = grid.x; (void)hipMemcpyToSymbol(HIP_SYMBOL(crt::g_poolTimeline), &buf, sizeof(buf)); }
      (void)hipMemsetAsync(buf, 0, (size_t)grid.x * 24, stream); g_timelineHost = buf; g_timelineCount = grid.x; }
#endif
    const uint32_t ldsBytes = crt_pool_lds_bytes(sc->stackDepth, S, sc->poolRefBits) + extraLds;
    { int dev = 0; if (hipGetDevice(&dev) != hipSuccess) return hipGetLastError(); if (ldsBytes > crt_pool_lds_limit(dev)) return hipErrorInvalidValue; }
#define CRT_LAUNCH(K, C, SS) do { if (sc->poolRefBits == 32u) CRT_LAUNCH_R(K, C, SS, 32); else CRT_LAUNCH_R(K, C, SS, 16); } while (0)
#define CRT_LAUNCH_R(K, C, SS, RB) hipLaunchKernelGGL((crt::render_pool_kernel<K, C, SS, RB>), grid, block, ldsBytes, stream, *sc, (float4*)slab, (float*)facScratch, counters, tileClocks, tileOrder, tileFirst, tileStride, tileCount, tilesX, sppFirst, frames, passes, groups, wf, waveTab, tabBlocks, longFrames, rankFirst, tileCost, launchClk, tileClass)
#define CRT_LAUNCH_S(K, C) do { if (S == 64u) CRT_LAUNCH(K, C, 64); else CRT_LAUNCH(K, C, CRT_POOL_STREAMS); } while (0)
    if (sc->kind == 0) { if (collectStats) CRT_LAUNCH_S(0, true); else CRT_LAUNCH_S(0, false); }
    else { if (collectStats) CRT_LAUNCH_S(1, true); else CRT_LAUNCH_S(1, false); }
#undef CRT_LAUNCH_S
#undef CRT_LAUNCH
#undef CRT_LAUNCH_R
    return hipGetLastError();
}
```

cpu-ray-tracer_amd/csrc/device/sample_body.h:

```cpp
#pragma once
#include "dev_common.h"

namespace crt {

struct SurfPoint { f3 N; float tu, tv, refl, refr; f3 absorb; uint32_t tOff; int tW, tH, mat; };

__device__ __forceinline__ void set_material(SurfPoint& p, rec4 m0, rec4 m1)
{
    p.refl = m0.x; p.refr = m0.y; p.absorb = mk3(m0.z, m0.w, m1.x);
    p.tOff = asu(m1.y); p.tW = (int)asu(m1.z); p.tH = (int)asu(m1.w);
}
__device__ __forceinline__ SurfPoint floor_point(f3 floorN, float floorInvto, rec4 m0, rec4 m1, f3 I)
{
    SurfPoint p; p.N = floorN; p.tu = 0; p.tv = 0; p.mat = 1;
    if (floorN.y == 1) {
        float u = I.x, v = I.z;
        u *= floorInvto; v *= floorInvto;
        p.tu = u - __builtin_floorf(u); p.tv = v - __builtin_floorf(v);
    }
    set_material(p, m0, m1);
    return p;
}
__device__ __forceinline__ SurfPoint floor_point(f3 floorN, float floorInvto, const Material& m, f3 I)
{
    const rec4 m0 = {m.reflectivity, m.refractivity, m.absorption[0], m.absorption[1]}, m1 = {m.absorption[2], asf(m.texOffset), asf((uint32_t)m.texW), asf((uint32_t)m.texH)};
    return floor_point(floorN, floorInvto, m0, m1, I);
}
template <int KIND>
__device__ __forceinline__ SurfPoint mesh_point(rec4 s0, rec4 s1, rec4 s2, rec4 s3, float u, float v, int objIdx, const char* __restrict__ geom, uint32_t instOff, const Material* __restrict__ mats)
{
    SurfPoint p;
    const f3 n0 = mk3(s0.x, s0.y, s0.z), n1 = mk3(s0.w, s1.x, s1.y), n2 = mk3(s1.z, s1.w, s2.x);
    const float w = 1 - u - v;
    const f3 Nn = w * n0 + u * n1 + v * n2;
    p.tu = w * s2.y + u * s2.w + v * s3.y;
    p.tv = w * s2.z + u * s3.x + v * s3.z;
    p.mat = (int)asu(s3.w);
    const rec4* mp = reinterpret_cast<const rec4*>(mats + p.mat);
    set_material(p, mp[0], mp[1]);
    if (KIND == 0) p.N = normalize3(Nn);
    else {
        const uint32_t io = instOff + (uint32_t)(objIdx - 2) * 128u + 64u;
        const rec4 r0 = ldp<0>(geom, io), r1 = ldp<1>(geom, io), r2 = ldp<2>(geom, io);
        p.N = normalize3(mk3(r0.x * Nn.x + r0.y * Nn.y + r0.z * Nn.z + r0.w * 0.0f,
                             r1.x * Nn.x + r1.y * Nn.y + r1.z * Nn.z + r1.w * 0.0f,
                             r2.x * Nn.x + r2.y * Nn.y + r2.z * Nn.z + r2.w * 0.0f));
    }
    return p;
}
__device__ __forceinline__ f3 face_ray(f3 N, f3 D) { return (dot3(N, D) > 0) ? -N : N; }

__device__ __forceinline__ f3 medium_of(bool inside, f3 absorb, float t)
{
    f3 medium = mk3(1, 1, 1);
    if (inside) {
        const f3 ab = absorb * -t;
        medium = mk3(crt_expf(ab.x), crt_expf(ab.y), crt_expf(ab.z));
    }
    return medium;
}
enum Branch : int { kMirror, kDielectric, kDiffuse };
struct Bounce { f3 v; Branch branch; bool newInside; };
__device__ __forceinline__ Bounce draw_bounce(uint32_t& seed, f3 D, f3 N, bool inside, float refl, float refr)
{
    Bounce b; b.newInside = false;
    const float r = rnd(seed);
    if (r < refl) {
        b.v = D - 2.0f * N * dot3(N, D); b.branch = kMirror;
    } else if (r < refl + refr) {
        b.v = D - 2.0f * N * dot3(N, D); b.branch = kDielectric;
        const float n1 = inside ? 1.2f : 1, n2 = inside ? 1 : 1.2f;
        const float eta = n1 / n2, cosi = dot3(-D, N);
        const float cost2 = 1.0f - eta * eta * (1 - cosi * cosi);
        if (cost2 > 0) {
            const float a = n1 - n2, b2 = n1 + n2, R0 = (a * a) / (b2 * b2), cc = 1 - cosi;
            const float Fr = R0 + (1 - R0) * (cc * cc * cc * cc * cc);
            const f3 T = eta * D + ((eta * cosi - sqrt_exact(__builtin_fabsf(cost2))) * N);
            if (rnd(seed) > Fr) { b.v = T; b.newInside = !inside; }
        }
    } else {
        f3 Rr;
        do {
            const float rz = rnd_pm1(seed);
            const float ry = rnd_pm1(seed);
            const float rx = rnd_pm1(seed);
            Rr = mk3(rx, ry, rz);
        } while (dot3(Rr, Rr) > 1);
        if (dot3(Rr, N) < 0) Rr = Rr * -1.0f;
        b.v = Rr; b.branch = kDiffuse;
    }
    return b;
}
__device__ __forceinline__ f3 bounce_factor(Branch branch, f3 c, f3 medium, f3 nv, f3 N)
{
    if (branch != kDiffuse) return c * medium;
    const f3 brdf = c * CRT_INVPI;
    return medium * brdf * 2.0f * CRT_PI * dot3(nv, N);
}
__device__ __forceinline__ void sample_unwind(const float* fst, int depth, f3& L)
{
#pragma unroll
    for (int k = 4; k >= 0; k--)
        if (depth > k) { const float* fd = fst + (uint32_t)(3 * k) * 64u; L = mk3(fd[0], fd[64], fd[128]) * L; }
}

__device__ __forceinline__ f3 primary_target(f3 camPos, f3 TL, f3 right, f3 down, float invW, float invH, uint32_t tx, uint32_t ty, uint32_t pix, uint32_t& seed)
{
    const int x = (int)(tx * 16u + (pix & 15u)), y = (int)(ty * 16u + (pix >> 4));
    const float jy = rnd(seed);
    const float jx = rnd(seed);
    const float u = ((float)x + jx) * invW, vv = ((float)y + jy) * invH;
    const f3 P = TL + u * right + vv * down;
    return P - camPos;
}
template <bool PRIM>
__device__ __forceinline__ LightFloor light_floor_from_kernarg()
{
    const kernarg_f lp = scene_floats(offsetof(Scene, lightInvT));
    const kernarg_f ax = scene_floats(offsetof(Scene, lightAxis));
    LightFloor lf;
#pragma unroll
    for (int i = 0; i < 12; i++) lf.lightInvT[i] = lp[i];
    lf.lightSize = lp[15]; lf.floorN[0] = lp[19]; lf.floorN[1] = lp[20]; lf.floorN[2] = lp[21]; lf.floorD = lp[22];
    lf.lightAxis = asu(ax[0]); lf.floorAxisY = asu(ax[1]);
    lf.preOy = lf.preOx = lf.preOz = lf.preNum = 0.0f;
    if constexpr (PRIM) {
        constexpr size_t pl = (offsetof(Scene, primLight) - offsetof(Scene, lightInvT)) / 4;
        lf.preOy = lp[pl]; lf.preOx = lp[pl + 1]; lf.preOz = lp[pl + 2]; lf.preNum = lp[pl + 3];
    }
    return lf;
}

struct Ordered { uint32_t nearRef, farRef; bool hitN, push; };
__device__ __forceinline__ Ordered ordered_step(float d1, float d2, uint32_t refA, uint32_t refB)
{
    const bool sw = d1 > d2;
    const float dn = sw ? d2 : d1, df = sw ? d1 : d2;
    Ordered o;
    o.nearRef = sw ? refB : refA; o.farRef = sw ? refA : refB;
    o.hitN = dn != 1e30f; o.push = o.hitN && df != 1e30f;
    return o;
}

}
```

Measured before the change: 32450 Mrays/s.

## Render all-sky tiles in a dedicated lightweight kernel behind the pool launch

Adds a specialized sky kernel that, for tiles classified as sky-only, generates primary rays and looks up the environment texture directly, with no BVH traversal or pool machinery. Sky tiles are moved to the tail of the tile order, removed from the pool launch range, and their measured launch time is folded into the job and wave planning. The aim is to stop spending pool wavefronts and scheduler state on trivially cheap tiles and to rebalance the pool's long tail. It adds planning complexity and an extra launch, and relies on the host-side tile classification being exact.

After: 33340 Mrays/s (median of 6 runs). 1.03x the previous value.

```diff
diff --git a/cpu-ray-tracer_amd/csrc/abi.cpp b/cpu-ray-tracer_amd/csrc/abi.cpp
--- a/cpu-ray-tracer_amd/csrc/abi.cpp
+++ b/cpu-ray-tracer_amd/csrc/abi.cpp
@@ -64,6 +64,7 @@
     uint64_t tickEpoch = 0; uint32_t tickNextSpp = 0, tickPasses = 0;
     uint32_t aheadFrames = 0;
     hipStream_t aheadStream = nullptr;
+    hipStream_t skyStream = nullptr;
     crt::Scene hScene{};
     crt::Counters* dCounters = nullptr;
     uint32_t* dQueryCursor = nullptr;
@@ -77,6 +78,7 @@
     bool classDirty = true;
     uint8_t* dTileClass = nullptr;
     uint8_t* hTileClass[2] = {nullptr, nullptr}; hipEvent_t classCopied[2] = {nullptr, nullptr}; int classFlip = 0;
+    std::vector<uint8_t> hostClass; uint32_t skyTiles = 0, skyLaunches = 0; double skyWindowTicks = 0;
     bool haveScene = false;
     struct Flat { int32_t kind = 0; uint64_t leafOff = 0, tlasOff = 0, tlasPairOff = 0, instOff = 0, shadeOff = 0; uint32_t tlasNodeCount = 0, maxHeight = 0;
                   uint32_t objects = 0;
@@ -138,7 +140,7 @@
     std::vector<uint32_t> jobCost;
     std::vector<uint32_t> jobOrder;
     uint32_t* dJobDesc = nullptr; uint32_t* hJobDesc = nullptr; uint32_t jobDescCap = 0, jobBlocks = 0, jobHead = 0; hipEvent_t jobDescReady = nullptr;
-    uint32_t planWindows = 0, planFrames = 0; bool planPool = false, planValid = false;
+    uint32_t planWindows = 0, planFrames = 0, planSky = 0, planSkyAsked = 0; bool planPool = false, planValid = false;
     double jobTrialMs[2] = {0, 0};
     uint32_t jobWaveOff = 0, jobWaveBlocks = 0, jobLongFrames = 0, jobLongWaves = 0, lastLongWaves = 0;
     std::vector<hipEvent_t> splitEvents;
@@ -358,6 +360,7 @@
     for (hipEvent_t e : c->retiredEvents) (void)hipEventDestroy(e);
     for (auto& a : c->ahead) (void)hipEventDestroy(a.end);
     if (c->aheadStream) (void)hipStreamDestroy(c->aheadStream);
+    if (c->skyStream) (void)hipStreamDestroy(c->skyStream);
     for (auto& ev : c->evPool) { (void)hipEventDestroy(ev.a); (void)hipEventDestroy(ev.b); }
     for (auto& ev : c->evRender) { (void)hipEventDestroy(ev.a); (void)hipEventDestroy(ev.b); }
     for (auto& ev : c->evAcc) { (void)hipEventDestroy(ev.a); (void)hipEventDestroy(ev.b); }
@@ -911,6 +914,13 @@
     return 0;
 }
 
+static uint32_t sky_to_tail(const std::vector<uint8_t>& cls, std::vector<uint32_t>& order)
+{
+    if (cls.size() != order.size()) return 0u;
+    const auto tail = std::stable_partition(order.begin(), order.end(), [&](uint32_t i) { return cls[i] != crt::kTileSky; });
+    return (uint32_t)(order.end() - tail);
+}
+
 static int update_tile_order(crt_ctx* c)
 {
     if (!c->orderDirty || c->tileCount == 0) return 0;
@@ -951,7 +961,8 @@
     for (int k = 0; k <= crt_ctx::kLatStages; k++) { c->tuneCount[k] = 0; c->tuneMs[k] = 0; }
     c->latStage = 0; c->latBest = 0; c->latDone = false; c->latWarm = false; c->latConfirming = false; c->latQueue.clear(); c->costPending = false; c->latProbed = false;
     first.insert(first.end(), rest.begin(), rest.end());
-    c->jobCostValid = false; c->jobCostPending = false; c->planValid = false;
+    (void)sky_to_tail(c->hostClass, first);
+    c->jobCostValid = false; c->jobCostPending = false; c->planValid = false; c->skyWindowTicks = 0;
     { const int r = upload_tile_order(c, first); if (r) return r; }
     c->orderDirty = false;
     return 0;
@@ -968,6 +979,13 @@
         HIPCK(c, ensure_event(&c->classCopied[k]));
     } else HIPCK(c, hipEventSynchronize(c->classCopied[k]));
     crt::classify_tiles(c->hScene, c->cfg.width, c->cfg.height, (uint32_t)c->tilesX, c->tileFirst, c->tileStride, c->tileCount, c->hTileClass[k]);
+    {
+        const uint8_t* cls = c->hTileClass[k];
+        bool same = c->hostClass.size() == c->tileCount; uint32_t sky = 0;
+        for (uint32_t i = 0; i < c->tileCount; i++) { const bool s = cls[i] == crt::kTileSky; sky += s ? 1u : 0u; if (same && s != (c->hostClass[i] == crt::kTileSky)) same = false; }
+        c->hostClass.assign(cls, cls + c->tileCount); c->skyTiles = sky;
+        if (!same) c->orderDirty = true;
+    }
     HIPCK(c, hipMemcpyAsync(c->dTileClass, c->hTileClass[k], (size_t)c->tileCount, hipMemcpyHostToDevice, c->stream));
     HIPCK(c, hipEventRecord(c->classCopied[k], c->stream));
     c->orderReady = c->classCopied[k];
@@ -1244,8 +1262,24 @@
 }
 
 static size_t job_cost_clk_offset(const crt_ctx* c) { return (((size_t)c->tileCount + 1u) & ~(size_t)1u) * 4u; }
-static size_t job_cost_bytes(const crt_ctx* c) { return job_cost_clk_offset(c) + 24u; }
-
+static size_t job_cost_bytes(const crt_ctx* c) { return job_cost_clk_offset(c) + 40u; }
+
+static bool sky_behind() { const char* e = hook("CRT_SKY_PLACEMENT"); return !(e && !strcmp(e, "ahead")); }
+static uint32_t sky_split(const crt_ctx* c, bool pool)
+{
+    if (!pool || c->cfg.collectStats || c->classDirty || !c->dTileClass || c->hostClass.size() != c->tileCount) return 0u;
+    if (hook("CRT_DEBUG_NO_TILE_CLASS") || hook("CRT_DEBUG_NO_SKY_KERNEL")) return 0u;
+    if (hook("CRT_POOL_WAVE_FRAMES")) return 0u;
+    return c->skyTiles;
+}
+
+static uint32_t job_order(const std::vector<uint32_t>& cost, const std::vector<uint8_t>& cls, std::vector<uint32_t>& order)
+{
+    order.resize(cost.size());
+    for (uint32_t i = 0; i < (uint32_t)cost.size(); i++) order[i] = i;
+    std::stable_sort(order.begin(), order.end(), [&](uint32_t a, uint32_t b) { return cost[a] > cost[b]; });
+    return sky_to_tail(cls, order);
+}
 static int adopt_job_costs(crt_ctx* c)
 {
     const uint32_t n = c->tileCount;
@@ -1258,18 +1292,22 @@
         if (c->recWindows && (double)c->recWaves >= 1.5 * (double)c->recResident && s0 > 0) c->poolWindowTicks = (s0 + drain) / (double)c->recWindows / (c->recPool ? 1.0 : 1.2);
         if (hook("CRT_LAT_VERBOSE")) fprintf(stderr, "[crt] measured %u windows with %s: %u wavefronts, last one started %.2f ms after the first, then %.2f ms of drain -> %.3f ms of machine time per window under the pool\n", c->recWindows, c->recPool ? "the pool" : "one stream per lane", c->recWaves, s0 * 1e-5, drain * 1e-5, c->poolWindowTicks * 1e-5);
     }
-    c->jobOrder.resize(n);
-    for (uint32_t i = 0; i < n; i++) c->jobOrder[i] = i;
-    std::stable_sort(c->jobOrder.begin(), c->jobOrder.end(), [&](uint32_t a, uint32_t b) { return c->jobCost[a] > c->jobCost[b]; });
+    {
+        const unsigned long long* clk = reinterpret_cast<const unsigned long long*>(reinterpret_cast<const char*>(c->hJobCost) + job_cost_clk_offset(c)) + 3;
+        c->skyWindowTicks = (c->recWindows && clk[0] && clk[1] > ~clk[0]) ? (double)(clk[1] - ~clk[0]) / (double)c->recWindows : 0.0;
+        if (hook("CRT_LAT_VERBOSE")) fprintf(stderr, "[crt] the sky launch of the measuring job: %.3f ms per window\n", c->skyWindowTicks * 1e-5);
+    }
+    job_order(c->jobCost, c->hostClass, c->jobOrder);
     c->jobCostValid = true; c->planValid = false;
     return upload_tile_order(c, c->jobOrder);
 }
 
-static void plan_job(const crt_ctx* c, uint32_t windows, uint32_t frames, bool pool, std::vector<uint32_t>& table, uint32_t* head)
+static void plan_job(const crt_ctx* c, uint32_t windows, uint32_t frames, bool pool, std::vector<uint32_t>& table, uint32_t* head, uint32_t nSky = 0u, double skyTicks = 0.0)
 {
     table.clear(); *head = 0;
-    const uint32_t n = c->tileCount;
-    if (!c->jobCostValid || windows < 2u || windows > 64u || n > 0x10000u || c->cfg.collectStats || hook("CRT_SPLIT_OFF")) return;
+    if (nSky >= c->tileCount) return;
+    const uint32_t n = c->tileCount - nSky;
+    if (!c->jobCostValid || windows < 2u || windows > 64u || c->tileCount > 0x10000u || c->cfg.collectStats || hook("CRT_SPLIT_OFF")) return;
     if (pool && c->streams.size() < 2) return;
     if (const char* e = hook("CRT_SPLIT_FORCE")) {
         const uint32_t h = std::min<uint32_t>((uint32_t)atoi(e), pool ? n - 1u : n);
@@ -1288,7 +1326,8 @@
         int k = 1; while (k < 6 && kLatG[k] * v > T) k++;
         *cls = 2 + k; return K * (64.0 / kLatLanes[k]) * kLatG[k] * v / narrowSlots;
     };
-    auto machine = [&](double T) { double m = 0; int cls; for (uint32_t v : c->jobCost) m += cheapest((double)v, T, &cls); return m; };
+    std::vector<uint8_t> planned(c->tileCount, 0); for (uint32_t r = 0; r < n; r++) planned[c->jobOrder[r]] = 1;
+    auto machine = [&](double T) { double m = 0; int cls; for (uint32_t i = 0; i < c->tileCount; i++) if (planned[i]) m += cheapest((double)c->jobCost[i], T, &cls); return m + skyTicks; };
     const double top = (double)c->jobCost[c->jobOrder[0]];
     double lo = top * kLatG[6], hi = std::max(poolLong * top, machine(1e30)) * 1.01;
     if (machine(lo) <= lo) hi = lo;
@@ -1315,7 +1354,7 @@
     *head = pool ? h : 0u;
 }
 
-struct PoolWaveTerms { double poolLong = 2.4, load = 1.0, safety = 1.0, guard = 12.0, share = 1.0; };
+struct PoolWaveTerms { double poolLong = 2.4, load = 1.0, safety = 1.0, guard = 12.0, share = 1.0, tailTicks = 0.0, tailWaves = 0.0; };
 static uint64_t pool_wave_plan(const uint32_t* cost, uint32_t nr, uint32_t frames, uint32_t S, double perCost, double startTicks, uint32_t resident, const PoolWaveTerms& tm,
                                std::vector<uint32_t>& wf, uint32_t* longFrames, std::vector<double>* start, double* aimOut)
 {
@@ -1329,9 +1368,10 @@
     double aim = startTicks, m = startTicks;
     std::vector<double> st(nr);
     for (uint32_t r = 0; r < nr; r++) { st[r] = m; m += (double)(F1 / 64u) * (double)cost[r] * perCost; aim += (double)((frames + 63u) / 64u) * (double)cost[r] * perCost; }
+    aim += tm.tailTicks;
     if (start) *start = st;
     if (aimOut) *aimOut = aim;
-    if ((double)plain < tm.guard * (double)resident) return plain;
+    if ((double)plain + tm.tailWaves < tm.guard * (double)resident) return plain;
     const uint64_t shortWaves = (uint64_t)nr * ((frames - F1 + S - 1u) / S);
     for (int kMax = 3; kMax >= 1; kMax--) {
         uint64_t waves = shortWaves; bool any = false;
@@ -1342,7 +1382,7 @@
             waves += F1 / wf[r];
         }
         if (!any) break;
-        if ((double)waves >= tm.guard * (double)resident) { *longFrames = F1; return waves; }
+        if ((double)waves + tm.tailWaves >= tm.guard * (double)resident) { *longFrames = F1; return waves; }
     }
     wf.assign(nr, S);
     return plain;
@@ -1374,39 +1414,64 @@
     return (uint32_t)std::min<long>(v, 8192) / S * S;
 }
 
+struct PoolWavePlan { uint32_t off = 0, blocks = 0, longFrames = 0, longWaves = 0, ranks = 0; double aim = 0; };
+static PoolWavePlan plan_pool_waves(const crt_ctx* c, uint32_t windows, uint32_t frames, uint32_t head, uint32_t nSky, double skyTicks, std::vector<uint32_t>& table)
+{
+    PoolWavePlan p;
+    PoolWaveTerms terms;
+    const uint32_t S = crt_pool_streams(frames);
+    if (!c->jobCostValid || c->cfg.collectStats || head + nSky >= c->tileCount || !pool_wave_terms(terms) || forced_wave_frames(S)) return p;
+    const uint32_t nr = c->tileCount - nSky - head;
+    p.ranks = nr;
+    std::vector<uint32_t> cost(nr), wf, tab;
+    double costSum = 0; for (uint32_t v : c->jobCost) costSum += (double)v;
+    const double perCost = (c->poolWindowTicks > 0 && costSum > 0) ? c->poolWindowTicks / costSum : 1.0 / 4096.0;
+    double startTicks = 0;
+    if (sky_behind()) { terms.tailTicks = skyTicks; terms.tailWaves = (double)nSky * (double)((frames + S - 1u) / S); } else startTicks = skyTicks;
+    for (uint32_t r = 0; r < head; r++) startTicks += (double)windows * 1.2 * (double)c->jobCost[c->jobOrder[r]] * perCost;
+    for (uint32_t r = 0; r < nr; r++) cost[r] = c->jobCost[c->jobOrder[head + r]];
+    uint32_t F1 = 0, lw = 0, blocks = 0;
+    pool_wave_plan(cost.data(), nr, frames, S, perCost, startTicks, 4096u, terms, wf, &F1, nullptr, &p.aim);
+    if (F1) blocks = pool_wave_table(wf, F1, S, tab, &lw);
+    if (lw) {
+        for (uint32_t r = 0; r < nSky; r++) { tab.push_back(blocks); tab.push_back(S); }
+        p.off = (uint32_t)table.size(); p.blocks = blocks; p.longFrames = F1; p.longWaves = lw;
+        table.insert(table.end(), tab.begin(), tab.end());
+    }
+    if (hook("CRT_LAT_VERBOSE")) {
+        uint32_t cnt[4] = {0, 0, 0, 0}; double share[4] = {0, 0, 0, 0}, sum = 0;
+        for (uint32_t r = 0; r < nr; r++) { int k = 0; while ((S << k) < wf[r]) k++; cnt[k]++; share[k] += cost[r]; sum += cost[r]; }
+        fprintf(stderr, "[crt] pool launch of %u ranks x %u frames (%u sky ranks behind them: %.2f ms): aim %.1f ms, most expensive tile %.2f ms, long part %u frames in %u wavefronts, %u of them own more than %u frames (safety %.2f, guard %.1f x 4096, share %.2f); tiles by frames per wavefront (share of the cost):",
+                nr, frames, nSky, skyTicks * 1e-5, p.aim * 1e-5, nr ? cost[0] * 1e-5 : 0.0, F1, blocks, lw, S, terms.safety, terms.guard, terms.share);
+        for (int k = 0; k < 4; k++) fprintf(stderr, " %u: %u (%.3f)", S << k, cnt[k], sum > 0 ? share[k] / sum : 0.0);
+        fprintf(stderr, "\n");
+    }
+    return p;
+}
+
+static double sky_launch_ticks(const crt_ctx* c, uint32_t windows, uint32_t nSky)
+{
+    return (nSky && c->jobCostValid) ? c->skyWindowTicks * (double)windows : 0.0;
+}
+
 static int install_job_plan(crt_ctx* c, uint32_t windows, uint32_t frames, bool pool)
 {
-    if (c->planValid && c->planWindows == windows && c->planFrames == frames && c->planPool == pool) return 0;
+    const uint32_t asked = sky_split(c, pool);
+    if (c->planValid && c->planWindows == windows && c->planFrames == frames && c->planPool == pool && c->planSkyAsked == asked) return 0;
+    uint32_t nSky = asked;
+    double skyTicks = sky_launch_ticks(c, windows, nSky);
     std::vector<uint32_t> table; uint32_t head = 0;
-    plan_job(c, windows, frames, pool, table, &head);
-    c->planValid = true; c->planWindows = windows; c->planFrames = frames; c->planPool = pool; c->jobHead = head; c->jobBlocks = (uint32_t)table.size();
+    plan_job(c, windows, frames, pool, table, &head, nSky, skyTicks);
+    if (head && nSky) {
+        nSky = 0; skyTicks = 0;
+        plan_job(c, windows, frames, pool, table, &head);
+    }
+    c->planValid = true; c->planWindows = windows; c->planFrames = frames; c->planPool = pool; c->planSkyAsked = asked; c->planSky = nSky; c->jobHead = head; c->jobBlocks = (uint32_t)table.size();
     c->jobTrialMs[0] = c->jobTrialMs[1] = 0;
     c->jobWaveOff = c->jobWaveBlocks = c->jobLongFrames = c->jobLongWaves = 0;
-    PoolWaveTerms terms;
-    const uint32_t S = crt_pool_streams(frames);
-    if (pool && c->jobCostValid && !c->cfg.collectStats && head < c->tileCount && pool_wave_terms(terms) && !forced_wave_frames(S)) {
-        const uint32_t nr = c->tileCount - head;
-        std::vector<uint32_t> cost(nr), wf, tab;
-        double costSum = 0; for (uint32_t v : c->jobCost) costSum += (double)v;
-        const double perCost = (c->poolWindowTicks > 0 && costSum > 0) ? c->poolWindowTicks / costSum : 1.0 / 4096.0;
-        double startTicks = 0;
-        for (uint32_t r = 0; r < head; r++) startTicks += (double)windows * 1.2 * (double)c->jobCost[c->jobOrder[r]] * perCost;
-        for (uint32_t r = 0; r < nr; r++) cost[r] = c->jobCost[c->jobOrder[head + r]];
-        double aim = 0; uint32_t F1 = 0, lw = 0, blocks = 0;
-        pool_wave_plan(cost.data(), nr, frames, S, perCost, startTicks, 4096u, terms, wf, &F1, nullptr, &aim);
-        if (F1) blocks = pool_wave_table(wf, F1, S, tab, &lw);
-        if (lw) {
-            c->jobWaveOff = (uint32_t)table.size(); c->jobWaveBlocks = blocks; c->jobLongFrames = F1; c->jobLongWaves = lw;
-            table.insert(table.end(), tab.begin(), tab.end());
-        }
-        if (hook("CRT_LAT_VERBOSE")) {
-            uint32_t cnt[4] = {0, 0, 0, 0}; double share[4] = {0, 0, 0, 0}, sum = 0;
-            for (uint32_t r = 0; r < nr; r++) { int k = 0; while ((S << k) < wf[r]) k++; cnt[k]++; share[k] += cost[r]; sum += cost[r]; }
-            fprintf(stderr, "[crt] pool launch of %u ranks x %u frames: aim %.1f ms, most expensive tile %.2f ms, long part %u frames in %u wavefronts, %u of them own more than %u frames (safety %.2f, guard %.1f x 4096, share %.2f); tiles by frames per wavefront (share of the cost):",
-                    nr, frames, aim * 1e-5, nr ? cost[0] * 1e-5 : 0.0, F1, blocks, lw, S, terms.safety, terms.guard, terms.share);
-            for (int k = 0; k < 4; k++) fprintf(stderr, " %u: %u (%.3f)", S << k, cnt[k], sum > 0 ? share[k] / sum : 0.0);
-            fprintf(stderr, "\n");
-        }
+    if (pool) {
+        const PoolWavePlan p = plan_pool_waves(c, windows, frames, head, nSky, skyTicks, table);
+        c->jobWaveOff = p.off; c->jobWaveBlocks = p.blocks; c->jobLongFrames = p.longFrames; c->jobLongWaves = p.longWaves;
     }
     if (table.empty()) return 0;
     if (c->jobDescCap < table.size()) {
@@ -1432,6 +1497,7 @@
     bool wantCost = false, wantJobCost = false, pool = false;
     uint32_t head = 0, jobBlocks = 0; unsigned long long* jobClk = nullptr;
     uint32_t waveFrames = 0, waveBlocks = 0, longFrames = 0, longWaves = 0; const uint32_t* waveTab = nullptr;
+    uint32_t sky = 0;
 };
 
 static int next_block_table(crt_ctx* c);
@@ -1480,6 +1546,7 @@
     const bool poolByDefault = c->hScene.poolRefBits == 16u || c->poolMinWaves == 0;
     const uint64_t minWaves = c->poolMinWaves != 65000u ? c->poolMinWaves : (c->jobCostValid ? 43000u : 65000u);
     L.pool = c->usePool && poolByDefault && pool_can_run(c, L.nf) && (uint64_t)c->tileCount * L.windows >= minWaves && (c->poolMinWaves == 0 || L.nf > 64u);
+    L.sky = sky_split(c, L.pool);
     if (L.nf > 64u && c->jobCostValid) {
         if ((r = install_job_plan(c, L.windows, L.nf, L.pool))) return r;
         int use = 1;
@@ -1488,18 +1555,19 @@
             else if (c->jobTrialMs[1] > 0 && c->jobTrialMs[0] == 0) use = 0;
             c->evRender.back().mode = 100 + use;
         }
+        if (use) L.sky = c->planSky;
         if (use) { L.head = c->jobHead; L.jobBlocks = c->jobBlocks; if (L.pool && c->jobLongWaves) { L.waveTab = c->dJobDesc + c->jobWaveOff; L.waveBlocks = c->jobWaveBlocks; L.longFrames = c->jobLongFrames; L.longWaves = c->jobLongWaves; } }
     }
     if (L.pool) if (const uint32_t S = crt_pool_streams(L.nf); const uint32_t n = forced_wave_frames(S)) {
         L.waveFrames = n; L.waveTab = nullptr; L.waveBlocks = 0;
-        L.longWaves = n > S ? (c->tileCount - L.head) * (L.nf / n + ((L.nf % n) > S ? 1u : 0u)) : 0u;
+        L.longWaves = n > S ? (c->tileCount - L.sky - L.head) * (L.nf / n + ((L.nf % n) > S ? 1u : 0u)) : 0u;
     }
     if (L.jobBlocks || L.waveTab) HIPCK(c, hipStreamWaitEvent(L.st, c->jobDescReady, 0));
     if (L.wantJobCost) {
         L.jobClk = reinterpret_cast<unsigned long long*>(reinterpret_cast<char*>(c->dJobCost) + job_cost_clk_offset(c));
         c->recPool = L.pool; c->recWindows = L.windows;
         const uint32_t perWave = L.pool ? std::max(crt_pool_streams(L.nf), L.waveFrames) : 64u;
-        c->recWaves = L.pool ? c->tileCount * ((L.nf + perWave - 1u) / perWave) : c->tileCount * L.windows;
+        c->recWaves = L.pool ? (c->tileCount - L.sky) * ((L.nf + perWave - 1u) / perWave) : c->tileCount * L.windows;
         c->recResident = L.pool ? 4096u : 5120u;
         if (L.pool && c->hScene.poolRefBits == 32u)
             c->recResident = 256u * std::min(16u, (160u * 1024u) / std::max(1u, pool_lds_need(c, L.nf)));
@@ -1525,6 +1593,13 @@
     if (L.pool) {
         void* scratch = (char*)L.slab + (size_t)L.windows * sample_bytes_per_window(c, L.passes);
         hipStream_t st2 = st;
+        const bool skyBehind = sky_behind();
+        auto launch_sky = [&](hipStream_t s) -> hipError_t {
+            return crt_launch_render_sky(&c->hScene, L.slab, c->dCounters, c->dTileOrder, c->tileCount - L.sky, L.sky, c->tileFirst, c->tileStride, c->tileCount, (uint32_t)c->tilesX,
+                                         L.sppFirst, L.nf, L.passes, L.jobClk ? L.jobClk + 3 : nullptr, s);
+        };
+        if (L.sky && !skyBehind) { le = launch_sky(st); if (le == hipSuccess) c->skyLaunches++; }
+        if (le != hipSuccess) return le;
         if (L.jobBlocks) {
             le = launch_table(c->dJobDesc, L.jobBlocks, nullptr);
             st2 = c->streams[(size_t)(c->launchSeq++ % c->streams.size())];
@@ -1532,11 +1607,24 @@
         }
         if (le == hipSuccess)
             le = crt_launch_render_pool(&c->hScene, L.slab, scratch, c->dCounters, c->dTileClocks, c->dTileOrder, c->tileFirst, c->tileStride, c->tileCount, (uint32_t)c->tilesX,
-                                        L.sppFirst, L.nf, L.passes, c->cfg.collectStats, L.jobBlocks ? L.head : 0u, L.waveFrames, L.waveTab, L.waveBlocks, L.longFrames,
+                                        L.sppFirst, L.nf, L.passes, c->cfg.collectStats, L.jobBlocks ? L.head : 0u, c->tileCount - L.sky, L.waveFrames, L.waveTab, L.waveBlocks, L.longFrames,
                                         L.wantJobCost ? c->dJobCost : nullptr, L.jobClk,
                                         (c->classDirty || hook("CRT_DEBUG_NO_TILE_CLASS")) ? nullptr : c->dTileClass , c->extraLds, st2);
         if (le == hipSuccess) c->lastLongWaves = L.longWaves;
         if (L.jobBlocks && le == hipSuccess) le = join(st2);
+        if (L.sky && skyBehind && le == hipSuccess) {
+            if (!c->skyStream && !hook("CRT_SKY_PRIORITY")) {
+                int least = 0, greatest = 0;
+                le = hipDeviceGetStreamPriorityRange(&least, &greatest);
+                if (le == hipSuccess) le = hipStreamCreateWithPriority(&c->skyStream, hipStreamNonBlocking, least);
+                if (le != hipSuccess) return le;
+            }
+            hipStream_t st3 = c->skyStream;
+            if (hook("CRT_SKY_PRIORITY")) { st3 = c->streams[(size_t)(c->launchSeq++ % c->streams.size())]; if (st3 == st2 && c->streams.size() > 1) st3 = c->streams[(size_t)(c->launchSeq++ % c->streams.size())]; }
+            if (st3 != st) le = hipStreamWaitEvent(st3, L.ev.a, 0);
+            if (le == hipSuccess) le = launch_sky(st3);
+            if (le == hipSuccess) { c->skyLaunches++; le = join(st3); }
+        }
     } else if (L.jobBlocks) {
         le = launch_table(c->dJobDesc, L.jobBlocks, nullptr);
     } else if (L.blockDesc && L.nBlocks) {
@@ -1600,7 +1688,7 @@
     if (le != hipSuccess) {
         return c->hip(le, pool ? "launch of render_pool_kernel" : "launch of render_tiles_kernel");
     }
-    if (pool) c->poolLaunches++;
+    if (pool && L.sky < c->tileCount) c->poolLaunches++;
     HIPCK(c, hipEventRecord(ev.b, st));
     pairGuard.armed = false;
     c->lastRenderEnd = ev.b;
@@ -1646,8 +1734,8 @@
     HIPCK(c, hipSetDevice(c->cfg.device));
     { int r = discard_ahead(c); if (r) return r; }
     if (c->tileCount == 0 || frames == 0) return CRT_OK;
+    { int r = update_tile_class(c); if (r) return r; }
     { int r = update_tile_order(c); if (r) return r; }
-    { int r = update_tile_class(c); if (r) return r; }
     if (c->streams.empty()) {
         int n = c->cfg.renderStreams;
         if (n <= 0) n = 7;
@@ -2893,6 +2981,45 @@
     if (start) memcpy(start, st.data(), (size_t)nr * 8);
     return (long long)waves;
 }
+extern "C" int crt_debug_sky_split(const uint32_t* cost, const uint8_t* cls, uint32_t n, uint32_t windows, uint32_t frames, double poolWindowTicks, double skyWindowTicks,
+                                   uint32_t* order, uint32_t* skyFirst, uint32_t* head, uint32_t* planRanks, uint32_t* waveTab, uint32_t* tabBlocks, uint32_t* longFrames)
+{
+    if (!cls || !n || !order || !skyFirst || !head || !planRanks || !waveTab || !tabBlocks || !longFrames) return CRT_ERR_INVALID;
+    crt_ctx c;
+    c.tileCount = n; c.poolWindowTicks = poolWindowTicks; c.skyWindowTicks = skyWindowTicks;
+    c.hostClass.assign(cls, cls + n);
+    *head = *planRanks = *tabBlocks = *longFrames = 0;
+    if (!cost) {
+        c.jobOrder.resize(n); for (uint32_t i = 0; i < n; i++) c.jobOrder[i] = i;
+        c.skyTiles = sky_to_tail(c.hostClass, c.jobOrder);
+    } else {
+        c.jobCost.assign(cost, cost + n); c.jobCostValid = true;
+        c.skyTiles = job_order(c.jobCost, c.hostClass, c.jobOrder);
+        c.streams.assign(2, nullptr);
+        const double skyTicks = c.skyTiles ? skyWindowTicks * (double)windows : 0.0;
+        std::vector<uint32_t> table;
+        plan_job(&c, windows, frames, true, table, head, c.skyTiles, skyTicks);
+        table.clear();
+        const PoolWavePlan p = plan_pool_waves(&c, windows, frames, *head, c.skyTiles, skyTicks, table);
+        c.streams.clear();
+        *planRanks = p.ranks; *tabBlocks = p.blocks; *longFrames = p.longFrames;
+        if (table.size() > 2u * (size_t)n) return CRT_ERR_INVALID;
+        memcpy(waveTab, table.data(), table.size() * 4);
+    }
+    memcpy(order, c.jobOrder.data(), (size_t)n * 4);
+    *skyFirst = n - c.skyTiles;
+    return (int)c.skyTiles;
+}
+extern "C" int crt_debug_sky_launches(crt_ctx* c) { return c ? (int)c->skyLaunches : -1; }
+extern "C" int crt_debug_job_costs(crt_ctx* c, uint32_t* out, double* poolWindowTicks, double* skyWindowTicks)
+{
+    if (!c || !out) return CRT_ERR_INVALID;
+    if (!c->jobCostValid || c->jobCost.size() != c->tileCount) return CRT_ERR_STATE;
+    memcpy(out, c->jobCost.data(), (size_t)c->tileCount * 4);
+    if (poolWindowTicks) *poolWindowTicks = c->poolWindowTicks;
+    if (skyWindowTicks) *skyWindowTicks = c->skyWindowTicks;
+    return CRT_OK;
+}
 extern "C" int crt_debug_pool_long_waves(crt_ctx* c) { return c ? (int)c->lastLongWaves : -1; }
 extern "C" void crt_debug_pool_wave_terms(double* out) { const PoolWaveTerms tm; out[0] = tm.poolLong; out[1] = tm.load; out[2] = tm.safety; out[3] = tm.guard; out[4] = tm.share; }
 
diff --git a/cpu-ray-tracer_amd/csrc/device/launch.h b/cpu-ray-tracer_amd/csrc/device/launch.h
--- a/cpu-ray-tracer_amd/csrc/device/launch.h
+++ b/cpu-ray-tracer_amd/csrc/device/launch.h
@@ -28,8 +28,9 @@
 uint32_t crt_pool_streams(uint32_t frames);
 size_t crt_pool_scratch_bytes_per_window(uint32_t tileCount);
 hipError_t crt_launch_render_pool(const crt::Scene* sc, void* slab, void* facScratch, crt::Counters* counters, unsigned long long* tileClocks, const uint32_t* tileOrder, uint32_t tileFirst,
-    uint32_t tileStride, uint32_t tileCount, uint32_t tilesX, uint32_t sppFirst, uint32_t frames, uint32_t passes, int collectStats, uint32_t rankFirst, uint32_t waveFrames,
-    const uint32_t* waveTab, uint32_t tabBlocks, uint32_t longFrames, uint32_t* tileCost, unsigned long long* launchClk,
+    uint32_t tileStride, uint32_t tileCount, uint32_t tilesX, uint32_t sppFirst, uint32_t frames, uint32_t passes, int collectStats, uint32_t rankFirst,
+    uint32_t rankEnd , uint32_t waveFrames,
+    const uint32_t* waveTab , uint32_t tabBlocks, uint32_t longFrames, uint32_t* tileCost, unsigned long long* launchClk,
     const uint8_t* tileClass , uint32_t extraLds ,
     hipStream_t stream);
 uint32_t crt_pool_lds_bytes(uint32_t stackDepth, uint32_t streams, uint32_t refBits );
@@ -37,6 +38,10 @@
 int crt_debug_pool_stamps(unsigned long long* out, int reset);
 int crt_debug_pool_density(unsigned long long* out, int reset);
 size_t crt_debug_pool_timeline(unsigned long long* out, size_t cap);
+
+hipError_t crt_launch_render_sky(const crt::Scene* sc, void* slab, crt::Counters* counters, const uint32_t* tileOrder, uint32_t rankFirst, uint32_t skyTiles, uint32_t tileFirst,
+    uint32_t tileStride, uint32_t tileCount , uint32_t tilesX, uint32_t sppFirst, uint32_t frames, uint32_t passes,
+    unsigned long long* launchClk , hipStream_t stream);
 
 uint32_t crt_probe_paths(void);
 hipError_t crt_launch_probe(const crt::Scene* sc, uint32_t tileFirst, uint32_t tileStride, uint32_t tileCount, uint32_t tilesX, uint32_t* tileCost, hipStream_t stream);
diff --git a/cpu-ray-tracer_amd/csrc/device/render_pool.hip b/cpu-ray-tracer_amd/csrc/device/render_pool.hip
--- a/cpu-ray-tracer_amd/csrc/device/render_pool.hip
+++ b/cpu-ray-tracer_amd/csrc/device/render_pool.hip
@@ -130,7 +130,7 @@
     const f3 nil3 = mk3(0.0f, 0.0f, 0.0f);
 
     for (uint32_t s = lane; s < nStreams; s += 64u) {
-        st[F_SEED * S + s] = init_seed(tx + ty * (uint32_t)sc.W + (sppFirst + (frame0 + s) * passes) * 1799u);
+        st[F_SEED * S + s] = stream_seed(tx, ty, (uint32_t)sc.W, sppFirst, frame0 + s, passes);
         st[F_META * S + s] = kMetaFresh;
         qEnd[s] = (uint8_t)s;
         if (S > 64) slotFrame[s] = (uint16_t)s;
@@ -429,7 +429,7 @@
                     uint32_t pix = item, pass = 0;
                     if (fresh(passes) != 1u) { pix = item / passes; pass = item - pix * passes; }
                     const uint32_t fr = frame0 + (S > 64 ? (uint32_t)slotFrame[s] : s);
-                    sampleAt = (((size_t)(fr >> 6) * tileCount + tl) * 256u + pix) * rowLen + ((fr & 63u) * passes + pass);
+                    sampleAt = slab_position(fr, tileCount, tl, pix, rowLen, passes, pass);
                     item++;
                     gen = item < items;
                 }
@@ -442,7 +442,7 @@
                         mTake = mDone & mask_ult(f, nOwn);
                         if (lane_in(mTake)) {
                             slotFrame[s] = (uint16_t)f;
-                            seed = init_seed(tx + ty * (uint32_t)sc.W + (sppFirst + (frame0 + f) * passes) * 1799u);
+                            seed = stream_seed(tx, ty, (uint32_t)sc.W, sppFirst, frame0 + f, passes);
                             item = 0u;
                         }
                         nextFrame += pop32(mTake);
@@ -624,7 +624,7 @@
 #endif
 extern "C" hipError_t crt_launch_render_pool(const crt::Scene* sc, void* slab, void* facScratch, crt::Counters* counters, unsigned long long* tileClocks, const uint32_t* tileOrder,
                                              uint32_t tileFirst, uint32_t tileStride, uint32_t tileCount, uint32_t tilesX, uint32_t sppFirst,
-                                             uint32_t frames, uint32_t passes, int collectStats, uint32_t rankFirst, uint32_t waveFrames, const uint32_t* waveTab, uint32_t tabBlocks, uint32_t longFrames,
+                                             uint32_t frames, uint32_t passes, int collectStats, uint32_t rankFirst, uint32_t rankEnd, uint32_t waveFrames, const uint32_t* waveTab, uint32_t tabBlocks, uint32_t longFrames,
                                              uint32_t* tileCost, unsigned long long* launchClk, const uint8_t* tileClass, uint32_t extraLds, hipStream_t stream)
 {
     if (tileCount == 0 || frames == 0) return hipSuccess;
@@ -636,8 +636,9 @@
     if (waveTab && (tabBlocks == 0u || longFrames == 0u || longFrames > frames)) return hipErrorInvalidValue;
     const uint32_t groups = waveTab ? (frames - longFrames + S - 1u) / S : (frames + wf - 1u) / wf;
     if ((unsigned long long)tileCount * ((frames + S - 1u) / S) > 0x7fffffffull) return hipErrorInvalidValue;
-    if (rankFirst >= tileCount) return hipSuccess;
-    dim3 grid(waveTab ? tabBlocks + (tileCount - rankFirst) * groups : (tileCount - rankFirst) * groups), block(64);
+    if (rankEnd > tileCount) return hipErrorInvalidValue;
+    if (rankFirst >= rankEnd) return hipSuccess;
+    dim3 grid(waveTab ? tabBlocks + (rankEnd - rankFirst) * groups : (rankEnd - rankFirst) * groups), block(64);
 #ifdef CRT_POOL_TIMELINE
     { static unsigned long long* buf = nullptr; static size_t cap = 0;
       if (cap < (size_t)grid.x) { if (buf) (void)hipFree(buf); (void)hipMalloc((void**)&buf, (size_t)grid.x * 24); cap = grid.x; (void)hipMemcpyToSymbol(HIP_SYMBOL(crt::g_poolTimeline), &buf, sizeof(buf)); }
diff --git a/cpu-ray-tracer_amd/csrc/device/render_sky.hip b/cpu-ray-tracer_amd/csrc/device/render_sky.hip
--- /dev/null
+++ b/cpu-ray-tracer_amd/csrc/device/render_sky.hip
@@ -0,0 +1,54 @@
+#include "launch.h"
+#include "sample_body.h"
+
+namespace crt {
+
+__global__ __launch_bounds__(64) void render_sky_kernel(const Scene sc, float4* __restrict__ slab, Counters* __restrict__ counters, const uint32_t* __restrict__ tileOrder,
+                                                        uint32_t rankFirst, uint32_t skyTiles, uint32_t tileFirst, uint32_t tileStride, uint32_t tileCount, uint32_t tilesX,
+                                                        uint32_t sppFirst, uint32_t frames, uint32_t passes, uint32_t groups, unsigned long long* __restrict__ launchClk)
+{
+    const uint32_t lane = threadIdx.x;
+    const uint32_t r = blockIdx.x / groups, grp = blockIdx.x - r * groups;
+    if (r >= skyTiles) return;
+    const unsigned long long clk0 = launchClk ? wall_clock64() : 0ull;
+    const uint32_t tl = tileOrder[rankFirst + r];
+    const uint32_t tile = tileFirst + tl * tileStride;
+    const uint32_t tx = tile % tilesX, ty = tile / tilesX;
+    const uint32_t fr = grp * 64u + lane;
+    const uint32_t items = 256u * passes, rowLen = 64u * passes;
+    uint32_t paths = 0;
+    if (fr < frames) {
+        uint32_t seed = stream_seed(tx, ty, (uint32_t)sc.W, sppFirst, fr, passes);
+        const f3 camPos = mk3(sc.camPos[0], sc.camPos[1], sc.camPos[2]), TL = mk3(sc.topLeft[0], sc.topLeft[1], sc.topLeft[2]);
+        const f3 right = mk3(sc.primRight[0], sc.primRight[1], sc.primRight[2]), down = mk3(sc.primDown[0], sc.primDown[1], sc.primDown[2]);
+        uint32_t pix = 0, pass = 0;
+#pragma unroll 4
+        for (uint32_t item = 0; item < items; item++) {
+            const f3 v = primary_target(camPos, TL, right, down, sc.invW, sc.invH, tx, ty, pix, seed);
+            const f3 D = v * rcp_exact(sqrt_exact(dot3(v, v)));
+            float phi, theta; sky_angles(D, phi, theta);
+            const f3 L = tex_unpack(sc.texels[tex_index(sc.skyOffset, sc.skyW, sc.skyH, phi * CRT_INV2PI, theta * CRT_INVPI)]);
+            slab[slab_position(fr, tileCount, tl, pix, rowLen, passes, pass)] = make_float4(L.x, L.y, L.z, 0.0f);
+            if (++pass == passes) { pass = 0; pix++; }
+        }
+        paths = items;
+    }
+    const uint32_t sum = wave_sum(paths);
+    if (lane == 0 && sum) { atomicAdd(&counters->v[0], (unsigned long long)sum); atomicAdd(&counters->v[1], (unsigned long long)sum); }
+    if (launchClk && lane == 0) { atomicMax(&launchClk[0], ~clk0); atomicMax(&launchClk[1], wall_clock64()); }
+}
+
+}
+
+extern "C" hipError_t crt_launch_render_sky(const crt::Scene* sc, void* slab, crt::Counters* counters, const uint32_t* tileOrder, uint32_t rankFirst, uint32_t skyTiles,
+                                            uint32_t tileFirst, uint32_t tileStride, uint32_t tileCount, uint32_t tilesX, uint32_t sppFirst, uint32_t frames, uint32_t passes,
+                                            unsigned long long* launchClk, hipStream_t stream)
+{
+    if (skyTiles == 0 || frames == 0) return hipSuccess;
+    if (!tileOrder || rankFirst > tileCount || skyTiles > tileCount - rankFirst || passes == 0) return hipErrorInvalidValue;
+    const uint32_t groups = (frames + 63u) / 64u;
+    if ((unsigned long long)skyTiles * groups > 0x7fffffffull) return hipErrorInvalidValue;
+    hipLaunchKernelGGL(crt::render_sky_kernel, dim3(skyTiles * groups), dim3(64), 0, stream, *sc, (float4*)slab, counters, tileOrder, rankFirst, skyTiles, tileFirst, tileStride,
+                       tileCount, tilesX, sppFirst, frames, passes, groups, launchClk);
+    return hipGetLastError();
+}
diff --git a/cpu-ray-tracer_amd/csrc/device/sample_body.h b/cpu-ray-tracer_amd/csrc/device/sample_body.h
--- a/cpu-ray-tracer_amd/csrc/device/sample_body.h
+++ b/cpu-ray-tracer_amd/csrc/device/sample_body.h
@@ -104,6 +104,14 @@
         if (depth > k) { const float* fd = fst + (uint32_t)(3 * k) * 64u; L = mk3(fd[0], fd[64], fd[128]) * L; }
 }
 
+__device__ __forceinline__ uint32_t stream_seed(uint32_t tx, uint32_t ty, uint32_t W, uint32_t sppFirst, uint32_t frame, uint32_t passes)
+{
+    return init_seed(tx + ty * W + (sppFirst + frame * passes) * 1799u);
+}
+__device__ __forceinline__ size_t slab_position(uint32_t fr, uint32_t tileCount, uint32_t tl, uint32_t pix, uint32_t rowLen, uint32_t passes, uint32_t pass)
+{
+    return (((size_t)(fr >> 6) * tileCount + tl) * 256u + pix) * rowLen + ((fr & 63u) * passes + pass);
+}
 __device__ __forceinline__ f3 primary_target(f3 camPos, f3 TL, f3 right, f3 down, float invW, float invH, uint32_t tx, uint32_t ty, uint32_t pix, uint32_t& seed)
 {
     const int x = (int)(tx * 16u + (pix & 15u)), y = (int)(ty * 16u + (pix >> 4));
```
